# lancedb/lance

Hardware: AMD Instinct MI355X
Metric: QPS @ recall@10 (SIFT-1M IVF_PQ nlist=256 M=16) + index-build sec (higher is better)
Workload: dtype f32; 1 GPU; SIFT-1M-like 1Mx128 f32, IVF_PQ nlist=256 M=16 nbits=8, build+search on MI355X; n=1000000, d=128, nlist=256, m=16, k=10, nprobes=10, refine_factor=10, parallelism=single

## Files before the change

lance_amd/csrc/kernels.h:

```cpp
#pragma once
#include <stdint.h>

#include "common.h"

namespace lh {

struct PairwiseArgs {
  const void *x_native = nullptr;
  int x_dtype = 0;
  const float *x = nullptr;
  bool lanes32 = false;
  int64_t n = 0;
  int64_t ldx = 0;
  int x_batch_off = 0;
  const float *cent = nullptr;
  int k = 0;
  int64_t cent_batch_stride = 0;
  const float *bias = nullptr;
  int64_t bias_batch_stride = 0;
  uint32_t *ids = nullptr;
  float *dists = nullptr;
  int64_t out_batch_stride = 0;
  uint8_t *codes = nullptr;
  int codes_ld = 0;
  float *matrix = nullptr;
  const uint8_t *active = nullptr;
  bool x_aligned = false;
  bool cent_aligned = false;
  bool check_finite = false;
  const uint16_t *x_plane16 = nullptr;
  const float *x_plane_n2 = nullptr;
  int x_plane_dp = 0;
  float *part_vb = nullptr;
  float *part_v = nullptr;
  uint32_t *part_idx = nullptr;
};

struct PqmArgs {
  PairwiseArgs p;
  const void *xn = nullptr;
  const float *rcent = nullptr;
  const uint32_t *rpart = nullptr;
  int round_f16 = 0;
  uint32_t *fb_cnt;
  uint32_t *fb_items;
  int batches;
};
bool pq_mfma_supported(const PairwiseArgs &p, int d, int metric, int batches);
int launch_pq_mfma(lance_hip_ctx *ctx, const PairwiseArgs &p, int d, int batches);
bool pq_mfma_encode_supported(int dtype, int d, int m, int nbits, const void *x, const float *cent, const float *codebook, int64_t n);
int launch_pq_mfma_encode(lance_hip_ctx *ctx, int dtype, const void *x, int64_t n, int d, const float *cent, const uint32_t *part_ids,
                          int residual, const float *codebook, int m, uint8_t *codes);

struct FlatPool {
  const float *x;
  const void *x_native = nullptr;
  int x_dtype = 0;
  const uint64_t *row_ids;
  int64_t r0, r1;
  const float *q;
  int nq, k, cap;
  uint32_t *tkey;
  uint64_t *trid;
  uint32_t *cnt;
  uint32_t *pkeys;
  uint64_t *prids;
  uint32_t *overflow;
  const float *row_sy = nullptr;
  const float *q_norm = nullptr;
};

int launch_wide_filter(lance_hip_ctx *ctx, const FlatPool &fp, int d, int metric);
int build_allow_bits(lance_hip_ctx *ctx, const uint64_t *row_ids, uint64_t n, const uint8_t *allow_by_rowid, uint64_t n_allow, const uint32_t **bits_out);
bool flat_mfma_supported(int metric, int d, int nq, const void *x, const float *q);
int flat_mfma_prepare(lance_hip_ctx *ctx, const float *q, int nq, int d, const uint16_t **qhi, const uint16_t **qlo, const float **qn);
int launch_flat_filter_mfma(lance_hip_ctx *ctx, const FlatPool &e, int d, int metric, const uint16_t *qhi, const uint16_t *qlo, const float *qn);
bool flat_mfma_wide_supported(int metric, int d, int nq, int64_t n, const float *x, const float *q);
int flat_mfma_wide_prepare_rows(lance_hip_ctx *ctx, const float *x, int64_t n, int d, const uint16_t **xb, const float **xn2);
int flat_mfma_wide_prepare_queries(lance_hip_ctx *ctx, const float *q, int nq, int d, const uint16_t **qb, const float **qn2);
int launch_flat_filter_mfma_wide(lance_hip_ctx *ctx, const FlatPool &e, int d, int metric, const uint16_t *xb, const float *xn2, const uint16_t *qb,
                                 const float *qn2);

int launch_assign(lance_hip_ctx *ctx, const PairwiseArgs &p, int d, int metric, int batches);
bool assign_reads_native(PairwiseArgs p, int d, int batches);
bool encode_fused_supported(int dtype, int d, int m, int nbits, const void *x, const float *cent, const float *codebook);
int launch_encode_fused(lance_hip_ctx *ctx, int dtype, const void *x, int64_t n, int d, const float *cent, const uint32_t *part_ids,
                        int residual, const float *codebook, int m, uint8_t *codes);
bool xform_fused_supported(int dtype, int metric, int d, int m, int nbits, int64_t n, int nlist, const void *x, const float *cent,
                           const float *codebook, uint8_t *codes, bool lanes32);
int launch_xform_fused(lance_hip_ctx *ctx, int dtype, int metric, const void *x, int64_t n, int d, const float *cent, int nlist,
                       const float *codebook, int m, uint32_t *part_ids, float *dists, uint8_t *codes, bool round_f16);
bool xform_tail_supported(int d, int m, int nbits, int64_t n, const float *x, const float *cent, const float *codebook);
int launch_xform_tail(lance_hip_ctx *ctx, const float *x, int64_t n, int d, const float *cent, const uint32_t *part_ids, int residual, bool round_f16,
                      const float *codebook, int m, uint8_t *codes);
bool xform_pqtrain_supported(const PairwiseArgs &p, int sd, int batches);
int launch_xform_pqtrain(lance_hip_ctx *ctx, const PairwiseArgs &p, int sd, int batches, uint32_t *fb_cnt, uint32_t *fb_items);
bool xform_assign_supported(const PairwiseArgs &p, int d, int metric, int batches);
int launch_xform_assign(lance_hip_ctx *ctx, const PairwiseArgs &p, int d, int metric);
int launch_xform_sweep_groups(lance_hip_ctx *ctx, int metric, const float *q, uint32_t nq, int d, const float *cent, uint32_t nlist, uint32_t *maxbits,
                              float *gkey, int ng, float *e2, const uint16_t *cpl_ready = nullptr, const uint32_t *maxbits_ready = nullptr);
size_t xform_coarse_planes_elems(uint32_t nlist, int d);
int xform_coarse_planes(lance_hip_ctx *ctx, int metric, const float *cent, uint32_t nlist, int d, uint16_t *cpl, uint32_t *maxbits );
bool coarse_groups_shape(int d, uint32_t nlist);
bool mfma_assign_supported(const PairwiseArgs &p, int d, int batches);
int launch_assign_mfma(lance_hip_ctx *ctx, const PairwiseArgs &p, int d, int metric);
int launch_dist_matrix(lance_hip_ctx *ctx, const PairwiseArgs &p, int d, int metric, int batches);

int stable_group(lance_hip_ctx *ctx, const uint32_t *ids, int64_t n, int64_t id_stride, int k, int batches,
                 uint32_t *starts, uint32_t *sorted_rows, int64_t out_stride, const uint8_t *active);

int kmeans_train_batched(lance_hip_ctx *ctx, int metric, const float *x, int64_t n, int64_t ldx, int x_batch_off, int d,
                         int k, int B, uint32_t max_iters, double tol, float balance_factor_scaled, bool have_init,
                         const uint64_t *seeds, float *cent, double *loss_out, uint32_t *iters_out, bool f16_arith = false);

int kmeans_train_hierarchical(lance_hip_ctx *ctx, int metric, const float *x, int64_t n, int d, int target_k, uint32_t max_iters,
                              double tol, float bf_scaled, int hierarchical_k, uint64_t seed, float *cent_out, uint32_t *n_out,
                              bool f16_arith = false);
int check_dtype(int dtype, const char *what);
int model_dtype(int dtype);
int as_f32(lance_hip_ctx *ctx, int dtype, const void *p, size_t count, const char *slot, const float **out);
int widen_into(lance_hip_ctx *ctx, int dtype, const void *p, size_t count, float *dst);
int from_f32(lance_hip_ctx *ctx, int dtype, const float *src, void *dst, size_t count);
int launch_residual(lance_hip_ctx *ctx, const float *x, int64_t n, int d, const float *cent, const uint32_t *part_ids, float *out, bool f16);


bool pm_supported(const lance_hip_index *ix, uint32_t keff, int has_range, uint32_t nq, uint32_t nprobes);
int ivfpq_scan_merge_pm(lance_hip_ctx *ctx, const lance_hip_index *ix, const float *qs, uint32_t nq, const uint32_t *probes,
                        uint32_t nprobes, uint32_t keff, uint32_t k, bool do_refine, uint64_t *ids, float *dists,
                        uint64_t *cand_rid, uint32_t *cand_cnt, uint32_t *flags, const uint32_t *allow);
int find_partitions_f32(lance_hip_ctx *ctx, int metric, const float *qf, uint32_t nq, uint32_t d, const float *cf, uint32_t nlist,
                        uint32_t nprobes, uint32_t *part_ids, float *dists, bool lanes32);
bool flat_small_supported(int metric, int dtype, uint32_t d, uint32_t nq, uint32_t k, uint64_t n);
int flat_topk_small(lance_hip_ctx *ctx, int metric, int dtype, const void *x, const uint64_t *row_ids, uint64_t n, uint32_t d, const float *q,
                    uint32_t nq, uint32_t k, uint64_t *ids, float *dists, bool *done);
bool coarse_mfma_supported(int metric, int d, uint32_t nq, uint32_t nlist, uint32_t nprobes, bool lanes32, const float *q, const float *cent);
int find_partitions_mfma(lance_hip_ctx *ctx, int metric, const float *q, uint32_t nq, int d, const float *cent, uint32_t nlist, uint32_t nprobes,
                         float *matrix, uint32_t *part_ids, float *dists, const uint16_t *cpl_ready = nullptr, const uint32_t *maxbits_ready = nullptr);
int launch_normalize(lance_hip_ctx *ctx, const float *x, int64_t n, int d, float *out, bool f16);
int launch_normalize_planes(lance_hip_ctx *ctx, const float *x, int64_t n, int d, float *out, bool f16, uint16_t *plane16, int dp, float *n2);

int qscan_index_constants(lance_hip_ctx *ctx, lance_hip_index *ix);
constexpr int QSCAN_SEG_CAP = 256;
struct SelectOut;
bool qscan_supported(const lance_hip_index *ix, uint32_t nq, uint32_t nprobes);
bool qscan_tiled_shape(int m, int sd);
int qscan_classb_to_rescan(lance_hip_ctx *ctx, const uint32_t *tbound, uint32_t nq, uint32_t nprobes, uint32_t *seg_cnt, uint32_t *qovf);
int qscan_nearest_keys(lance_hip_ctx *ctx, const uint32_t *probes, uint32_t nq, uint32_t nprobes, uint32_t *keys, uint32_t nb = 1);
int qscan_item_tables(lance_hip_ctx *ctx, const uint32_t *pair_starts, int nlist, int G, uint32_t *item_start, int4 *desc, uint32_t max_items);
int qscan_group(lance_hip_ctx *ctx, const uint32_t *probes, uint32_t nq, uint32_t nprobes, int nlist, const uint32_t *tglobal,
                uint32_t *keys, uint32_t *tbound, uint32_t *pair_starts, uint32_t *pair_idx, uint32_t *item_start4, int4 *desc4,
                uint32_t max_items4, int G = 4, int dot = 0);
int qbound_launch(lance_hip_ctx *ctx, const lance_hip_index *ix, const float *qs, uint32_t nq, uint32_t keff, const uint32_t *pair_starts0,
                  const uint32_t *pair_idx0, uint32_t *item_start, int4 *desc, uint32_t max_items, uint32_t *tglobal, const uint32_t *allow);
int qscan_launch(lance_hip_ctx *ctx, const lance_hip_index *ix, const float *qs, uint32_t nq, uint32_t nprobes, const uint32_t *pair_idx,
                 const uint32_t *item_start4, const int4 *desc4, uint32_t max_items4, const uint32_t *tbound, uint32_t *seg_cnt,
                 uint32_t *seg_pos, uint32_t *qovf, const uint32_t *allow, const uint32_t *probes = nullptr);
bool qscan_pt_enabled(const lance_hip_index *ix);
int qscan_pt_mode(const lance_hip_index *ix);
int qbound_pt_launch(lance_hip_ctx *ctx, const lance_hip_index *ix, const float *qs, uint32_t nq, uint32_t nprobes, uint32_t keff,
                     const uint32_t *probes, const uint32_t *pair_starts0, const uint32_t *pair_idx0, uint32_t *item_start, int4 *desc,
                     uint32_t max_items, uint32_t *tglobal, const uint32_t *allow);
int qmerge_launch(lance_hip_ctx *ctx, const lance_hip_index *ix, const float *qs, uint32_t nq, const uint32_t *probes, uint32_t nprobes,
                  const uint32_t *tbound, uint32_t *tglobal, const uint32_t *seg_cnt, const uint32_t *seg_pos, const uint32_t *qovf,
                  uint32_t *pool_key, uint32_t *pool_pos, uint32_t *pool_cnt, int pool_cap, const SelectOut &o, const uint32_t *allow,
                  const uint32_t *qslack = nullptr, const float *seg_val = nullptr, const float *seg_scale = nullptr);
constexpr int LH_NOT_TAKEN = 1;
bool mscan_supported(const lance_hip_index *ix, uint32_t nq, uint32_t nprobes);
bool mscan_batch_shape(const lance_hip_index *ix, uint32_t nq, uint32_t nprobes);
bool mscan_dot_ready(const lance_hip_index *ix, uint32_t nq, uint32_t nprobes);
int mscan_launch(lance_hip_ctx *ctx, const lance_hip_index *ix, const float *qs, uint32_t nq, uint32_t nprobes, const uint32_t *probes,
                 const uint32_t *pair_starts, const uint32_t *pair_idx, const uint32_t *tbound, uint32_t *seg_cnt, uint32_t *seg_pos,
                 uint32_t *qovf, const uint32_t *allow, uint32_t **qslack_out, float **seg_val_out, float **seg_scale_out);
void mscan_cut_params(int *cut_shift, uint32_t *cut_slack);
int mscan_prewarm(lance_hip_ctx *ctx, const lance_hip_index *ix);
int msbound_launch(lance_hip_ctx *ctx, const lance_hip_index *ix, const float *qs, uint32_t nq, uint32_t keff, const uint32_t *pair_starts0,
                   const uint32_t *pair_idx0, uint32_t *item_start, int4 *desc, uint32_t max_items, uint32_t *tglobal, const uint32_t *allow,
                   uint32_t nb = 1);
int qscan_items(lance_hip_ctx *ctx, const uint32_t *pair_starts, int nvp, int G, uint32_t *item_start, int4 *desc, uint32_t max_items);
const uint8_t *raw_compact_prepare(lance_hip_ctx *ctx, const lance_hip_index *ix);

}
```

lance_amd/csrc/search_ms.hip:

```cpp
#include <algorithm>
#include <cmath>
#include <cstdio>
#include <cstdlib>
#include <cstring>
#include <vector>

#include "common.h"
#include "exact.cuh"
#include "index.h"
#include "kernels.h"
#include "search_common.cuh"
#include "q_common.cuh"

namespace lh {

typedef _Float16 ms_h8 __attribute__((ext_vector_type(8)));
typedef _Float16 ms_h4 __attribute__((ext_vector_type(4)));
typedef float ms_f16v __attribute__((ext_vector_type(16)));

constexpr float MS_SE = 30000.0f;
constexpr float MS_SLACK_CAP = 1500.0f;
constexpr int MS_CUT_SHIFT = 6;
typedef __attribute__((address_space(1))) const void *ms_gptr;
typedef __attribute__((address_space(3))) void *ms_lptr;

__global__ __launch_bounds__(256) void ms_codebook_kernel(const float *__restrict__ cb, int64_t nwords, int sd, float scale, _Float16 *__restrict__ cbh,
                                                          float *__restrict__ cbn2, const float *__restrict__ mu) {
  const int64_t w = (int64_t)blockIdx.x * 256 + threadIdx.x;
  if (w >= nwords) return;
  float s = 0.0f;
  for (int u = 0; u < sd; ++u) {
    const float v = mu ? cb[w * sd + u] - mu[(w >> 8) * sd + u] : cb[w * sd + u];
    cbh[w * sd + u] = (_Float16)(v * scale);
    s += v * v;
  }
  cbn2[w] = s;
}

__global__ __launch_bounds__(256) void ms_row_norm_kernel(const uint8_t *__restrict__ codes, int64_t n, int m, const float *__restrict__ cbn2, float sigma2,
                                                          float *__restrict__ row_cn2) {
  const int64_t r = (int64_t)blockIdx.x * 256 + threadIdx.x;
  if (r >= n) return;
  const uint8_t *rc = codes + r * m;
  float s = 0.0f;
  for (int mm = 0; mm < m; ++mm) s += cbn2[mm * 256 + rc[mm]];
  row_cn2[r] = s * sigma2;
}

__global__ __launch_bounds__(256) void ms_max_kernel(const float *__restrict__ v, int64_t n, uint32_t *__restrict__ out) {
  float m = 0.0f;
  for (int64_t i = (int64_t)blockIdx.x * 256 + threadIdx.x; i < n; i += (int64_t)gridDim.x * 256) m = fmaxf(m, v[i]);
#pragma unroll
  for (int o = 32; o > 0; o >>= 1) m = fmaxf(m, __shfl_xor(m, o, 64));
  if ((threadIdx.x & 63) == 0) atomicMax(out, __float_as_uint(m));
}

__global__ __launch_bounds__(256) void ms_part_max_kernel(const float *__restrict__ v, const uint32_t *__restrict__ part_offsets, float inv_sigma,
                                                          float *__restrict__ cmaxp) {
  __shared__ float wm[4];
  const uint32_t b = part_offsets[blockIdx.x], e = part_offsets[blockIdx.x + 1];
  float m = 0.0f;
  for (uint32_t i = b + threadIdx.x; i < e; i += 256) m = fmaxf(m, v[i]);
#pragma unroll
  for (int o = 32; o > 0; o >>= 1) m = fmaxf(m, __shfl_xor(m, o, 64));
  if ((threadIdx.x & 63) == 0) wm[threadIdx.x >> 6] = m;
  __syncthreads();
  if (threadIdx.x == 0) cmaxp[blockIdx.x] = sqrtf(fmaxf(fmaxf(wm[0], wm[1]), fmaxf(wm[2], wm[3]))) * inv_sigma * 1.0001f;
}

struct MsPrepArgs {
  const float *q, *centroids;
  const uint32_t *pair_idx;
  const uint32_t *pair_starts;
  const uint32_t *probes;
  const uint32_t *tbound;
  int d, nprobes, nlist, round_f16;
  float sigma;
  _Float16 *rh;
  f4 *prm;
  uint32_t *qslack;
  uint32_t *seg_cnt, *qovf, *ovf;
  uint32_t nan_slot;
  f2 *prm2;
  int dot = 0;
  float cmax = 0.0f;
  const float *cmaxp = nullptr;
  float cmax_full = 0.0f;
  const float *mu = nullptr;
  int m = 0;
};

constexpr int MS_PPW = 4;
__global__ __launch_bounds__(256) void ms_prep_kernel(MsPrepArgs p) {
  const uint32_t g0 = (blockIdx.x * 4u + (threadIdx.x >> 6)) * (uint32_t)MS_PPW;
  const uint32_t ng = p.pair_starts[p.nlist];
  const int lane = threadIdx.x & 63;
  if (blockIdx.x == 0 && threadIdx.x == 0) p.prm[p.nan_slot] = f4{__uint_as_float(0x7FC00000u), 0.0f, 0.0f, 0.0f};
  if (g0 >= ng) return;
  uint32_t pair[MS_PPW];
  const float *qv[MS_PPW], *cv[MS_PPW];
#pragma unroll
  for (int t = 0; t < MS_PPW; ++t) {
    const uint32_t g = min(g0 + (uint32_t)t, ng - 1u);
    pair[t] = p.pair_idx[g];
  }
#pragma unroll
  for (int t = 0; t < MS_PPW; ++t) {
    qv[t] = p.q + (int64_t)(pair[t] / (uint32_t)p.nprobes) * p.d;
    cv[t] = p.centroids + (int64_t)p.probes[pair[t]] * p.d;
  }
  float n2[MS_PPW], vmax[MS_PPW], qmu[MS_PPW];
  bool bad[MS_PPW];
#pragma unroll
  for (int t = 0; t < MS_PPW; ++t) { n2[t] = 0.0f; vmax[t] = 0.0f; qmu[t] = 0.0f; bad[t] = false; }
  for (int e = lane; e < p.d; e += 64) {
    float v[MS_PPW];
    const float mue = p.dot ? p.mu[e] : 0.0f;
#pragma unroll
    for (int t = 0; t < MS_PPW; ++t) v[t] = p.dot ? qv[t][e] : qv[t][e] - cv[t][e];
    const float hs = p.dot ? 0.5f * p.sigma : p.sigma;
#pragma unroll
    for (int t = 0; t < MS_PPW; ++t) {
      if (p.round_f16 && !p.dot) v[t] = __half2float(__float2half_rn(v[t]));
      n2[t] += v[t] * v[t];
      qmu[t] += v[t] * mue;
      vmax[t] = fmaxf(vmax[t], fabsf(v[t]));
      bad[t] |= !(fabsf(v[t]) < INFINITY);
      if (g0 + (uint32_t)t < ng) p.rh[(int64_t)(g0 + t) * p.d + e] = (_Float16)(v[t] * hs);
    }
  }
#pragma unroll
  for (int t = 0; t < MS_PPW; ++t) {
#pragma unroll
    for (int o = 32; o > 0; o >>= 1) {
      n2[t] += __shfl_xor(n2[t], o, 64); qmu[t] += __shfl_xor(qmu[t], o, 64); vmax[t] = fmaxf(vmax[t], __shfl_xor(vmax[t], o, 64));
    }
    bad[t] = __any(bad[t]);
  }
  float n2l = n2[0], vml = vmax[0], qmul = qmu[0]; bool badl = bad[0]; uint32_t pairl = pair[0];
#pragma unroll
  for (int t = 1; t < MS_PPW; ++t) if (lane == t) { n2l = n2[t]; vml = vmax[t]; qmul = qmu[t]; badl = bad[t]; pairl = pair[t]; }
  if (lane >= MS_PPW || g0 + (uint32_t)lane >= ng) return;
  const uint32_t q = pairl / (uint32_t)p.nprobes;
  const float T = key_to_float(p.tbound[q]);
  const float sqd = sqrtf((float)p.d) + 1.0f;
  const float sig2 = p.sigma * p.sigma;
  float s, eu, lim, zsum;
  bool ok;
  if (p.dot) {
    const float qn = sqrtf(n2l) * 1.000001f;
    const float G = qn * p.cmax * 1.000001f, Gf = qn * p.cmax_full * 1.000001f;
    const float e_abs = 6.1035156e-5f * sqd * (qn + 2.0f * p.cmax) / p.sigma + (float)p.d * 3.7252903e-9f / sig2;
    auto slack = [&](float g) {
      return 1.05f * (9.9609375e-4f * g + 1.5258789e-5f * (g + 1.0f + fabsf(T) + fabsf(qmul) + Gf) + 5.9604645e-8f * (float)((p.m + 2) * (p.m + 2))) + e_abs;
    };
    const float Tq = (T - 1.0f) + qmul;
    const float Tp = (Tq + G) + slack(G);
    s = MS_SE / Tp;
    const float Gp = fminf(G, qn * p.cmaxp[p.probes[pairl]] * 1.000001f);
    const float E = slack(Gp);
    eu = E * s * 1.1f + 3.0f;
    lim = Tq + E;
    zsum = (lim + G) * s;
    ok = !badl && fabsf(T) < INFINITY && Tp > 0.0f && Tp < INFINITY && s > 0.0f && s < INFINITY && Gf < INFINITY && vml * p.sigma < 60000.0f &&
         eu <= MS_SLACK_CAP && fabsf(lim * sig2) < INFINITY && G * s < 1e30f && fabsf(zsum) < 1e30f;
  } else {
    s = MS_SE / T;
    const float rn = sqrtf(n2l) * 1.000001f, st = sqrtf(T) * 1.000001f;
    const float e_abs = 6.1035156e-5f * sqd * (3.0f * rn + 2.0f * st) / p.sigma + (float)p.d * 3.7252903e-9f / (p.sigma * p.sigma);
    const float E = 1.05f * (1.9921875e-3f * rn * (rn + st) + 1.2207031e-4f * (n2l + T)) + e_abs;
    eu = E * s * 1.1f + 3.0f;
    lim = (T * 1.0000077f + E) - n2l;
    zsum = (T * 1.0000077f + E) * s;
    ok = !badl && T > 0.0f && T < INFINITY && s > 0.0f && s < INFINITY && n2l < INFINITY && vml * p.sigma < 60000.0f &&
         eu <= MS_SLACK_CAP && fabsf(lim * sig2) < INFINITY && n2l * s < 1e30f;
  }
  f4 o;
  if (ok) {
    o.x = -(lim * sig2); o.y = s / sig2; o.z = n2l * s;
    p.prm2[pairl] = f2{o.y, zsum};
    atomicMax(&p.qslack[q], (uint32_t)ceilf(eu));
  } else {
    o.x = __uint_as_float(0x7FC00000u); o.y = 0.0f; o.z = 0.0f;
    p.seg_cnt[pairl] = (uint32_t)Q_CAP + 1u;
    p.qovf[q] = 1u;
    p.ovf[1u + atomicAdd(&p.ovf[0], 1u)] = pairl;
  }
  o.w = __uint_as_float(pairl);
  p.prm[g0 + (uint32_t)lane] = o;
}

#ifndef LH_MS3_PB
#define LH_MS3_PB 512
#endif
constexpr int MS3_PB = LH_MS3_PB;
constexpr int MS3_RS = 3072;
static int ms_rows_per_slice() {
  static const int v = [] { const char *e = getenv("LANCE_HIP_MS_RS"); const int x = e ? atoi(e) : MS3_RS; return x >= 64 ? (x / 64) * 64 : MS3_RS; }();
  return v;
}
static int ms_rows_per_slice2() {
  static const int v = [] { const char *e = getenv("LANCE_HIP_MS_RS2"); const int x = e ? atoi(e) : 0; return x >= 64 ? (x / 64) * 64 : ms_rows_per_slice(); }();
  return v;
}
struct MsSlice { uint32_t off, np, row_begin, row_count, gs, qp, pad0, pad1; };
__host__ __device__ __forceinline__ uint32_t ms_nrs(uint32_t np, uint32_t rs1, uint32_t rs2) { return np <= rs1 ? (np ? 1u : 0u) : 1u + (np - rs1 + rs2 - 1u) / rs2; }
__device__ __forceinline__ uint32_t ms_row_begin(uint32_t rs, uint32_t rs1, uint32_t rs2) { return rs ? rs1 + (rs - 1u) * rs2 : 0u; }
__device__ __forceinline__ uint32_t ms_row_count(uint32_t rs, uint32_t np, uint32_t rs1, uint32_t rs2) {
  return rs ? min(rs2, np - ms_row_begin(rs, rs1, rs2)) : min(rs1, np);
}

__device__ __forceinline__ uint32_t ms_work_class(uint32_t rows, uint32_t pairs, uint32_t rs_rows) {
  const uint64_t w = (uint64_t)rows * pairs;
  return 31u - (uint32_t)min<uint64_t>(31u, w * 32u / ((uint64_t)rs_rows * MS3_PB));
}
struct MsSplit { uint32_t npb, blk, nrs; };
__device__ __forceinline__ MsSplit ms_split(uint32_t qp, uint32_t np, uint32_t rs_rows, uint32_t rs2_rows) {
  MsSplit r;
  r.npb = (qp + MS3_PB - 1) / MS3_PB;
  r.blk = r.npb ? ((((qp + r.npb - 1) / r.npb) + 31u) & ~31u) : 0u;
  r.nrs = ms_nrs(np, rs_rows, rs2_rows);
  return r;
}

__global__ __launch_bounds__(256) void ms_slice_table_kernel(const uint32_t *__restrict__ pair_starts, const uint32_t *__restrict__ part_offsets, int nlist,
                                                             uint32_t rs_rows, uint32_t rs2_rows, uint32_t cls_rows, uint32_t *__restrict__ slice_start,
                                                             uint32_t *__restrict__ slice_ctr, uint32_t *__restrict__ cls_cursor) {
  __shared__ uint32_t wsum[4];
  __shared__ uint32_t carry_s;
  __shared__ uint32_t hist[32];
  const int lane = threadIdx.x & 63, wave = threadIdx.x >> 6;
  if (threadIdx.x == 0) { carry_s = 0; slice_ctr[0] = 0u; }
  if (threadIdx.x < 32) hist[threadIdx.x] = 0u;
  __syncthreads();
  for (int base = 0; base < nlist; base += 256) {
    const int i = base + threadIdx.x;
    uint32_t v = 0;
    if (i < nlist) {
      const uint32_t qp = pair_starts[i + 1] - pair_starts[i], np = part_offsets[i + 1] - part_offsets[i];
      const MsSplit sp = ms_split(qp, np, rs_rows, rs2_rows);
      v = sp.npb * sp.nrs;
      for (uint32_t pb = 0; pb < sp.npb; pb += max(1u, sp.npb - 1u)) {
        const uint32_t pairs = min(sp.blk, qp - pb * sp.blk), npb_same = (pb + 1 == sp.npb) ? 1u : sp.npb - 1u;
        if (sp.nrs > 0) atomicAdd(&hist[ms_work_class(ms_row_count(0u, np, rs_rows, rs2_rows), pairs, cls_rows)], npb_same);
        if (sp.nrs > 2) atomicAdd(&hist[ms_work_class(rs2_rows, pairs, cls_rows)], npb_same * (sp.nrs - 2u));
        if (sp.nrs > 1) atomicAdd(&hist[ms_work_class(ms_row_count(sp.nrs - 1u, np, rs_rows, rs2_rows), pairs, cls_rows)], npb_same);
        if (sp.npb == 1) break;
      }
    }
    uint32_t incl = v;
#pragma unroll
    for (int off = 1; off < 64; off <<= 1) {
      const uint32_t t = __shfl_up(incl, off, 64);
      if (lane >= off) incl += t;
    }
    if (lane == 63) wsum[wave] = incl;
    __syncthreads();
    uint32_t woff = 0;
    for (int w = 0; w < wave; ++w) woff += wsum[w];
    const uint32_t carry = carry_s;
    if (i < nlist) slice_start[i] = carry + woff + incl - v;
    __syncthreads();
    if (threadIdx.x == 255) carry_s = carry + woff + incl;
    __syncthreads();
  }
  if (threadIdx.x == 0) {
    slice_start[nlist] = carry_s;
    uint32_t run = 0;
    for (int c = 0; c < 32; ++c) { cls_cursor[c] = run; run += hist[c]; }
  }
}

__global__ __launch_bounds__(256) void ms_slice_desc_kernel(const uint32_t *__restrict__ slice_start, const uint32_t *__restrict__ pair_starts,
                                                            const uint32_t *__restrict__ part_offsets, int nlist, uint32_t rs_rows, uint32_t rs2_rows, uint32_t cls_rows,
                                                            MsSlice *__restrict__ slices, uint32_t *__restrict__ cls_cursor, uint32_t *__restrict__ order) {
  const int part = blockIdx.x * 4 + (threadIdx.x >> 6), lane = threadIdx.x & 63;
  if (part >= nlist) return;
  const uint32_t s0 = slice_start[part], s1 = slice_start[part + 1];
  if (s1 == s0) return;
  const uint32_t off = part_offsets[part], np = part_offsets[part + 1] - off;
  const uint32_t gs = pair_starts[part], qp = pair_starts[part + 1] - gs;
  const MsSplit sp = ms_split(qp, np, rs_rows, rs2_rows);
  for (uint32_t t = (uint32_t)lane; t < s1 - s0; t += 64u) {
    const uint32_t pb = t / sp.nrs, rs = t - pb * sp.nrs;
    MsSlice u;
    u.off = off; u.np = np; u.row_begin = ms_row_begin(rs, rs_rows, rs2_rows); u.row_count = ms_row_count(rs, np, rs_rows, rs2_rows);
    u.gs = gs + pb * sp.blk; u.qp = min(sp.blk, qp - pb * sp.blk); u.pad0 = u.pad1 = 0u;
    slices[s0 + t] = u;
    order[atomicAdd(&cls_cursor[ms_work_class(u.row_count, u.qp, cls_rows)], 1u)] = s0 + t;
  }
}

struct MscanArgs {
  const uint32_t *order;
  const MsSlice *slices;
  const uint32_t *slice_start;
  uint32_t *slice_ctr;
  const uint8_t *codes;
  const _Float16 *cbh;
  const float *row_cn2;
  const _Float16 *rh;
  const f4 *prm;
  const f2 *prm2;
  uint32_t nan_slot;
  int nlist, nprobes;
  uint32_t *seg_cnt, *seg_pos;
  uint2 *seg_pv = nullptr;
  uint32_t *ovf;
  const uint32_t *allow;
#ifdef LH_TIMING_EXPERIMENTS
  int dbg = 0;
#endif
  unsigned long long *prof_slices = nullptr;
  unsigned long long *prof = nullptr;
};

#ifdef LH_TIMING_EXPERIMENTS
#define MS_DBG(p) ((p).dbg)
#else
#define MS_DBG(p) 0
#endif

constexpr int MS_QH = 64;
template <int SD, int KS, bool PROF = false>
__global__ __launch_bounds__(1024, 4) void ivfpq_mscan_kernel(MscanArgs p) {
  constexpr int D = KS * 16;
  constexpr int M = D / SD;
  constexpr int RB = D * 2;
  constexpr int CPR = RB / 16;
  constexpr int RPK = 256 / RB;
  constexpr int SPI = 16384 / RB;
  __shared__ __attribute__((aligned(16))) char sB[MS3_PB * RB];
  __shared__ __attribute__((aligned(16))) float sLim[MS3_PB];
  __shared__ __attribute__((aligned(16))) uint32_t sPair[MS3_PB];
  __shared__ __attribute__((aligned(8))) uint2 sQ[16][2][MS_QH + 1];
  __shared__ uint32_t s_slice, s_chunk;
  const int lane = threadIdx.x & 63, wave = __builtin_amdgcn_readfirstlane((int)(threadIdx.x >> 6));
  const int j = lane & 31, g = lane >> 5;
  const uint32_t nslices = p.slice_start[p.nlist];

  uint2 *const qw = &sQ[wave][0][0];
  uint32_t cur = 0;
  uint32_t qn = 0;
  uint32_t pd_n = 0, pd_base = 0;
  uint32_t pd_k = 0;
  float ncn2v = 0.0f;
  long long pc_t0 = 0, pc_stage = 0, pc_gather = 0, pc_tiles = 0, pc_flush = 0, pct = 0, pc_nchunk = 0;
  if constexpr (PROF) { pc_t0 = clock64(); pct = pc_t0; }
  auto flush_end = [&]() {
    if (pd_n) {
      if ((uint32_t)lane < pd_n && pd_k != 0xFFFFFFFFu) {
        const uint2 ent = qw[((uint32_t)(MS_QH + 1) - cur) + (uint32_t)lane];
        const uint32_t pair = sPair[ent.x >> 8];
        if (pd_k < (uint32_t)Q_CAP) {
          p.seg_pv[(int64_t)pair * Q_CAP + pd_k] = make_uint2(pd_base + (ent.x & 255u), ent.y);
        } else if (pd_k == (uint32_t)Q_CAP) {
          p.ovf[1u + atomicAdd(&p.ovf[0], 1u)] = pair;
        }
      }
      pd_n = 0;
    }
  };
  auto flush_begin = [&](uint32_t pos_base) {
    pd_k = 0xFFFFFFFFu;
    {
      const uint2 raw = qw[cur + (uint32_t)lane];
      const uint32_t ln_e = raw.x & 63u, vv = (raw.x >> 6) & 15u, jbb = raw.x >> 10;
      const float nv = __shfl(ncn2v, (int)(ln_e & 31u), 64);
      const uint2 ent = make_uint2(((jbb * 32u + 4u * (ln_e >> 5) + (vv & 3u) + 8u * (vv >> 2)) << 8) | (ln_e & 31u), __float_as_uint(__uint_as_float(raw.y) - nv));
      if ((uint32_t)lane < qn && !(MS_DBG(p) & 1)) {
        qw[cur + (uint32_t)lane] = ent;
        if (row_allowed(p.allow, pos_base + (ent.x & 255u))) pd_k = atomicAdd(&p.seg_cnt[sPair[ent.x >> 8]], 1u);
      }
    }
    pd_n = qn; pd_base = pos_base; qn = 0;
    cur = (uint32_t)(MS_QH + 1) - cur;
  };

  for (;;) {
    __syncthreads();
    if (threadIdx.x == 0) { s_slice = atomicAdd(p.slice_ctr, 1u); s_chunk = 0u; }
    __syncthreads();
    const uint32_t slice = s_slice;
    if (slice >= nslices) break;
    long long pc_slice0 = 0;
    if constexpr (PROF) pc_slice0 = clock64();
    const MsSlice U = p.slices[p.order[slice]];
    const int Qp = (int)U.qp;
    const int nslots = ((Qp + 31) >> 5) << 5;
    {
      const char *src = reinterpret_cast<const char *>(p.rh + (int64_t)U.gs * D);
#pragma unroll 4
      for (int it = 0; it < MS3_PB / SPI; ++it) {
        const int slot = it * SPI + wave * (SPI / 16) + lane / CPR, k = lane % CPR;
        if (it * SPI < nslots && slot < Qp)
          __builtin_amdgcn_global_load_lds((ms_gptr)(src + (int64_t)slot * RB + ((k ^ ((slot / RPK) & (CPR - 1))) << 4)),
                                           (ms_lptr)(&sB[(it * SPI + wave * (SPI / 16)) * RB]), 16, 0, 0);
      }
      const int slot = (wave & 7) * 64 + lane;
      if (slot < nslots) {
        const float *ps = reinterpret_cast<const float *>(slot < Qp && !(MS_DBG(p) & 2) ? p.prm + (int64_t)U.gs + slot : p.prm + p.nan_slot);
        if (wave < 8) __builtin_amdgcn_global_load_lds((ms_gptr)ps, (ms_lptr)(&sLim[(wave & 7) * 64]), 4, 0, 0);
        else __builtin_amdgcn_global_load_lds((ms_gptr)(ps + 3), (ms_lptr)(&sPair[(wave & 7) * 64]), 4, 0, 0);
      }
    }
    asm volatile("s_waitcnt vmcnt(0)" ::: "memory");
    __syncthreads();
    if constexpr (PROF) { const long long t = clock64(); pc_stage += t - pct; pct = t; }
    const uint32_t nchunks = (U.row_count + 31u) >> 5;
    const int nblk = nslots >> 5;
    const int row_end = (int)(U.row_begin + U.row_count);

    for (;;) {
      uint32_t c = 0;
      if (lane == 0) c = atomicAdd(&s_chunk, 1u);
      c = (uint32_t)__builtin_amdgcn_readfirstlane((int)c);
      if (c >= nchunks) break;
      const int row0 = (int)(U.row_begin + c * 32u);

      ms_h8 rw[KS];
      {
        const int rowc = min(row0 + j, row_end - 1);
        uint32_t cw[M / 4];
        {
          const uint4 *rc4 = reinterpret_cast<const uint4 *>(p.codes + ((int64_t)U.off + rowc) * M);
#pragma unroll
          for (int w = 0; w < M / 16; ++w) { const uint4 t = rc4[w]; cw[4 * w] = t.x; cw[4 * w + 1] = t.y; cw[4 * w + 2] = t.z; cw[4 * w + 3] = t.w; }
        }
        ncn2v = row0 + j < row_end ? -p.row_cn2[(int64_t)U.off + rowc] : -INFINITY;
        auto code = [&](int mm) -> uint32_t { return (cw[mm >> 2] >> (8 * (mm & 3))) & 255u; };
#pragma unroll
        for (int s = 0; s < KS; ++s) {
          if constexpr (SD == 8) {
            const uint32_t c0 = code(2 * s), c1 = code(2 * s + 1);
            const int mm = 2 * s + g;
            rw[s] = *reinterpret_cast<const ms_h8 *>(reinterpret_cast<const char *>(p.cbh) + (uint32_t)(((uint32_t)mm * 256u + (g ? c1 : c0)) * 16u));
          } else {
            static_assert(SD == 4, "sub-dimension 4 / 8");
            const uint32_t c0 = g ? code(4 * s + 2) : code(4 * s), c1 = g ? code(4 * s + 3) : code(4 * s + 1);
            const int mm = 4 * s + 2 * g;
            const ms_h4 lo = *reinterpret_cast<const ms_h4 *>(reinterpret_cast<const char *>(p.cbh) + (uint32_t)(((uint32_t)mm * 256u + c0) * 8u));
            const ms_h4 hi = *reinterpret_cast<const ms_h4 *>(reinterpret_cast<const char *>(p.cbh) + (uint32_t)(((uint32_t)(mm + 1) * 256u + c1) * 8u));
            rw[s] = ms_h8{lo[0], lo[1], lo[2], lo[3], hi[0], hi[1], hi[2], hi[3]};
          }
        }
      }
      const uint32_t pos_base = U.off + (uint32_t)row0;
      asm volatile("s_waitcnt vmcnt(0)" ::: "memory");
#pragma unroll
      for (int s = 0; s < KS; ++s) asm volatile("" : "+v"(rw[s]));
      asm volatile("" : "+v"(ncn2v));
      if constexpr (PROF) {
        const long long t = clock64(); pc_gather += t - pct; pct = t;
      }

      ms_h8 qa[KS];
      auto load_qa = [&](int jbx) {
        const int sl = jbx * 32 + j;
        const char *br = &sB[sl * RB];
        const int key = (sl / RPK) & (CPR - 1);
#pragma unroll
        for (int s = 0; s < KS; ++s) qa[s] = *reinterpret_cast<const ms_h8 *>(br + (((2 * s + g) ^ key) << 4));
      };
      load_qa(0);
      for (int jb = 0; jb < nblk; ++jb) {
        const int slot = jb * 32 + j;
        ms_f16v acc;
        {
          const f4 *lp = reinterpret_cast<const f4 *>(&sLim[jb * 32 + 4 * g]);
#pragma unroll
          for (int vq = 0; vq < 4; ++vq) {
            const f4 t = lp[2 * vq];
            acc[4 * vq] = t.x; acc[4 * vq + 1] = t.y; acc[4 * vq + 2] = t.z; acc[4 * vq + 3] = t.w;
          }
        }
        if (qn > (uint32_t)(MS_QH - 32)) {
          if constexpr (PROF) { const long long t = clock64(); pc_tiles += t - pct; pct = t; }
          flush_end(); flush_begin(pos_base);
          if constexpr (PROF) { const long long t = clock64(); pc_flush += t - pct; pct = t; }
        }
        uint32_t qraw = qn;
#pragma unroll
        for (int s = 0; s < KS; ++s) acc = __builtin_amdgcn_mfma_f32_32x32x16_f16(qa[s], rw[s], acc, 0, 0, 0);
        __builtin_amdgcn_sched_barrier(0);
        load_qa(min(jb + 1, nblk - 1));
        __builtin_amdgcn_sched_barrier(0);
        uint64_t mk[16];
#pragma unroll
        for (int v = 0; v < 16; ++v) mk[v] = __ballot(acc[v] <= ncn2v);
        __builtin_amdgcn_sched_barrier(0);
#pragma unroll
        for (int v = 0; v < 16; ++v) {
          if (mk[v]) {
            const uint32_t idx = min(qraw + __builtin_amdgcn_mbcnt_hi((uint32_t)(mk[v] >> 32), __builtin_amdgcn_mbcnt_lo((uint32_t)mk[v], 0u)),
                                     (uint32_t)MS_QH);
            if (acc[v] <= ncn2v) {
#ifdef MS_LN_RECOMPUTE
              uint32_t ln;
              asm volatile("v_mbcnt_lo_u32_b32 %0, -1, 0\n\tv_mbcnt_hi_u32_b32 %0, -1, %0" : "=v"(ln));
#else
              const uint32_t ln = (uint32_t)lane;
#endif
              qw[cur + idx] = make_uint2((((uint32_t)jb << 10) | (uint32_t)(v << 6)) | ln, __float_as_uint(acc[v]));
            }
            qraw += (uint32_t)__popcll(mk[v]);
          }
        }
        qn = min(qraw, (uint32_t)MS_QH);
        if (qraw > (uint32_t)MS_QH) {
          if (g == 0 && slot < Qp) {
            const uint32_t pair = sPair[slot];
            const uint32_t k = atomicAdd(&p.seg_cnt[pair], (uint32_t)Q_CAP + 1u);
            if (k <= (uint32_t)Q_CAP) p.ovf[1u + atomicAdd(&p.ovf[0], 1u)] = pair;
          }
        }
      }
      if constexpr (PROF) { const long long t = clock64(); pc_tiles += t - pct; pct = t; }
      flush_end(); flush_begin(pos_base);
      if constexpr (PROF) { const long long t = clock64(); pc_flush += t - pct; pct = t; ++pc_nchunk; }
    }
    flush_end();
    if constexpr (PROF) {
      __syncthreads();
      if (threadIdx.x == 0 && p.prof_slices) p.prof_slices[slice] = (unsigned long long)(clock64() - pc_slice0);
    }
  }
  if constexpr (PROF) {
    if (lane == 0) {
      const long long t1 = clock64();
      atomicAdd(&p.prof[0], (unsigned long long)pc_stage);
      atomicAdd(&p.prof[1], (unsigned long long)pc_gather);
      atomicAdd(&p.prof[2], (unsigned long long)pc_tiles);
      atomicAdd(&p.prof[3], (unsigned long long)pc_flush);
      atomicAdd(&p.prof[4], (unsigned long long)(t1 - pc_t0));
      atomicAdd(&p.prof[5], 1ull);
      atomicAdd(&p.prof[6], (unsigned long long)pc_nchunk);
      atomicMax(&p.prof[7], (unsigned long long)(t1 - pc_t0));
    }
  }
}

constexpr int MSB_BQ = 64;
constexpr int MSB_BINS = 512;
constexpr float MSB_MEAN_BIN = 496.0f;
struct MsBoundArgs {
  const float *q, *centroids, *cb_mean;
  const uint32_t *pair_idx0;
  const uint32_t *item_start;
  const int4 *desc;
  const uint32_t *part_offsets;
  const uint8_t *codes;
  const _Float16 *cbh;
  const float *row_cn2;
  int d, nlist, keff, round_f16;
  float sigma;
  uint32_t *tglobal;
  const uint32_t *allow;
  int dot = 0;
  float cmax = 0.0f, cmax_full = 0.0f;
  const float *cmaxp = nullptr;
  uint32_t nb = 1;
};

template <int SD, int KS>
__global__ __launch_bounds__(1024) void ms_bound_kernel(MsBoundArgs p) {
  constexpr int D = KS * 16;
  constexpr int M = D / SD;
  constexpr int RB = D * 2;
  constexpr int CPR = RB / 16;
  constexpr int RPK = 256 / RB;
  constexpr int CBB = 256 * D * 2;
  __shared__ __attribute__((aligned(16))) char sCB[CBB];
  __shared__ __attribute__((aligned(16))) char sB[MSB_BQ * RB];
  __shared__ __attribute__((aligned(16))) uint32_t sH[MSB_BQ * (MSB_BINS / 2)];
  __shared__ __attribute__((aligned(16))) float sPa[MSB_BQ];
  __shared__ __attribute__((aligned(16))) float sPb[MSB_BQ];
  __shared__ float sN2[MSB_BQ], sSb[MSB_BQ], sRmu[MSB_BQ];
  __shared__ uint32_t s_chunk;
  const int lane = threadIdx.x & 63, wave = threadIdx.x >> 6;
  const int j = lane & 31, g = lane >> 5;
  const uint32_t item = blockIdx.x;
  if (item >= p.item_start[p.nlist]) return;
  const int4 dsc = p.desc[item];
  const int part = dsc.x, i0 = dsc.y, cnt = dsc.z;
  const uint32_t off = p.part_offsets[part];
  const int np_all = (int)(p.part_offsets[part + 1] - off);
  if (np_all < p.keff) return;
  const int np = min(np_all, 65535);
  const int nslots = ((cnt + 31) >> 5) << 5;

  for (int b = (int)threadIdx.x * 16; b < CBB; b += 1024 * 16)
    *reinterpret_cast<uint4 *>(&sCB[b]) = *reinterpret_cast<const uint4 *>(reinterpret_cast<const char *>(p.cbh) + b);
  for (int i = threadIdx.x; i < MSB_BQ * (MSB_BINS / 2); i += 1024) sH[i] = 0u;
  if (threadIdx.x == 0) s_chunk = 0u;
  {
    constexpr int SPW = MSB_BQ / 16;
    const int e = 2 * lane;
    uint32_t qi[SPW];
#pragma unroll
    for (int t = 0; t < SPW; ++t) { const int sl = wave + 16 * t; qi[t] = sl < cnt ? p.pair_idx0[i0 + sl] / p.nb : 0u; }
    f2 qv[SPW], cv = {0.0f, 0.0f}, mu = {0.0f, 0.0f};
    if (e < D) {
      if (!p.dot) cv = *reinterpret_cast<const f2 *>(p.centroids + (int64_t)part * D + e);
      mu = *reinterpret_cast<const f2 *>(p.cb_mean + e);
    }
    const float hs = p.dot ? 0.5f * p.sigma : p.sigma;
#pragma unroll
    for (int t = 0; t < SPW; ++t) {
      qv[t] = f2{0.0f, 0.0f};
      if (wave + 16 * t < cnt && e < D) qv[t] = *reinterpret_cast<const f2 *>(p.q + (int64_t)qi[t] * D + e);
    }
#pragma unroll
    for (int t = 0; t < SPW; ++t) {
      const int sl = wave + 16 * t;
      if (sl >= nslots) break;
      const int key = (sl / RPK) & (CPR - 1);
      float n2 = 0.0f, vmax = 0.0f, rmu = 0.0f;
      bool bad = false;
      uint32_t packed = 0u;
      if (sl < cnt && e < D) {
        float v0 = qv[t].x - cv.x, v1 = qv[t].y - cv.y;
        if (p.round_f16 && !p.dot) { v0 = __half2float(__float2half_rn(v0)); v1 = __half2float(__float2half_rn(v1)); }
        n2 = v0 * v0 + v1 * v1;
        vmax = fmaxf(fabsf(v0), fabsf(v1));
        rmu = v0 * mu.x + v1 * mu.y;
        bad = !(fabsf(v0) < INFINITY) || !(fabsf(v1) < INFINITY);
        typedef _Float16 h2 __attribute__((ext_vector_type(2)));
        const h2 hv = {(_Float16)(v0 * hs), (_Float16)(v1 * hs)};
        packed = __builtin_bit_cast(uint32_t, hv);
      }
      if (e < D) *reinterpret_cast<uint32_t *>(&sB[sl * RB + ((((e >> 3) ^ key)) << 4) + ((e & 7) << 1)]) = packed;
#pragma unroll
      for (int o = 32; o > 0; o >>= 1) {
        n2 += __shfl_xor(n2, o, 64); rmu += __shfl_xor(rmu, o, 64); vmax = fmaxf(vmax, __shfl_xor(vmax, o, 64));
      }
      bad = __any(bad);
      if (lane == 0) {
        float a = __uint_as_float(0x7FC00000u), b = 0.0f, sb = 0.0f;
        if (sl < cnt) {
          const float G = p.dot ? sqrtf(n2) * 1.000001f * fminf(p.cmax, p.cmaxp[part]) * 1.000001f : 0.0f;
          const float mean = p.dot ? G : n2 - 2.0f * rmu + p.cb_mean[D];
          const float off = p.dot ? G : n2;
          sb = MSB_MEAN_BIN / mean;
          const float sig2 = p.sigma * p.sigma;
          const bool ok = !bad && off < INFINITY && vmax * p.sigma < 60000.0f && mean > 0.0f && mean < INFINITY && sb > 0.0f && sb < INFINITY &&
                          off * sb < 1e30f && sb / sig2 > 0.0f && sb / sig2 < INFINITY;
          if (ok) { a = sb / sig2; b = off * sb; }
        }
        sPa[sl] = a; sPb[sl] = b; sN2[sl] = n2; sSb[sl] = sb; sRmu[sl] = rmu;
      }
    }
  }
  for (int sl = nslots + (int)threadIdx.x; sl < MSB_BQ; sl += 1024) { sPa[sl] = __uint_as_float(0x7FC00000u); sPb[sl] = 0.0f; }
  __syncthreads();

  const uint32_t nchunks = ((uint32_t)np + 31u) >> 5;
  const int nblk = nslots >> 5;
  auto take = [&]() -> uint32_t {
    uint32_t c = 0;
    if (lane == 0) c = atomicAdd(&s_chunk, 1u);
    return (uint32_t)__builtin_amdgcn_readfirstlane((int)c);
  };
  uint32_t cwn[M / 4];
  float cn2n = INFINITY;
  auto request = [&](uint32_t c) {
    const int row0 = (int)(c * 32u);
    const int rowc = min(row0 + j, np - 1);
    const uint4 *rc4 = reinterpret_cast<const uint4 *>(p.codes + ((int64_t)off + rowc) * M);
#pragma unroll
    for (int w = 0; w < M / 16; ++w) { const uint4 t = rc4[w]; cwn[4 * w] = t.x; cwn[4 * w + 1] = t.y; cwn[4 * w + 2] = t.z; cwn[4 * w + 3] = t.w; }
    const bool live = row0 + j < np && row_allowed(p.allow, off + (uint32_t)rowc);
    cn2n = live ? p.row_cn2[(int64_t)off + rowc] : INFINITY;
  };
  uint32_t c = take();
  if (c < nchunks) request(c);
  while (c < nchunks) {
    const uint32_t cnext = take();
    uint32_t cw[M / 4];
#pragma unroll
    for (int w = 0; w < M / 4; ++w) cw[w] = cwn[w];
    const float cn2v = cn2n;
    asm volatile("s_waitcnt vmcnt(0)" ::: "memory");
#pragma unroll
    for (int w = 0; w < M / 4; ++w) asm volatile("" : "+v"(cw[w]));
    if (cnext < nchunks) request(cnext);
    ms_h8 rw[KS];
    {
      auto code = [&](int mm) -> uint32_t { return (cw[mm >> 2] >> (8 * (mm & 3))) & 255u; };
#pragma unroll
      for (int s = 0; s < KS; ++s) {
        if constexpr (SD == 8) {
          const uint32_t c0 = code(2 * s), c1 = code(2 * s + 1);
          const int mm = 2 * s + g;
          rw[s] = *reinterpret_cast<const ms_h8 *>(&sCB[((uint32_t)mm * 256u + (g ? c1 : c0)) * 16u]);
        } else {
          static_assert(SD == 4, "sub-dimension 4 / 8");
          const uint32_t c0 = g ? code(4 * s + 2) : code(4 * s), c1 = g ? code(4 * s + 3) : code(4 * s + 1);
          const int mm = 4 * s + 2 * g;
          const ms_h4 lo = *reinterpret_cast<const ms_h4 *>(&sCB[((uint32_t)mm * 256u + c0) * 8u]);
          const ms_h4 hi = *reinterpret_cast<const ms_h4 *>(&sCB[((uint32_t)(mm + 1) * 256u + c1) * 8u]);
          rw[s] = ms_h8{lo[0], lo[1], lo[2], lo[3], hi[0], hi[1], hi[2], hi[3]};
        }
      }
    }
    for (int jb = 0; jb < nblk; ++jb) {
      ms_h8 qa[KS];
      {
        const int sl = jb * 32 + j;
        const char *br = &sB[sl * RB];
        const int key = (sl / RPK) & (CPR - 1);
#pragma unroll
        for (int s = 0; s < KS; ++s) qa[s] = *reinterpret_cast<const ms_h8 *>(br + (((2 * s + g) ^ key) << 4));
      }
      ms_f16v acc;
#pragma unroll
      for (int v = 0; v < 16; ++v) acc[v] = 0.0f;
#pragma unroll
      for (int s = 0; s < KS; ++s) acc = __builtin_amdgcn_mfma_f32_32x32x16_f16(qa[s], rw[s], acc, 0, 0, 0);
      const f4 *pa = reinterpret_cast<const f4 *>(&sPa[jb * 32 + 4 * g]);
      const f4 *pb = reinterpret_cast<const f4 *>(&sPb[jb * 32 + 4 * g]);
#pragma unroll
      for (int vq = 0; vq < 4; ++vq) {
        const f4 a4 = pa[2 * vq], b4 = pb[2 * vq];
#pragma unroll
        for (int e = 0; e < 4; ++e) {
          const float t = __builtin_fmaf(acc[4 * vq + e] + cn2v, a4[e], b4[e]);
          if (t < (float)MSB_BINS) {
            const int bin = max((int)t, 0);
            const int slot = jb * 32 + 8 * vq + 4 * g + e;
            atomicAdd(&sH[slot * (MSB_BINS / 2) + (bin >> 1)], 1u << (16 * (bin & 1)));
          }
        }
      }
    }
    c = cnext;
  }
  __syncthreads();
  for (int sl = wave; sl < cnt; sl += 16) {
    const float a = sPa[sl];
    if (!(a > 0.0f)) continue;
    const uint4 hw = *reinterpret_cast<const uint4 *>(&sH[sl * (MSB_BINS / 2) + lane * 4]);
    const uint32_t loc[8] = {hw.x & 0xFFFFu, hw.x >> 16, hw.y & 0xFFFFu, hw.y >> 16, hw.z & 0xFFFFu, hw.z >> 16, hw.w & 0xFFFFu, hw.w >> 16};
    uint32_t tot = 0;
#pragma unroll
    for (int i = 0; i < 8; ++i) tot += loc[i];
    uint32_t incl = tot;
#pragma unroll
    for (int o = 1; o < 64; o <<= 1) {
      const uint32_t t = __shfl_up(incl, o, 64);
      if (lane >= o) incl += t;
    }
    uint32_t run = incl - tot;
    int found = -1;
#pragma unroll
    for (int i = 0; i < 8; ++i) {
      run += loc[i];
      if (found < 0 && run >= (uint32_t)p.keff) found = lane * 8 + i;
    }
    const uint64_t mask = __ballot(found >= 0);
    if (mask) {
      const int leader = __ffsll((long long)mask) - 1;
      const int bin = __shfl(found, leader, 64);
      if (lane == 0) {
        const float n2 = sN2[sl], sb = sSb[sl];
        const float Ta = (float)(bin + 1) / sb * 1.000001f;
        const float rn = sqrtf(n2) * 1.000001f, st = sqrtf(Ta) * 1.000001f;
        const float sqd = sqrtf((float)D) + 1.0f;
        if (p.dot) {
          const float G = rn * fminf(p.cmax, p.cmaxp[part]) * 1.000001f, Gf = rn * p.cmax_full * 1.000001f, qmu = sRmu[sl];
          const float tmag = fabsf(1.0f - qmu) + G + Ta;
          const float e_abs = 6.1035156e-5f * sqd * (rn + 2.0f * p.cmax) / p.sigma + (float)D * 3.7252903e-9f / (p.sigma * p.sigma);
          const float E = 1.05f * (9.9609375e-4f * G + 1.5258789e-5f * (G + 1.0f + tmag + fabsf(qmu) + Gf) + 5.9604645e-8f * (float)((M + 2) * (M + 2))) + e_abs;
          const float T = (((1.0f - qmu) - G) + Ta) + (1.1f * E + 1.5258789e-5f * tmag);
          if (fabsf(T) < INFINITY) atomicMin(&p.tglobal[p.pair_idx0[i0 + sl] / p.nb], order_key(T));
        } else {
        const float e_abs = 6.1035156e-5f * sqd * (3.0f * rn + 2.0f * st) / p.sigma + (float)D * 3.7252903e-9f / (p.sigma * p.sigma);
        const float E = 1.05f * (1.9921875e-3f * rn * (rn + st) + 1.2207031e-4f * (n2 + Ta)) + e_abs;
        const float T = (Ta + 1.1f * E) * 1.0000153f;
        if (T > 0.0f && T < INFINITY) atomicMin(&p.tglobal[p.pair_idx0[i0 + sl] / p.nb], order_key(T));
        }
      }
    }
  }
}

static bool ms_shape(const lance_hip_index *ix, int *sd_out, int *ks_out) {
  if (!ix || ix->m == 0 || ix->nbits != 8 || ix->d % ix->m != 0) return false;
  const int d = (int)ix->d, m = (int)ix->m, sd = d / m;
  if (!(m == 16 || m == 32)) return false;
  const bool ok = (d == 128 && (sd == 8 || sd == 4)) || (d == 64 && sd == 4);
  if (!ok) return false;
  if (sd_out) *sd_out = sd;
  if (ks_out) *ks_out = d / 16;
  return true;
}

bool mscan_batch_shape(const lance_hip_index *ix, uint32_t nq, uint32_t nprobes) {
  static const bool off = getenv("LANCE_HIP_NO_MSCAN") != nullptr;
  static const uint32_t minq = getenv("LANCE_HIP_MSCAN_MINQ") ? (uint32_t)std::max(1, atoi(getenv("LANCE_HIP_MSCAN_MINQ"))) : 96u;
  if (off || !ms_shape(ix, nullptr, nullptr)) return false;
  if (ix->metric != LANCE_HIP_L2 && ix->metric != LANCE_HIP_COSINE && ix->metric != LANCE_HIP_DOT) return false;
  return (uint64_t)nq * nprobes >= (uint64_t)minq * ix->nlist;
}

static bool ms_dot_skew_ok(const lance_hip_index *ix) {
  static const double skew = getenv("LANCE_HIP_DOT_FLOW_SKEW") ? atof(getenv("LANCE_HIP_DOT_FLOW_SKEW")) : 1e18;
  return (double)ix->max_part * (double)ix->nlist <= skew * (double)ix->n;
}

bool mscan_dot_ready(const lance_hip_index *ix, uint32_t nq, uint32_t nprobes) {
  static const bool off = getenv("LANCE_HIP_NO_MSBOUND") != nullptr || getenv("LANCE_HIP_NO_DOT_FLOW") != nullptr;
  if (off || !mscan_batch_shape(ix, nq, nprobes) || !ix->cb_mean) return false;
  if (!ms_dot_skew_ok(ix)) return false;
  lance_hip_index *mix = const_cast<lance_hip_index *>(ix);
  std::lock_guard<std::mutex> lk(mix->lazy_mu);
  return !mix->ms || mix->ms->usable;
}

bool mscan_supported(const lance_hip_index *ix, uint32_t nq, uint32_t nprobes) {
  return mscan_batch_shape(ix, nq, nprobes) && qscan_supported(ix, nq, nprobes);
}

static int mscan_prepare(lance_hip_ctx *ctx, lance_hip_index *ix) {
  std::lock_guard<std::mutex> lk(ix->lazy_mu);
  if (ix->ms) return LANCE_HIP_OK;
  const int d = (int)ix->d, m = (int)ix->m, sd = d / m;
  const int64_t nwords = (int64_t)m * 256;
  std::vector<float> cb((size_t)nwords * sd);
  LH_CHECK_HIP(hipMemcpyAsync(cb.data(), ix->codebook, cb.size() * 4, hipMemcpyDeviceToHost, ctx->stream));
  LH_CHECK_HIP(hipStreamSynchronize(ctx->stream));
  const bool dot = ix->metric == LANCE_HIP_DOT;
  std::vector<float> mu;
  if (dot && ix->cb_mean) {
    mu.resize((size_t)d);
    LH_CHECK_HIP(hipMemcpyAsync(mu.data(), ix->cb_mean, (size_t)d * 4, hipMemcpyDeviceToHost, ctx->stream));
    LH_CHECK_HIP(hipStreamSynchronize(ctx->stream));
  }
  auto *mc = new lance_hip_index::MsConst();
  if (dot) {
    if (!ix->cb_mean) { mc->usable = false; ix->ms = mc; return LANCE_HIP_OK; }
    double tot = 0.0;
    for (int mm = 0; mm < m; ++mm) {
      double best = 0.0;
      for (int c = 0; c < 256; ++c) {
        double sq = 0.0;
        for (int u = 0; u < sd; ++u) { const double v = cb[((size_t)mm * 256 + c) * sd + u]; sq += v * v; }
        best = std::max(best, sq);
      }
      tot += best;
    }
    mc->cmax_full = (float)(std::sqrt(tot) * 1.00001);
  }
  float cbmax = 0.0f;
  for (size_t i = 0; i < cb.size(); ++i) cbmax = std::max(cbmax, std::fabs(dot ? cb[i] - mu[(i / ((size_t)256 * sd)) * sd + i % sd] : cb[i]));
  if (!(cbmax > 0.0f) || !std::isfinite(cbmax) || ix->n == 0) {
    mc->usable = false;
    ix->ms = mc;
    return LANCE_HIP_OK;
  }
  int e = 0;
  (void)std::frexp(cbmax, &e);
  mc->sigma = std::ldexp(1.0f, 13 - e);
  bool ok = hipMalloc(reinterpret_cast<void **>(&mc->cbh), (size_t)nwords * sd * 2) == hipSuccess;
  ok = ok && hipMalloc(reinterpret_cast<void **>(&mc->cbn2), (size_t)nwords * 4) == hipSuccess;
  ok = ok && hipMalloc(reinterpret_cast<void **>(&mc->row_cn2), (size_t)ix->n * 4) == hipSuccess;
  if (dot) ok = ok && hipMalloc(reinterpret_cast<void **>(&mc->cmaxp), (size_t)std::max<uint32_t>(ix->nlist, 1u) * 4) == hipSuccess;
  auto drop = [&]() { (void)hipFree(mc->cbh); (void)hipFree(mc->cbn2); (void)hipFree(mc->row_cn2); (void)hipFree(mc->cmaxp); delete mc; };
  if (!ok) { drop(); set_error("matrix-core scan: out of device memory for the index constants"); return LANCE_HIP_ENOMEM; }
  hipLaunchKernelGGL(ms_codebook_kernel, dim3((unsigned)cdiv((uint64_t)nwords, 256)), dim3(256), 0, ctx->stream, ix->codebook, nwords, sd,
                     -2.0f * mc->sigma, reinterpret_cast<_Float16 *>(mc->cbh), mc->cbn2, dot ? ix->cb_mean : nullptr);
  hipLaunchKernelGGL(ms_row_norm_kernel, dim3((unsigned)cdiv(ix->n, 256)), dim3(256), 0, ctx->stream, ix->codes, (int64_t)ix->n, m, mc->cbn2,
                     mc->sigma * mc->sigma, mc->row_cn2);
  uint32_t rowmax_bits = 0;
  if (dot) {
    uint32_t *mx = reinterpret_cast<uint32_t *>(mc->cbn2);
    (void)lh::memset_async(mx, 0, 4, ctx->stream);
    hipLaunchKernelGGL(ms_max_kernel, dim3(256), dim3(256), 0, ctx->stream, mc->row_cn2, (int64_t)ix->n, mx);
    (void)hipMemcpyAsync(&rowmax_bits, mx, 4, hipMemcpyDeviceToHost, ctx->stream);
    hipLaunchKernelGGL(ms_part_max_kernel, dim3(ix->nlist), dim3(256), 0, ctx->stream, mc->row_cn2, ix->part_offsets, 1.0f / mc->sigma, mc->cmaxp);
    (void)lh::memset_async(mc->row_cn2, 0, (size_t)ix->n * 4, ctx->stream);
  }
  for (uint32_t pid = 0; pid < ix->nlist; ++pid) {
    const uint32_t rs = ms_nrs((uint32_t)(ix->part_offsets_h[pid + 1] - ix->part_offsets_h[pid]), (uint32_t)ms_rows_per_slice(), (uint32_t)ms_rows_per_slice2());
    mc->sum_rs += rs; mc->max_rs = std::max(mc->max_rs, rs);
  }
  if (hipGetLastError() != hipSuccess || hipStreamSynchronize(ctx->stream) != hipSuccess) {
    drop();
    set_error("matrix-core scan: building the index constants failed");
    return LANCE_HIP_ERUNTIME;
  }
  if (dot) {
    float rm; memcpy(&rm, &rowmax_bits, 4);
    mc->cmax = (float)(std::sqrt((double)rm) / (double)mc->sigma * 1.0001);
    if (!(mc->cmax > 0.0f) || !std::isfinite(mc->cmax)) mc->cmax = mc->cmax_full;
  }
  mc->usable = true;
  ix->ms = mc;
  return LANCE_HIP_OK;
}

int mscan_launch(lance_hip_ctx *ctx, const lance_hip_index *ix_c, const float *qs, uint32_t nq, uint32_t nprobes, const uint32_t *probes,
                 const uint32_t *pair_starts, const uint32_t *pair_idx, const uint32_t *tbound, uint32_t *seg_cnt, uint32_t *seg_pos,
                 uint32_t *qovf, const uint32_t *allow, uint32_t **qslack_out, float **seg_val_out, float **seg_scale_out) {
  lance_hip_index *ix = const_cast<lance_hip_index *>(ix_c);
  int sd = 0, ks = 0;
  if (!ms_shape(ix, &sd, &ks)) return LH_NOT_TAKEN;
  LH_TRY(mscan_prepare(ctx, ix));
  if (!ix->ms->usable) return LH_NOT_TAKEN;
  const int d = (int)ix->d, nlist = (int)ix->nlist;
  const size_t npairs = (size_t)nq * nprobes;
  const uint64_t cap = (uint64_t)ix->ms->sum_rs + (uint64_t)ix->ms->max_rs * cdiv(npairs, MS3_PB) + 8;
  _Float16 *rh = reinterpret_cast<_Float16 *>(ctx->scratch("ms.rh", (npairs + 32) * (size_t)d * 2));
  f4 *prm = reinterpret_cast<f4 *>(ctx->scratch("ms.prm", (npairs + 32) * 16));
  f2 *prm2 = reinterpret_cast<f2 *>(ctx->scratch("ms.prm2", npairs * 8));
  uint32_t *qslack = ctx->scratch_t<uint32_t>("ms.qslack", nq);
  uint32_t *slice_start = ctx->scratch_t<uint32_t>("ms.slice_start", (size_t)nlist + 2 + 32);
  MsSlice *slices = reinterpret_cast<MsSlice *>(ctx->scratch("ms.slices", cap * sizeof(MsSlice)));
  uint32_t *order = ctx->scratch_t<uint32_t>("ms.order", cap);
  float *seg_val = ctx->scratch_t<float>("ms.seg_val", npairs * Q_CAP * 2);
  uint32_t *ovf = ctx->scratch_t<uint32_t>("q.ovf", npairs + 1);
  if (!rh || !prm || !prm2 || !qslack || !slice_start || !slices || !order || !seg_val || !ovf) return LANCE_HIP_ENOMEM;
  uint32_t *slice_ctr = slice_start + nlist + 1, *cls_cursor = slice_ctr + 1;
  const uint32_t nan_slot = (uint32_t)npairs + 1u;
  {
    ScopedTimer t(ctx, "q_residual");
    LH_CHECK_HIP(lh::memset_multi(ctx->stream, {{seg_cnt, 0, npairs * 4}, {qovf, 0, (size_t)nq * 4}, {qslack, 0, (size_t)nq * 4}, {ovf, 0, 4}}));
    MsPrepArgs pa;
    pa.q = qs; pa.centroids = ix->centroids; pa.pair_idx = pair_idx; pa.pair_starts = pair_starts; pa.probes = probes; pa.tbound = tbound;
    pa.d = d; pa.nprobes = (int)nprobes; pa.nlist = nlist; pa.round_f16 = ix->dtype == LANCE_HIP_F16 ? 1 : 0;
    pa.sigma = ix->ms->sigma; pa.rh = rh; pa.prm = prm; pa.qslack = qslack; pa.seg_cnt = seg_cnt; pa.qovf = qovf; pa.ovf = ovf;
    pa.nan_slot = nan_slot; pa.prm2 = prm2;
    pa.dot = ix->metric == LANCE_HIP_DOT ? 1 : 0; pa.cmax = ix->ms->cmax; pa.cmax_full = ix->ms->cmax_full; pa.cmaxp = ix->ms->cmaxp; pa.mu = ix->cb_mean; pa.m = (int)ix->m;
    hipLaunchKernelGGL(ms_prep_kernel, dim3((unsigned)cdiv(npairs, 4 * MS_PPW)), dim3(256), 0, ctx->stream, pa);
    const uint32_t rs_rows = (uint32_t)ms_rows_per_slice(), rs2_rows = (uint32_t)ms_rows_per_slice2();
    static const bool no_order = getenv("LANCE_HIP_MS_NOORDER") != nullptr;
    const uint32_t cls_rows = no_order ? 0x40000000u : rs_rows;
    hipLaunchKernelGGL(ms_slice_table_kernel, dim3(1), dim3(256), 0, ctx->stream, pair_starts, ix->part_offsets, nlist, rs_rows, rs2_rows, cls_rows, slice_start,
                       slice_ctr, cls_cursor);
    hipLaunchKernelGGL(ms_slice_desc_kernel, dim3((unsigned)cdiv((uint64_t)nlist, 4)), dim3(256), 0, ctx->stream, slice_start, pair_starts, ix->part_offsets,
                       nlist, rs_rows, rs2_rows, cls_rows, slices, cls_cursor, order);
  }
  ScopedTimer t(ctx, "ivfpq_scan_c1");
  ScopedTimer tm(ctx, "ivfpq_mscan");
  MscanArgs a;
  a.order = order; a.slices = slices; a.slice_start = slice_start; a.slice_ctr = slice_ctr; a.codes = ix->codes;
  a.cbh = reinterpret_cast<const _Float16 *>(ix->ms->cbh); a.row_cn2 = ix->ms->row_cn2; a.rh = rh; a.prm = prm; a.prm2 = prm2;
  a.nan_slot = nan_slot; a.nlist = nlist; a.nprobes = (int)nprobes;
  a.seg_cnt = seg_cnt; a.seg_pos = seg_pos; a.seg_pv = reinterpret_cast<uint2 *>(seg_val); a.ovf = ovf; a.allow = allow;
#ifdef LH_TIMING_EXPERIMENTS
  static const int dbg = [] {
    const int v = getenv("LANCE_HIP_MS_DBG") ? atoi(getenv("LANCE_HIP_MS_DBG")) : 0;
    if (v) fprintf(stderr, "lance_hip: LANCE_HIP_MS_DBG=%d -- timing experiment, search RESULTS ARE WRONG\n", v);
    return v;
  }();
  a.dbg = dbg;
#endif
  static const int grid_env = getenv("LANCE_HIP_MS_GRID") ? atoi(getenv("LANCE_HIP_MS_GRID")) : 0;
  const unsigned grid = (unsigned)std::min<uint64_t>((uint64_t)(grid_env > 0 ? std::min(grid_env, ctx->num_cus) : ctx->num_cus), cap);
  static const bool prof = getenv("LANCE_HIP_MS_PROF") != nullptr;
  if (prof && sd == 8 && ks == 8 && !ctx->capturing) {
    a.prof = ctx->scratch_t<unsigned long long>("ms.prof", 8);
    if (!a.prof) return LANCE_HIP_ENOMEM;
    LH_CHECK_HIP(lh::memset_async(a.prof, 0, 64, ctx->stream));
    a.prof_slices = ctx->scratch_t<unsigned long long>("ms.prof_slices", cap);
    if (!a.prof_slices) return LANCE_HIP_ENOMEM;
    LH_CHECK_HIP(lh::memset_async(a.prof_slices, 0, cap * 8, ctx->stream));
    hipLaunchKernelGGL((ivfpq_mscan_kernel<8, 8, true>), dim3(grid), dim3(1024), 0, ctx->stream, a);
    unsigned long long h[8];
    LH_CHECK_HIP(hipMemcpyAsync(h, a.prof, 64, hipMemcpyDeviceToHost, ctx->stream));
    LH_CHECK_HIP(hipStreamSynchronize(ctx->stream));
    {
      std::vector<unsigned long long> st(cap);
      std::vector<MsSlice> sl(cap);
      std::vector<uint32_t> ord(cap), ss((size_t)nlist + 1);
      (void)hipMemcpy(st.data(), a.prof_slices, cap * 8, hipMemcpyDeviceToHost);
      (void)hipMemcpy(sl.data(), slices, cap * sizeof(MsSlice), hipMemcpyDeviceToHost);
      (void)hipMemcpy(ord.data(), order, cap * 4, hipMemcpyDeviceToHost);
      (void)hipMemcpy(ss.data(), slice_start, ((size_t)nlist + 1) * 4, hipMemcpyDeviceToHost);
      const uint32_t ns = ss[nlist];
      std::vector<uint32_t> idx(ns);
      for (uint32_t i = 0; i < ns; ++i) idx[i] = i;
      std::sort(idx.begin(), idx.end(), [&](uint32_t x, uint32_t y) { return st[x] > st[y]; });
      double tot = 0, totw = 0;
      for (uint32_t i = 0; i < ns; ++i) { tot += (double)st[i]; totw += (double)sl[ord[i]].row_count * sl[ord[i]].qp; }
      fprintf(stderr, "[ms prof] %u slices, mean %.0f ticks, mean ticks per 1000 cells %.2f; slowest (taken#, ticks, rows, pairs, ticks per 1000 cells):", ns, tot / ns, tot / totw * 1e3);
      for (uint32_t t = 0; t < std::min<uint32_t>(ns, 12); ++t) {
        const uint32_t i = idx[t];
        fprintf(stderr, " (%u, %llu, %u, %u, %.2f)", i, st[i], sl[ord[i]].row_count, sl[ord[i]].qp, (double)st[i] / ((double)sl[ord[i]].row_count * sl[ord[i]].qp) * 1e3);
      }
      fprintf(stderr, " | last taken:");
      for (uint32_t i = ns > 12 ? ns - 12 : 0; i < ns; ++i)
        fprintf(stderr, " (%u, %llu, %u, %u)", i, st[i], sl[ord[i]].row_count, sl[ord[i]].qp);
      fprintf(stderr, "\n");
    }
    if (h[5])
      fprintf(stderr, "[ms prof] waves=%llu chunks/wave %.2f | s_memtime ticks per wave: stage+barriers %.0f | gather %.0f | tiles %.0f | flush %.0f | life %.0f (longest %llu)\n",
              h[5], (double)h[6] / h[5], (double)h[0] / h[5], (double)h[1] / h[5], (double)h[2] / h[5], (double)h[3] / h[5], (double)h[4] / h[5], h[7]);
  } else if (sd == 8 && ks == 8) hipLaunchKernelGGL((ivfpq_mscan_kernel<8, 8>), dim3(grid), dim3(1024), 0, ctx->stream, a);
  else if (sd == 4 && ks == 8) hipLaunchKernelGGL((ivfpq_mscan_kernel<4, 8>), dim3(grid), dim3(1024), 0, ctx->stream, a);
  else if (sd == 4 && ks == 4) hipLaunchKernelGGL((ivfpq_mscan_kernel<4, 4>), dim3(grid), dim3(1024), 0, ctx->stream, a);
  else { set_error("matrix-core scan: unsupported shape (d=%d, sd=%d)", d, sd); return LANCE_HIP_EINVAL; }
  LH_CHECK_HIP(hipGetLastError());
  *qslack_out = qslack; *seg_val_out = seg_val; *seg_scale_out = reinterpret_cast<float *>(prm2);
  return LANCE_HIP_OK;
}

int msbound_launch(lance_hip_ctx *ctx, const lance_hip_index *ix_c, const float *qs, uint32_t nq, uint32_t keff, const uint32_t *pair_starts0,
                   const uint32_t *pair_idx0, uint32_t *item_start, int4 *desc, uint32_t max_items, uint32_t *tglobal, const uint32_t *allow,
                   uint32_t nb) {
  static const bool off = getenv("LANCE_HIP_NO_MSBOUND") != nullptr;
  lance_hip_index *ix = const_cast<lance_hip_index *>(ix_c);
  int sd = 0, ks = 0;
  const bool dot = ix->metric == LANCE_HIP_DOT;
  if (off || !ms_shape(ix, &sd, &ks) || !ix->cb_mean || (!dot && ix->max_part >= 65536u)) return LH_NOT_TAKEN;
  if (((reinterpret_cast<uintptr_t>(qs) | reinterpret_cast<uintptr_t>(ix->centroids)) & 7) != 0) return LH_NOT_TAKEN;
  LH_TRY(mscan_prepare(ctx, ix));
  if (!ix->ms->usable) return LH_NOT_TAKEN;
  const int nlist = (int)ix->nlist;
  LH_TRY(qscan_items(ctx, pair_starts0, nlist, MSB_BQ, item_start, desc, max_items));
  if (!((sd == 8 && ks == 8) || (sd == 4 && (ks == 8 || ks == 4)))) return LH_NOT_TAKEN;
  ScopedTimer t(ctx, "ivfpq_msbound");
  MsBoundArgs a;
  a.q = qs; a.centroids = ix->centroids; a.cb_mean = ix->cb_mean; a.pair_idx0 = pair_idx0; a.item_start = item_start; a.desc = desc;
  a.part_offsets = ix->part_offsets; a.codes = ix->codes; a.cbh = reinterpret_cast<const _Float16 *>(ix->ms->cbh); a.row_cn2 = ix->ms->row_cn2;
  a.d = (int)ix->d; a.nlist = nlist; a.keff = (int)keff; a.round_f16 = ix->dtype == LANCE_HIP_F16 ? 1 : 0; a.sigma = ix->ms->sigma;
  a.tglobal = tglobal; a.allow = allow;
  a.dot = ix->metric == LANCE_HIP_DOT ? 1 : 0; a.cmax = ix->ms->cmax; a.cmax_full = ix->ms->cmax_full; a.cmaxp = ix->ms->cmaxp;
  a.nb = std::max<uint32_t>(nb, 1u);
  const unsigned grid = (unsigned)std::min<uint64_t>(max_items, (uint64_t)nq * a.nb / MSB_BQ + (uint64_t)nlist + 1);
  if (sd == 8 && ks == 8) hipLaunchKernelGGL((ms_bound_kernel<8, 8>), dim3(grid), dim3(1024), 0, ctx->stream, a);
  else if (sd == 4 && ks == 8) hipLaunchKernelGGL((ms_bound_kernel<4, 8>), dim3(grid), dim3(1024), 0, ctx->stream, a);
  else hipLaunchKernelGGL((ms_bound_kernel<4, 4>), dim3(grid), dim3(1024), 0, ctx->stream, a);
  LH_CHECK_HIP(hipGetLastError());
  return LANCE_HIP_OK;
}

int mscan_prewarm(lance_hip_ctx *ctx, const lance_hip_index *ix_c) {
  lance_hip_index *ix = const_cast<lance_hip_index *>(ix_c);
  static const bool off = getenv("LANCE_HIP_NO_MSCAN") != nullptr;
  if (off || !ms_shape(ix, nullptr, nullptr) || !ix->model_finite) return LANCE_HIP_OK;
  if (ix->metric == LANCE_HIP_DOT && (!ms_dot_skew_ok(ix) || getenv("LANCE_HIP_NO_DOT_FLOW"))) return LANCE_HIP_OK;
  return mscan_prepare(ctx, ix);
}

void mscan_cut_params(int *cut_shift, uint32_t *cut_slack) { *cut_shift = MS_CUT_SHIFT; *cut_slack = 2u; }

}
```

lance_amd/csrc/search_pm.hip:

```cpp
#include <algorithm>
#include <cstdio>
#include <cstdlib>
#include <cstdlib>
#include <vector>

#include "common.h"
#include "exact.cuh"
#include "index.h"
#include "kernels.h"
#include "search_common.cuh"
#include "pm_common.cuh"

#pragma clang fp contract(off)

namespace lh {

#ifndef LH_PM_BS
#define LH_PM_BS 512
#endif
#ifndef LH_PM_STATIC_LUT
#define LH_PM_STATIC_LUT 0
#endif
constexpr int PM_BS = LH_PM_BS;
constexpr int PM_CAP = PM_BS + 256;
// ... 288 lines not shown
    }
#pragma unroll
    for (int u = 0; u < RP; ++u) scan_rows(base, u, cwc[u], T0, T1);
    __syncthreads();
    if constexpr (RP > 1) {
      if (misc[5] & ROUND_OVF) {
        __syncthreads();
        if (threadIdx.x == 0) { misc[0] = cnt0_before; misc[2] = cnt1_before; misc[5] &= ~ROUND_OVF; }
        __syncthreads();
#pragma unroll
        for (int u = 0; u < RP; ++u) {
          const uint32_t r0 = misc[0], r1 = misc[2];
          __syncthreads();
          if ((int)r0 > CAP - PM_BS) tighten_bs<PM_BS, CAP>(b0, p.keff, sorted, &misc[4]);
          if ((int)r1 > CAP - PM_BS) tighten_bs<PM_BS, CAP>(b1, p.keff, sorted, &misc[4]);
          scan_rows(base, u, cwc[u], misc[1], misc[3]);
          __syncthreads();
        }
        if (misc[5] & ROUND_OVF) {
          __syncthreads();
          if (threadIdx.x == 0) misc[5] = (misc[5] & ~ROUND_OVF) | FLAG_OVERFLOW;
          __syncthreads();
        }
      }
    } else {
      if (misc[5] & ROUND_OVF) {
        __syncthreads();
        if (threadIdx.x == 0) misc[5] = (misc[5] & ~ROUND_OVF) | FLAG_OVERFLOW;
        __syncthreads();
      }
    }
  }
  const long long pt4 = p.prof ? clock64() : 0;
  __shared__ uint32_t s_tg[2], s_base[2], s_tot[2], s_wr[2];
  for (int j = 0; j < 2; ++j) {
    if (j == 1 && !has1) break;
    const CandBuf &b = j ? b1 : b0;
    if ((int)*b.cnt > p.keff + 32) tighten_bs<PM_BS, CAP>(b, p.keff, sorted, &misc[4]);
    if ((int)*b.cnt > PM_BS) tighten_bs<PM_BS, CAP>(b, p.keff, sorted, &misc[4]);
  }
  __syncthreads();
  if (threadIdx.x < 2) {
    const int j = threadIdx.x;
    const CandBuf &b = j ? b1 : b0;
    const bool on = j == 0 || has1;
    uint32_t tg = on ? *b.T : 0u;
    if (on && *b.cnt > 0 && tg < misc[6 + j]) tg = min(atomicMin(&p.tglobal[j ? q1 : q0], tg), tg);
    s_tg[j] = tg; s_tot[j] = 0; s_wr[j] = 0;
  }
  __syncthreads();
  const int c0n = min((int)*b0.cnt, CAP), c1n = has1 ? min((int)*b1.cnt, CAP) : 0;
  {
    uint32_t m0 = 0, m1 = 0;
    const uint32_t tg0 = s_tg[0], tg1 = s_tg[1];
    for (int i = threadIdx.x; i < c0n; i += PM_BS) m0 += ck0[i] <= tg0 ? 1u : 0u;
    for (int i = threadIdx.x; i < c1n; i += PM_BS) m1 += ck1[i] <= tg1 ? 1u : 0u;
    if (m0) atomicAdd(&s_tot[0], m0);
    if (m1) atomicAdd(&s_tot[1], m1);
  }
  __syncthreads();
  if (threadIdx.x < 2) {
    const int j = threadIdx.x;
    const uint32_t tot = s_tot[j];
    s_base[j] = tot ? atomicAdd(&p.pool_cnt[j ? q1 : q0], tot) : 0u;
  }
  __syncthreads();
  for (int j = 0; j < 2; ++j) {
    const uint32_t tot = s_tot[j], basep = s_base[j], tg = s_tg[j];
    if (!tot) continue;
    const int qj = j ? q1 : q0;
    if (basep + tot > (uint32_t)p.pool_cap) {
      if (threadIdx.x == 0) atomicOr(&p.flags[qj], FLAG_OVERFLOW);
      continue;
    }
    const uint32_t *bk = j ? ck1 : ck0, *bp = j ? cp1 : cp0;
    const int c = j ? c1n : c0n;
    for (int i = threadIdx.x; i < c; i += PM_BS) {
      if (bk[i] <= tg) {
        const uint32_t slot = basep + atomicAdd(&s_wr[j], 1u);
        p.pool_key[(int64_t)qj * p.pool_cap + slot] = bk[i];
        p.pool_pos[(int64_t)qj * p.pool_cap + slot] = bp[i];
      }
    }
  }
  if (p.prof && threadIdx.x == 0) {
    const long long pt5 = clock64();
    atomicAdd(&p.prof[0], (unsigned long long)(pt1 - pt0)); atomicAdd(&p.prof[1], (unsigned long long)(pt2 - pt1));
    atomicAdd(&p.prof[2], (unsigned long long)(pt3 - pt2)); atomicAdd(&p.prof[3], (unsigned long long)(pt4 - pt3));
    atomicAdd(&p.prof[4], (unsigned long long)(pt5 - pt4)); atomicAdd(&p.prof[5], 1ull);
  }
  if (threadIdx.x == 0 && (misc[5] & FLAG_OVERFLOW)) {
    atomicOr(&p.flags[q0], FLAG_OVERFLOW);
    if (has1) atomicOr(&p.flags[q1], FLAG_OVERFLOW);
  }
}

template <int SD, int METRIC, int MU, int RPL, int CAP>
__global__ __launch_bounds__(PM_BS) void ivfpq_scan_pm_kernel(PmArgs p) {
  pm_scan_item<SD, METRIC, MU, RPL, CAP>(p, blockIdx.x);
}

template <int SD, int METRIC, int MU, int RPL, int CAP>
__global__ __launch_bounds__(PM_BS) void ivfpq_scan_pm_loop_kernel(PmArgs p) {
  const uint32_t lo = p.cls == 1 ? p.item_start[p.nlist] : 0u;
  const uint32_t hi = p.item_start[(p.cls == 0 ? 1 : 2) * p.nlist];
  for (uint32_t item = lo + blockIdx.x; item < hi; item += gridDim.x) {
    pm_scan_item<SD, METRIC, MU, RPL, CAP>(p, item);
    __syncthreads();
  }
}

constexpr int PMM_CAP = 1024;
__global__ __launch_bounds__(256) void ivfpq_merge_pm_kernel(const uint32_t *__restrict__ pool_key, const uint32_t *__restrict__ pool_pos,
                                                             const uint32_t *__restrict__ pool_cnt, const uint32_t *__restrict__ tglobal,
                                                             const uint64_t *__restrict__ row_ids, int pool_cap, SelectOut o) {
  __shared__ uint32_t ckey[PMM_CAP], cpos[PMM_CAP], sorted[256], misc[8];
  __shared__ uint64_t rid[SCAN_LCAP];
  __shared__ uint32_t skey[SCAN_LCAP], spos[SCAN_LCAP];
  __shared__ int s_amb;
  const int q = blockIdx.x;
  if (o.flags[q] & FLAG_OVERFLOW) return;
  const int n = min((int)pool_cnt[q], pool_cap);
  if (threadIdx.x == 0) { misc[0] = 0; misc[1] = tglobal[q]; s_amb = 0; }
  __syncthreads();
  CandBuf b{ckey, cpos, &misc[0], &misc[1]};
  const uint32_t *pk = pool_key + (int64_t)q * pool_cap, *pp = pool_pos + (int64_t)q * pool_cap;
  for (int base = 0; base < n; base += 512) {
    const bool need_tighten = (int)misc[0] > PMM_CAP - 512;
    __syncthreads();
    if (need_tighten) tighten_bs<256, PMM_CAP>(b, o.keff, sorted, &misc[2]);
    const uint32_t T = misc[1];
#pragma unroll
    for (int u = 0; u < 2; ++u) {
      const int i = base + u * 256 + threadIdx.x;
      if (i < n) {
        const uint32_t kk = pk[i];
        if (kk <= T) {
          const uint32_t slot = atomicAdd(&misc[0], 1u);
          if (slot < PMM_CAP) { ckey[slot] = kk; cpos[slot] = pp[i]; }
        }
      }
    }
    __syncthreads();
  }
  for (int iter = 0; iter < 8 && (int)misc[0] > SCAN_LCAP; ++iter) tighten_bs<256, PMM_CAP>(b, o.keff, sorted, &misc[2]);
  __syncthreads();
  int c = min((int)misc[0], PMM_CAP);
  if (c > SCAN_LCAP) {
    if (threadIdx.x == 0) atomicOr(&o.flags[q], FLAG_OVERFLOW);
    c = SCAN_LCAP;
  }
  for (int i = threadIdx.x; i < SCAN_LCAP; i += 256) {
    if (i < c) { skey[i] = ckey[i]; spos[i] = cpos[i]; rid[i] = row_ids[cpos[i]]; }
    else { skey[i] = 0xFFFFFFFFu; spos[i] = 0; rid[i] = ~0ull; }
  }
  __syncthreads();
  int Pq = 64;
  while (Pq < c) Pq <<= 1;
  bitonic_sort_kr<256>(skey, rid, spos, Pq);
  select_and_emit<256>(o, q, skey, rid, spos, c, &s_amb);
}

template <int SD, int METRIC>
static bool launch_pm_mu(lance_hip_ctx *ctx, const PmArgs &a, unsigned grid, size_t lds) {
  const int mu = a.m / 16;
  if (a.cls == 0 && a.bound_pass) {
    if (mu == 1) { hipLaunchKernelGGL((ivfpq_scan_pm_kernel<SD, METRIC, 1, 0, PM_CAP_BOUND>), dim3(grid), dim3(PM_BS), lds, ctx->stream, a); return true; }
    if (mu == 2) { hipLaunchKernelGGL((ivfpq_scan_pm_kernel<SD, METRIC, 2, 0, PM_CAP_BOUND>), dim3(grid), dim3(PM_BS), lds, ctx->stream, a); return true; }
  } else if (a.cls == 0) {
    if (mu == 1) { hipLaunchKernelGGL((ivfpq_scan_pm_kernel<SD, METRIC, 1, 1, PM_CAP>), dim3(grid), dim3(PM_BS), lds, ctx->stream, a); return true; }
    if (mu == 2) { hipLaunchKernelGGL((ivfpq_scan_pm_kernel<SD, METRIC, 2, 1, PM_CAP>), dim3(grid), dim3(PM_BS), lds, ctx->stream, a); return true; }
  } else if (a.unbounded) {
    if (mu == 1) { hipLaunchKernelGGL((ivfpq_scan_pm_loop_kernel<SD, METRIC, 1, 1, PM_CAP>), dim3(grid), dim3(PM_BS), lds, ctx->stream, a); return true; }
    if (mu == 2) { hipLaunchKernelGGL((ivfpq_scan_pm_loop_kernel<SD, METRIC, 2, 1, PM_CAP>), dim3(grid), dim3(PM_BS), lds, ctx->stream, a); return true; }
  } else {
    if (mu == 1) { hipLaunchKernelGGL((ivfpq_scan_pm_kernel<SD, METRIC, 1, PM_RPL1, PM_CAP>), dim3(grid), dim3(PM_BS), lds, ctx->stream, a); return true; }
    if (mu == 2) { hipLaunchKernelGGL((ivfpq_scan_pm_kernel<SD, METRIC, 2, 1, PM_CAP>), dim3(grid), dim3(PM_BS), lds, ctx->stream, a); return true; }
  }
  return false;
}

template <int METRIC>
static bool launch_pm_sd(lance_hip_ctx *ctx, const PmArgs &a, int sd, unsigned grid, size_t lds) {
  if (sd == 4) return launch_pm_mu<4, METRIC>(ctx, a, grid, lds);
  if (sd == 8) return launch_pm_mu<8, METRIC>(ctx, a, grid, lds);
  if (sd == 16) return launch_pm_mu<16, METRIC>(ctx, a, grid, lds);
  return false;
}

static bool pm_nobound() { static const bool v = getenv("LANCE_HIP_PM_NOBOUND") != nullptr; return v; }

bool pm_supported(const lance_hip_index *ix, uint32_t keff, int has_range, uint32_t nq, uint32_t nprobes) {
  const int d = (int)ix->d, m = (int)ix->m;
  if (ix->nbits != 8 || has_range || keff > (uint32_t)SCAN_MAX_KEFF) return false;
  if (m == 0 || d % m != 0) return false;
  const int sd = d / m;
  if (sd != 4 && sd != 8 && sd != 16) return false;
  if ((reinterpret_cast<uintptr_t>(ix->codebook) & 15) || (reinterpret_cast<uintptr_t>(ix->codes) & 15)) return false;
  if (qscan_tiled_shape(m, sd))
    return !pm_nobound() && qscan_supported(ix, nq, nprobes);
  if (m % 16 != 0 || m / 16 > 2) return false;
  return true;
}

static size_t pm_lds_base(int d, int m) {
  const int dpad = (d + 3) & ~3;
#if LH_PM_STATIC_LUT
  return (size_t)dpad * 8 + PM_BS * 4 + 8 * 4;
#else
  return (size_t)dpad * 8 + (size_t)m * 256 * 8 + PM_BS * 4 + 8 * 4;
#endif
}

static int ivfpq_scan_merge_q(lance_hip_ctx *ctx, const lance_hip_index *ix, const float *qs, uint32_t nq, const uint32_t *probes,
                              uint32_t nprobes, uint32_t keff, uint32_t k, bool do_refine, uint64_t *ids, float *dists,
                              uint64_t *cand_rid, uint32_t *cand_cnt, uint32_t *flags, const uint32_t *allow) {
  const int d = (int)ix->d, m = (int)ix->m, sd = d / m, nlist = (int)ix->nlist;
  const size_t npairs = (size_t)nq * nprobes;
  const uint32_t max_items2 = (uint32_t)(npairs / 2 + 2 * nlist + 2);
  const uint32_t max_items4 = (uint32_t)(npairs / 4 + nlist + 2);
  uint32_t *keys = ctx->scratch_t<uint32_t>("pm.keys", npairs);
  uint32_t *pair_starts = ctx->scratch_t<uint32_t>("pm.pair_starts", (size_t)2 * nlist + 1);
  uint32_t *pair_idx = ctx->scratch_t<uint32_t>("pm.pair_idx", npairs);
  uint32_t *item_start = ctx->scratch_t<uint32_t>("pm.item_start", (size_t)2 * nlist + 1);
  int4 *desc = ctx->scratch_t<int4>("pm.desc", max_items2);
  uint32_t *pair_starts0 = ctx->scratch_t<uint32_t>("q.pair_starts0", (size_t)nlist + 1);
  static const uint32_t dot_nb_env = getenv("LANCE_HIP_DOT_BOUND_LISTS") ? (uint32_t)std::max(1, atoi(getenv("LANCE_HIP_DOT_BOUND_LISTS"))) : 3u;
  static const uint32_t l2_nb_env = getenv("LANCE_HIP_BOUND_LISTS") ? (uint32_t)std::max(1, atoi(getenv("LANCE_HIP_BOUND_LISTS"))) : 1u;
  static const bool no_msbound_env = getenv("LANCE_HIP_NO_MSBOUND") != nullptr || getenv("LANCE_HIP_EXACT_BOUND") != nullptr;
  const uint32_t l2_nb = (!no_msbound_env && l2_nb_env > 1 && mscan_supported(ix, nq, nprobes) && qscan_pt_mode(ix) != 2) ? l2_nb_env : 1u;
  const uint32_t nb0 = std::min<uint32_t>(std::min<uint32_t>(ix->metric == LANCE_HIP_DOT ? dot_nb_env : l2_nb, 4u), nprobes);
  const uint32_t max_items0 = (uint32_t)((size_t)nq * nb0 / 2 + nlist + 2);
  uint32_t *pair_idx0 = ctx->scratch_t<uint32_t>("q.pair_idx0", (size_t)nq * nb0);
  uint32_t *item_start0 = ctx->scratch_t<uint32_t>("q.item_start0", (size_t)nlist + 1);
  int4 *desc0 = ctx->scratch_t<int4>("q.desc0", max_items0);
  uint32_t *item_start4 = ctx->scratch_t<uint32_t>("q.item_start4", (size_t)nlist + 1);
  int4 *desc4 = ctx->scratch_t<int4>("q.desc4", max_items4);
  uint32_t *tglobal = ctx->scratch_t<uint32_t>("pm.tglobal", (size_t)nq * 4);
  uint32_t *seg_cnt = ctx->scratch_t<uint32_t>("q.seg_cnt", npairs);
  uint32_t *seg_pos = ctx->scratch_t<uint32_t>("q.seg_pos", npairs * QSCAN_SEG_CAP);
  uint64_t pool_max = qscan_tiled_shape(m, sd) ? 65536 : 8192;
  while (pool_max > 8192 && (uint64_t)nq * pool_max * 8 > (1ull << 30)) pool_max /= 2;
  int pool_cap = (int)std::min<uint64_t>(pool_max, std::max<uint64_t>(512, (uint64_t)nprobes * (keff + 28)));
  pool_cap = (pool_cap + 255) & ~255;
  uint32_t *pool_key = ctx->scratch_t<uint32_t>("pm.pool_key", (size_t)nq * pool_cap);
  uint32_t *pool_pos = ctx->scratch_t<uint32_t>("pm.pool_pos", (size_t)nq * pool_cap);
  if (!keys || !pair_starts || !pair_idx || !item_start || !desc || !pair_starts0 || !pair_idx0 || !item_start0 || !desc0 || !item_start4 ||
      !desc4 || !tglobal || !seg_cnt || !seg_pos || !pool_key || !pool_pos)
    return LANCE_HIP_ENOMEM;
  uint32_t *pool_cnt = tglobal + nq, *tbound = tglobal + 2 * (size_t)nq, *qovf = tglobal + 3 * (size_t)nq;
  LH_CHECK_HIP(lh::memset_multi(ctx->stream, {{tglobal, 0xFF, (size_t)nq * 4}, {pool_cnt, 0, (size_t)nq * 4}}));
  PmArgs a;
  a.q = qs; a.probes = probes;
  a.centroids = ix->centroids; a.codebook = ix->codebook; a.part_offsets = ix->part_offsets; a.codes = ix->codes;
  a.d = d; a.m = m; a.nprobes = (int)nprobes; a.nlist = nlist; a.keff = (int)keff;
  const bool dot = ix->metric == LANCE_HIP_DOT;
  a.residual = dot ? 0 : 1;
  a.round_f16 = ix->dtype == LANCE_HIP_F16 ? 1 : 0;
  a.prof = nullptr;
  a.tglobal = tglobal; a.pool_key = pool_key; a.pool_pos = pool_pos; a.pool_cnt = pool_cnt; a.pool_cap = pool_cap; a.flags = flags;
  a.unbounded = 0; a.loop = 0; a.allow = allow;
  const bool tiled = qscan_tiled_shape(m, sd);
  static const bool exact_bound_env = getenv("LANCE_HIP_EXACT_BOUND") != nullptr;
  const bool exact_bound = exact_bound_env && !tiled && !dot;
  {
    ScopedTimer t(ctx, "pm_group");
    LH_TRY(qscan_nearest_keys(ctx, probes, nq, nprobes, keys, nb0));
    LH_TRY(stable_group(ctx, keys, (int64_t)nq * nb0, (int64_t)nq * nb0, nlist, 1, pair_starts0, pair_idx0, (int64_t)nq * nb0, nullptr));
    if (exact_bound) {
      hipLaunchKernelGGL(pm_item_table_kernel, dim3(1), dim3(256), 0, ctx->stream, pair_starts0, nlist, item_start0);
      hipLaunchKernelGGL(pm_item_desc_kernel, dim3((unsigned)cdiv(max_items0, 256)), dim3(256), 0, ctx->stream, item_start0, pair_starts0, pair_idx0,
                         nlist, nlist, 1, max_items0, desc0);
    }
  }
  if (exact_bound) {
    ScopedTimer t(ctx, "ivfpq_scan_c0");
    a.pair_starts = pair_starts0; a.pair_idx = pair_idx0; a.item_start = item_start0; a.desc = desc0;
    a.cls = 0; a.bound_pass = 1;
    const size_t lds = pm_lds_base(d, m) + (size_t)PM_CAP_BOUND * 16;
    const bool ok = launch_pm_sd<METRIC_L2>(ctx, a, sd, (unsigned)(nq / 2 + nlist + 1), lds);
    LH_REQUIRE(ok, "partition-major scan: unsupported shape (m=%d, sd=%d)", m, sd);
  } else if (!dot && qscan_pt_mode(ix) == 2) {
    ScopedTimer t(ctx, "ivfpq_scan_c0");
    LH_TRY(qbound_pt_launch(ctx, ix, qs, nq, nprobes, keff, probes, pair_starts0, pair_idx0, item_start0, desc0, (uint32_t)(nq / 4 + nlist + 2), tglobal,
                            allow));
  } else {
    ScopedTimer t(ctx, "ivfpq_scan_c0");
    int mb_rc = LH_NOT_TAKEN;
    if (mscan_supported(ix, nq, nprobes))
      mb_rc = msbound_launch(ctx, ix, qs, nq, keff, pair_starts0, pair_idx0, item_start0, desc0, (uint32_t)((size_t)nq * nb0 / 4 + nlist + 2), tglobal, allow, nb0);
    if (mb_rc < 0) return mb_rc;
    if (mb_rc == LH_NOT_TAKEN && dot) return LH_NOT_TAKEN;
    if (mb_rc == LH_NOT_TAKEN) LH_TRY(qbound_launch(ctx, ix, qs, nq, keff, pair_starts0, pair_idx0, item_start0, desc0, (uint32_t)(nq / 4 + nlist + 2), tglobal, allow));
  }
  {
    ScopedTimer t(ctx, "pm_group");
    LH_TRY(qscan_group(ctx, probes, nq, nprobes, nlist, tglobal, keys, tbound, pair_starts, pair_idx, item_start4, desc4, max_items4, 4, dot ? 1 : 0));
    hipLaunchKernelGGL(pm_item_table_kernel, dim3(1), dim3(256), 0, ctx->stream, pair_starts, 2 * nlist, item_start);
    hipLaunchKernelGGL(pm_item_desc_kernel, dim3((unsigned)cdiv(max_items2, 256)), dim3(256), 0, ctx->stream, item_start, pair_starts, pair_idx,
                       2 * nlist, nlist, (int)nprobes, max_items2, desc);
  }
  uint32_t *qslack = nullptr;
  float *seg_val = nullptr, *seg_scale = nullptr;
  int ms_rc = LH_NOT_TAKEN;
  if (mscan_supported(ix, nq, nprobes))
    ms_rc = mscan_launch(ctx, ix, qs, nq, nprobes, probes, pair_starts, pair_idx, tbound, seg_cnt, seg_pos, qovf, allow, &qslack, &seg_val, &seg_scale);
  if (ms_rc < 0) return ms_rc;
  if (ms_rc == LH_NOT_TAKEN && dot) return LH_NOT_TAKEN;
  if (ms_rc == LH_NOT_TAKEN) {
    qslack = nullptr; seg_val = nullptr; seg_scale = nullptr;
    LH_TRY(qscan_launch(ctx, ix, qs, nq, nprobes, pair_idx, item_start4, desc4, max_items4, tbound, seg_cnt, seg_pos, qovf, allow, probes));
  }
  static const bool q_stats = getenv("LANCE_HIP_Q_STATS") != nullptr;
  if (q_stats) {
    std::vector<uint32_t> sc(npairs), tb(nq);
    (void)hipMemcpyAsync(sc.data(), seg_cnt, npairs * 4, hipMemcpyDeviceToHost, ctx->stream);
    (void)hipMemcpyAsync(tb.data(), tbound, (size_t)nq * 4, hipMemcpyDeviceToHost, ctx->stream);
    (void)hipStreamSynchronize(ctx->stream);
    uint64_t tot = 0, ovf = 0, mx = 0, nb = 0, r0 = 0;
    for (size_t i = 0; i < npairs; ++i) { tot += std::min<uint32_t>(sc[i], QSCAN_SEG_CAP); ovf += sc[i] > (uint32_t)QSCAN_SEG_CAP; mx = std::max<uint64_t>(mx, sc[i]); if (i % nprobes == 0) r0 += sc[i]; }
    for (uint32_t i = 0; i < nq; ++i) nb += tb[i] == 0xFFFFFFFFu;
    fprintf(stderr, "[qscan] nq=%u nprobes=%u keff=%u survivors/query %.1f (nearest partition %.1f) max segment %llu overflowed segments %llu class-B queries %llu\n",
            nq, nprobes, keff, (double)tot / nq, (double)r0 / nq, (unsigned long long)mx, (unsigned long long)ovf, (unsigned long long)nb);
  }
  if (tiled) {
    ScopedTimer t(ctx, "ivfpq_scan_cb");
    LH_TRY(qscan_classb_to_rescan(ctx, tbound, nq, nprobes, seg_cnt, qovf));
  } else {
    ScopedTimer t(ctx, "ivfpq_scan_cb");
    a.pair_starts = pair_starts; a.pair_idx = pair_idx; a.item_start = item_start; a.desc = desc;
    a.cls = 1; a.bound_pass = 0; a.unbounded = 1; a.loop = 1;
    const size_t lds = pm_lds_base(d, m) + (size_t)PM_CAP * 16;
    const unsigned grid = (unsigned)std::min<uint64_t>((uint64_t)ctx->num_cus * 3, (uint64_t)max_items2);
    const bool ok = dot ? launch_pm_sd<METRIC_DOT>(ctx, a, sd, grid, lds) : launch_pm_sd<METRIC_L2>(ctx, a, sd, grid, lds);
    LH_REQUIRE(ok, "partition-major scan: unsupported shape (m=%d, sd=%d)", m, sd);
  }
  {
    SelectOut o;
    o.keff = (int)keff; o.k = (int)k; o.refine = do_refine ? 1 : 0;
    o.out_ids = ids; o.out_dists = dists; o.cand_rid = cand_rid; o.cand_cnt = cand_cnt; o.flags = flags;
    o.part_offsets = ix->part_offsets; o.nlist = nlist;
    ScopedTimer t(ctx, "ivfpq_merge");
    LH_TRY(qmerge_launch(ctx, ix, qs, nq, probes, nprobes, tbound, tglobal, seg_cnt, seg_pos, qovf, pool_key, pool_pos, pool_cnt, pool_cap, o, allow, qslack, seg_val, seg_scale));
  }
  LH_CHECK_HIP(hipGetLastError());
  return LANCE_HIP_OK;
}

int ivfpq_scan_merge_pm(lance_hip_ctx *ctx, const lance_hip_index *ix, const float *qs, uint32_t nq, const uint32_t *probes,
                        uint32_t nprobes, uint32_t keff, uint32_t k, bool do_refine, uint64_t *ids, float *dists,
                        uint64_t *cand_rid, uint32_t *cand_cnt, uint32_t *flags, const uint32_t *allow) {
  const int d = (int)ix->d, m = (int)ix->m, sd = d / m, nlist = (int)ix->nlist;
  const int scan_metric = ix->metric == LANCE_HIP_COSINE ? LANCE_HIP_L2 : ix->metric;
  if (!pm_nobound() && qscan_supported(ix, nq, nprobes)) {
    const int rc = ivfpq_scan_merge_q(ctx, ix, qs, nq, probes, nprobes, keff, k, do_refine, ids, dists, cand_rid, cand_cnt, flags, allow);
    if (rc != LH_NOT_TAKEN) return rc;
  }
  const size_t npairs = (size_t)nq * nprobes;
  uint32_t *pair_starts = ctx->scratch_t<uint32_t>("pm.pair_starts", (size_t)2 * nlist + 1);
  uint32_t *pair_idx = ctx->scratch_t<uint32_t>("pm.pair_idx", npairs);
  uint32_t *item_start = ctx->scratch_t<uint32_t>("pm.item_start", (size_t)2 * nlist + 1);
  uint32_t *tglobal = ctx->scratch_t<uint32_t>("pm.tglobal", (size_t)nq * 2);
  int pool_cap = (int)std::min<uint64_t>(8192, std::max<uint64_t>(512, (uint64_t)nprobes * (keff + 28)));
  pool_cap = (pool_cap + 255) & ~255;
  uint32_t *pool_key = ctx->scratch_t<uint32_t>("pm.pool_key", (size_t)nq * pool_cap);
  uint32_t *pool_pos = ctx->scratch_t<uint32_t>("pm.pool_pos", (size_t)nq * pool_cap);
  if (!pair_starts || !pair_idx || !item_start || !tglobal || !pool_key || !pool_pos) return LANCE_HIP_ENOMEM;
  uint32_t *pool_cnt = tglobal + nq;
  LH_CHECK_HIP(lh::memset_multi(ctx->stream, {{tglobal, 0xFF, (size_t)nq * 4}, {pool_cnt, 0, (size_t)nq * 4}}));
  uint32_t *keys = ctx->scratch_t<uint32_t>("pm.keys", npairs);
  const uint32_t max_items = (uint32_t)(npairs / 2 + 2 * nlist + 2);
  int4 *desc = ctx->scratch_t<int4>("pm.desc", max_items);
  if (!keys || !desc) return LANCE_HIP_ENOMEM;
  {
    ScopedTimer t(ctx, "pm_group");
    hipLaunchKernelGGL(pm_keys_kernel, dim3((unsigned)cdiv(npairs, 256)), dim3(256), 0, ctx->stream, probes, (int64_t)npairs, (int)nprobes,
                       nlist, keys);
    LH_TRY(stable_group(ctx, keys, (int64_t)npairs, (int64_t)npairs, 2 * nlist, 1, pair_starts, pair_idx, (int64_t)npairs, nullptr));
    hipLaunchKernelGGL(pm_item_table_kernel, dim3(1), dim3(256), 0, ctx->stream, pair_starts, 2 * nlist, item_start);
    hipLaunchKernelGGL(pm_item_desc_kernel, dim3((unsigned)cdiv(max_items, 256)), dim3(256), 0, ctx->stream, item_start, pair_starts, pair_idx,
                       2 * nlist, nlist, (int)nprobes, max_items, desc);
  }
  PmArgs a;
  a.q = qs; a.probes = probes; a.pair_starts = pair_starts; a.pair_idx = pair_idx; a.item_start = item_start;
  a.centroids = ix->centroids; a.codebook = ix->codebook; a.part_offsets = ix->part_offsets; a.codes = ix->codes;
  a.d = d; a.m = m; a.nprobes = (int)nprobes; a.nlist = nlist; a.keff = (int)keff;
  a.residual = scan_metric == LANCE_HIP_L2 ? 1 : 0;
  a.round_f16 = ix->dtype == LANCE_HIP_F16 ? 1 : 0;
  a.desc = desc;
  a.unbounded = 0; a.loop = 0; a.allow = allow;
  a.prof = nullptr;
  static const bool pm_prof = getenv("LANCE_HIP_PM_PROF") != nullptr;
  if (pm_prof) {
    a.prof = ctx->scratch_t<unsigned long long>("pm.prof", 8);
    if (a.prof) (void)lh::memset_async(a.prof, 0, 64, ctx->stream);
  }
  a.tglobal = tglobal; a.pool_key = pool_key; a.pool_pos = pool_pos; a.pool_cnt = pool_cnt; a.pool_cap = pool_cap; a.flags = flags;
  const size_t lds_base = pm_lds_base(d, m);
  {
    const bool nobound = pm_nobound();
    for (int pass = 0; pass < 2; ++pass) {
      if (nobound && pass == 1 && nprobes == 1) break;
      ScopedTimer t(ctx, pass == 0 ? "ivfpq_scan_c0" : "ivfpq_scan_c1");
      a.cls = pass == 0 ? 0 : (nobound ? 1 : 2);
      a.bound_pass = (pass == 0 && !nobound) ? 1 : 0;
      const size_t lds = lds_base + (size_t)(a.bound_pass ? PM_CAP_BOUND : PM_CAP) * 16;
      const size_t cpairs = a.cls == 0 ? (size_t)nq : (a.cls == 1 ? (size_t)nq * (nprobes - 1) : (size_t)nq * nprobes);
      const unsigned grid = (unsigned)(cpairs / 2 + (a.cls == 2 ? 2 : 1) * nlist + 1);
      bool ok = false;
      if (scan_metric == LANCE_HIP_DOT) {
        if (sd == 4) ok = launch_pm_mu<4, METRIC_DOT>(ctx, a, grid, lds);
        else if (sd == 8) ok = launch_pm_mu<8, METRIC_DOT>(ctx, a, grid, lds);
        else if (sd == 16) ok = launch_pm_mu<16, METRIC_DOT>(ctx, a, grid, lds);
      } else {
        if (sd == 4) ok = launch_pm_mu<4, METRIC_L2>(ctx, a, grid, lds);
        else if (sd == 8) ok = launch_pm_mu<8, METRIC_L2>(ctx, a, grid, lds);
        else if (sd == 16) ok = launch_pm_mu<16, METRIC_L2>(ctx, a, grid, lds);
      }
      LH_REQUIRE(ok, "partition-major scan: unsupported shape (m=%d, sd=%d)", m, sd);
      if (a.prof && pass == 1) {
        unsigned long long h[8];
        (void)hipMemcpyAsync(h, a.prof, 64, hipMemcpyDeviceToHost, ctx->stream);
        (void)hipStreamSynchronize(ctx->stream);
        if (h[5]) fprintf(stderr, "[pm prof] items=%llu clocks/item: desc %.0f | q,centroid,residual %.0f | LUT %.0f | scan %.0f | publish %.0f\n", h[5],
                          (double)h[0] / h[5], (double)h[1] / h[5], (double)h[2] / h[5], (double)h[3] / h[5], (double)h[4] / h[5]);
        (void)lh::memset_async(a.prof, 0, 64, ctx->stream);
      }
    }
  }
  {
    SelectOut o;
    o.keff = (int)keff; o.k = (int)k; o.refine = do_refine ? 1 : 0;
    o.out_ids = ids; o.out_dists = dists; o.cand_rid = cand_rid; o.cand_cnt = cand_cnt; o.flags = flags;
    o.part_offsets = ix->part_offsets; o.nlist = nlist;
    ScopedTimer t(ctx, "ivfpq_merge");
    hipLaunchKernelGGL(ivfpq_merge_pm_kernel, dim3(nq), dim3(256), 0, ctx->stream, pool_key, pool_pos, pool_cnt, tglobal, ix->row_ids, pool_cap, o);
  }
  LH_CHECK_HIP(hipGetLastError());
  return LANCE_HIP_OK;
}

}
```

lance_amd/csrc/search_q.hip:

```cpp
#include <algorithm>
#include <cstdio>
#include <cstdlib>

#include "common.h"
#include "exact.cuh"
#include "index.h"
#include "kernels.h"
#include "search_common.cuh"
#include "pm_common.cuh"
#include "q_common.cuh"

#pragma clang fp contract(off)

namespace lh {

__global__ __launch_bounds__(256) void q_tclass_keys_kernel(const uint32_t *__restrict__ probes, int64_t npairs, int nprobes, int nlist,
                                                            const uint32_t *__restrict__ tglobal, uint32_t *__restrict__ keys,
                                                            uint32_t *__restrict__ tbound, int dot) {
  const int64_t i = (int64_t)blockIdx.x * 256 + threadIdx.x;
  if (i >= npairs) return;
  const int64_t q = i / nprobes;
  const uint32_t T = tglobal[q];
  const bool usable = T > (dot ? 0x007FFFFFu : 0x80000000u) && T < 0xFF800000u;
  keys[i] = probes[i] + (usable ? 0u : (uint32_t)nlist);
// ... 17 lines not shown
    uint32_t incl = v;
#pragma unroll
    for (int off = 1; off < 64; off <<= 1) {
      const uint32_t t = __shfl_up(incl, off, 64);
      if (lane >= off) incl += t;
    }
    if (lane == 63) wsum[wave] = incl;
    __syncthreads();
    uint32_t woff = 0;
    for (int w = 0; w < wave; ++w) woff += wsum[w];
    const uint32_t carry = carry_s;
    if (i < nvp) item_start[i] = carry + woff + incl - v;
    __syncthreads();
    if (threadIdx.x == 255) carry_s = carry + woff + incl;
    __syncthreads();
  }
  if (threadIdx.x == 0) item_start[nvp] = carry_s;
}

__global__ __launch_bounds__(256) void q_item_desc_kernel(const uint32_t *__restrict__ item_start, const uint32_t *__restrict__ pair_starts,
                                                          int nvp, int G, uint32_t max_items, int4 *__restrict__ desc) {
  const uint32_t item = blockIdx.x * 256 + threadIdx.x;
  if (item >= max_items) return;
  int4 dsc = make_int4(-1, 0, 0, 0);
  if (item < item_start[nvp]) {
    int vp = (int)find_partition_dev(item_start, nvp, item);
    while (item_start[vp + 1] <= item) ++vp;
    const uint32_t g = item - item_start[vp];
    const uint32_t ps = pair_starts[vp], pe = pair_starts[vp + 1];
    const uint32_t i0 = ps + (uint32_t)G * g;
    dsc.x = vp;
    dsc.y = (int)i0;
    dsc.z = (int)min((uint32_t)G, pe - i0);
  }
  desc[item] = dsc;
}

__global__ __launch_bounds__(256) void q_residual_kernel(const float *__restrict__ q, const uint32_t *__restrict__ pair_idx,
                                                         const uint32_t *__restrict__ item_start, const int4 *__restrict__ desc,
                                                         const float *__restrict__ centroids, int d, int nlist, int pdiv, int round_f16,
                                                         f4 *__restrict__ rq) {
  const uint32_t item = blockIdx.x * 4u + (threadIdx.x >> 6);
  if (item >= item_start[nlist]) return;
  const int lane = threadIdx.x & 63;
  const int4 dsc = desc[item];
  const int part = dsc.x, i0 = dsc.y, cnt = dsc.z;
  uint32_t qj[Q_G];
#pragma unroll
  for (int j = 0; j < Q_G; ++j) qj[j] = pair_idx[i0 + (j < cnt ? j : 0)] / (uint32_t)pdiv;
  for (int dim = lane; dim < d; dim += 64) {
    const float cen = centroids[(int64_t)part * d + dim];
    f4 r4;
#pragma unroll
    for (int j = 0; j < Q_G; ++j) {
      float v = q[(int64_t)qj[j] * d + dim] - cen;
      if (round_f16) v = __half2float(__float2half_rn(v));
      r4[j] = -v;
    }
    rq[(int64_t)item * d + dim] = r4;
  }
}

template <int SD, int MU>
__global__ __launch_bounds__(Q_BS, (MU == 1 ? (SD <= 8 ? Q_WAVES : 6) : 4)) void ivfpq_qscan_kernel(QscanArgs p) {
  extern __shared__ __attribute__((aligned(16))) char smem[];
  constexpr int M = MU * 16;
  constexpr uint32_t CAPE = 65535u / M;
  constexpr uint32_t SE = CAPE - CAPE / 32;
  constexpr uint32_t LIM = SE + M + 2;
  static_assert(LIM < CAPE - 1, "a saturated entry must put the row above the limit");
  __shared__ __attribute__((aligned(16))) uint2 lutq[M * 256];
  uint32_t *cand = reinterpret_cast<uint32_t *>(smem);
  uint32_t *misc = cand + 4 * Q_CAP;
  float *sc = reinterpret_cast<float *>(misc + 4);
  uint16_t *csum = reinterpret_cast<uint16_t *>(sc + 4);

  const uint32_t item = blockIdx.x;
  if (item >= p.item_start[p.nlist]) return;
  {
    const int4 dsc = p.desc[item];
    const int part = dsc.x, i0 = dsc.y, cnt = dsc.z;
    const uint32_t off = p.part_offsets[part];
    const int np = (int)(p.part_offsets[part + 1] - off);
    if (np == 0) return;
    uint32_t qj[Q_G], rk[Q_G];
#pragma unroll
    for (int j = 0; j < Q_G; ++j) {
      const uint32_t pr = p.pair_idx[i0 + (j < cnt ? j : 0)];
      qj[j] = pr / (uint32_t)p.nprobes;
      rk[j] = pr % (uint32_t)p.nprobes;
    }
    if (threadIdx.x < Q_G) {
      misc[threadIdx.x] = 0;
      float s = 1e30f;
      if ((int)threadIdx.x < cnt) {
        const float T = key_to_float(p.tbound[qj[threadIdx.x]]);
        s = fminf((float)SE / T, 1e30f);
      }
      sc[threadIdx.x] = s * (1.0f / 65535.0f);
    }
    __syncthreads();
    const f4 *rq4 = p.rq + (int64_t)item * p.d;
    const uint32_t lim4[Q_G] = {LIM, LIM, LIM, LIM};
    {
      const int c = threadIdx.x & 255, half = __builtin_amdgcn_readfirstlane((int)(threadIdx.x >> 8));
      constexpr int MH = M / 2;
      const f4 s4 = *reinterpret_cast<const f4 *>(sc);
      const f2 s01 = {s4.x, s4.y}, s23 = {s4.z, s4.w};
#pragma unroll LH_Q_LUT_UNROLL
      for (int i = 0; i < MH; ++i) {
        const int mm = half * MH + i;
        f2 acc01, acc23;
        q_entry_acc<SD>(rq4 + mm * SD, p.codebook + ((int64_t)mm * 256 + c) * SD, acc01, acc23);
        lutq[mm * 256 + c] = q_entry_quantise<CAPE>(acc01, acc23, s01, s23);
      }
    }
    __syncthreads();
    {
      const uint8_t *pcodes = p.codes + (int64_t)off * M;
      uint4 cwn[MU];
      if ((int)threadIdx.x < np) {
#pragma unroll
        for (int w = 0; w < MU; ++w) cwn[w] = *reinterpret_cast<const uint4 *>(pcodes + (int64_t)threadIdx.x * M + w * 16);
      }
      for (int base = 0; base < np; base += Q_BS) {
        const int row = base + threadIdx.x;
        uint4 cw[MU];
#pragma unroll
        for (int w = 0; w < MU; ++w) cw[w] = cwn[w];
        if (row + Q_BS < np) {
#pragma unroll
          for (int w = 0; w < MU; ++w) cwn[w] = *reinterpret_cast<const uint4 *>(pcodes + (int64_t)(row + Q_BS) * M + w * 16);
        }
        if (row < np) {
          uint32_t a0 = 0, a1 = 0;
#pragma unroll
          for (int w = 0; w < MU; ++w) {
            const uint32_t cws[4] = {cw[w].x, cw[w].y, cw[w].z, cw[w].w};
#pragma unroll
            for (int e = 0; e < 4; ++e)
#pragma unroll
              for (int bb = 0; bb < 4; ++bb) {
                const uint2 v = lutq[(w * 16 + e * 4 + bb) * 256 + ((cws[e] >> (8 * bb)) & 255u)];
                a0 += v.x; a1 += v.y;
              }
          }
          const bool p0 = (a0 & 0xFFFFu) <= lim4[0], p1 = (a0 >> 16) <= lim4[1], p2 = (a1 & 0xFFFFu) <= lim4[2], p3 = (a1 >> 16) <= lim4[3];
          if ((p0 | p1 | p2 | p3) && row_allowed(p.allow, off + (uint32_t)row)) {
            const uint32_t pos = off + (uint32_t)row;
            if (p0) { const uint32_t slot = atomicAdd(&misc[0], 1u); if (slot < (uint32_t)Q_CAP) { cand[0 * Q_CAP + slot] = pos; csum[0 * Q_CAP + slot] = (uint16_t)(a0 & 0xFFFFu); } }
            if (p1) { const uint32_t slot = atomicAdd(&misc[1], 1u); if (slot < (uint32_t)Q_CAP) { cand[1 * Q_CAP + slot] = pos; csum[1 * Q_CAP + slot] = (uint16_t)(a0 >> 16); } }
            if (p2) { const uint32_t slot = atomicAdd(&misc[2], 1u); if (slot < (uint32_t)Q_CAP) { cand[2 * Q_CAP + slot] = pos; csum[2 * Q_CAP + slot] = (uint16_t)(a1 & 0xFFFFu); } }
            if (p3) { const uint32_t slot = atomicAdd(&misc[3], 1u); if (slot < (uint32_t)Q_CAP) { cand[3 * Q_CAP + slot] = pos; csum[3 * Q_CAP + slot] = (uint16_t)(a1 >> 16); } }
          }
        }
      }
    }
    __syncthreads();
#pragma unroll
    for (int j = 0; j < Q_G; ++j) {
      if (j < cnt) {
        const uint32_t raw = misc[j];
        const uint32_t n = raw > (uint32_t)Q_CAP ? (uint32_t)Q_CAP : raw;
        const int64_t seg = (int64_t)qj[j] * p.nprobes + rk[j];
        if (threadIdx.x == 0) {
          p.seg_cnt[seg] = raw;
          if (raw > (uint32_t)Q_CAP) { p.qovf[qj[j]] = 1u; p.ovf[1u + atomicAdd(&p.ovf[0], 1u)] = (uint32_t)seg; }
        }
        for (uint32_t i = threadIdx.x; i < n; i += Q_BS) {
          p.seg_pos[seg * Q_CAP + i] = cand[j * Q_CAP + i];
          p.seg_sum[seg * Q_CAP + i] = csum[j * Q_CAP + i];
        }
      }
    }
  }
}

template <int SD, int MU>
__global__ __launch_bounds__(Q_BS, (MU == 1 ? 6 : 4)) void ivfpq_qbound_kernel(QboundArgs p) {
  extern __shared__ __attribute__((aligned(16))) char smem[];
  constexpr int M = MU * 16;
  constexpr uint32_t CAPE = 65535u / M;
  constexpr uint32_t SE = CAPE - CAPE / 32;
  constexpr uint32_t HMAX = (uint32_t)(QB_BINS << QB_SHIFT) - 1u < CAPE - 1u ? (uint32_t)(QB_BINS << QB_SHIFT) - 1u : CAPE - 1u;
  __shared__ __attribute__((aligned(16))) uint2 lutq[M * 256];
  uint32_t *hist = reinterpret_cast<uint32_t *>(smem);
  float *sums = reinterpret_cast<float *>(hist + 4 * QB_BINS);
  float *sc = sums + 4;
  const int lane = threadIdx.x & 63, wave = threadIdx.x >> 6;
  const uint32_t item = blockIdx.x;
  if (item >= p.item_start[p.nlist]) return;
  {
    const int4 dsc = p.desc[item];
    const int part = dsc.x, i0 = dsc.y, cnt = dsc.z;
    const uint32_t off = p.part_offsets[part];
    const int np = (int)(p.part_offsets[part + 1] - off);
    if (np < p.keff) return;
    uint32_t qj[Q_G];
#pragma unroll
    for (int j = 0; j < Q_G; ++j) qj[j] = p.pair_idx[i0 + (j < cnt ? j : 0)];
    const f4 *rq4 = p.rq + (int64_t)item * p.d;
    for (int i = threadIdx.x; i < 4 * QB_BINS; i += Q_BS) hist[i] = 0u;
    if (threadIdx.x < 4) sums[threadIdx.x] = 0.0f;
    __syncthreads();
    const int c = threadIdx.x & 255, half = __builtin_amdgcn_readfirstlane((int)(threadIdx.x >> 8));
    constexpr int MH = M / 2;
    q_mean_entry_sums<Q_BS>(p.rq + (int64_t)item * p.d, p.cb_mean, p.d, sums);
    __syncthreads();
    if (threadIdx.x < Q_G) {
      const float mean = sums[threadIdx.x] + p.cb_mean[p.d];
      float s = 1e30f;
      if ((int)threadIdx.x < cnt && mean > 0.0f && mean < INFINITY) s = fminf((float)SE / mean, 1e30f);
      sc[threadIdx.x] = s;
    }
    __syncthreads();
    {
      const f4 s4 = *reinterpret_cast<const f4 *>(sc) * (1.0f / 65535.0f);
      const f2 s01 = {s4.x, s4.y}, s23 = {s4.z, s4.w};
#pragma unroll 1
      for (int i = 0; i < MH; ++i) {
        const int mm = half * MH + i;
        f2 acc01, acc23;
        q_entry_acc<SD>(rq4 + mm * SD, p.codebook + ((int64_t)mm * 256 + c) * SD, acc01, acc23);
        lutq[mm * 256 + c] = q_entry_quantise<CAPE>(acc01, acc23, s01, s23);
      }
    }
    __syncthreads();
    {
      const uint8_t *pcodes = p.codes + (int64_t)off * M;
      for (int row = threadIdx.x; row < np; row += Q_BS) {
        uint32_t a0 = 0, a1 = 0;
#pragma unroll
        for (int w = 0; w < MU; ++w) {
          const uint4 cw = *reinterpret_cast<const uint4 *>(pcodes + (int64_t)row * M + w * 16);
          const uint32_t cws[4] = {cw.x, cw.y, cw.z, cw.w};
#pragma unroll
          for (int e = 0; e < 4; ++e)
#pragma unroll
            for (int bb = 0; bb < 4; ++bb) {
              const uint2 v = lutq[(w * 16 + e * 4 + bb) * 256 + ((cws[e] >> (8 * bb)) & 255u)];
              a0 += v.x; a1 += v.y;
            }
        }
        const uint32_t sj[4] = {a0 & 0xFFFFu, a0 >> 16, a1 & 0xFFFFu, a1 >> 16};
        if (row_allowed(p.allow, off + (uint32_t)row)) {
#pragma unroll
          for (int j = 0; j < Q_G; ++j)
            if (sj[j] <= HMAX) atomicAdd(&hist[j * QB_BINS + (sj[j] >> QB_SHIFT)], 1u);
        }
      }
    }
    __syncthreads();
    if (wave < cnt) {
      const uint32_t *h = hist + wave * QB_BINS;
      constexpr int PER = QB_BINS / 64;
      uint32_t loc[PER], tot = 0;
#pragma unroll
      for (int i = 0; i < PER; ++i) { loc[i] = h[lane * PER + i]; tot += loc[i]; }
      uint32_t incl = tot;
#pragma unroll
      for (int o = 1; o < 64; o <<= 1) {
        const uint32_t t = __shfl_up(incl, o, 64);
        if (lane >= o) incl += t;
      }
      uint32_t run = incl - tot;
      int found = -1;
#pragma unroll
      for (int i = 0; i < PER; ++i) {
        run += loc[i];
        if (found < 0 && run >= (uint32_t)p.keff) found = lane * PER + i;
      }
      const uint64_t mask = __ballot(found >= 0);
      if (mask) {
        const int leader = __ffsll((long long)mask) - 1;
        const int bin = __shfl(found, leader, 64);
        if (lane == 0) {
          const float B = (float)(((uint32_t)bin + 1u) << QB_SHIFT);
          const float T = (B + (float)M) / sc[wave] * 1.00001f;
          if (T > 0.0f && T < INFINITY) atomicMin(&p.tglobal[qj[wave]], order_key(T));
        }
      }
    }
  }
}

constexpr int QM_G = 16;

struct QmergeArgs {
  const float *q;
  const uint32_t *probes;
  const float *centroids, *codebook;
  const uint8_t *codes;
  const uint64_t *row_ids;
  int d, nprobes, round_f16;
  int qm_g;
  int vec4;
  const uint16_t *seg_sum;
  int cut_shift;
  uint32_t cut_slack;
  const uint32_t *qslack;
  const float *seg_val;
  const uint2 *seg_pv;
  const f2 *seg_scale;
#ifdef LH_TIMING_EXPERIMENTS
  int dbg;
#define QM_DBG_RETURN(a, n) do { if ((a).dbg == (n)) return; } while (0)
#else
#define QM_DBG_RETURN(a, n) do { } while (0)
#endif
  const uint32_t *tbound;
  uint32_t *tglobal;
  const uint32_t *seg_cnt, *seg_pos;
  uint32_t *pool_key, *pool_pos, *pool_cnt;
  int pool_cap;
  const uint32_t *qovf;
  const uint32_t *ovf;
  const uint32_t *allow;
  SelectOut o;
};

template <int SD, int MU, int BS, bool DOT = false>
__global__ __launch_bounds__(BS) void ivfpq_qrescan_kernel(QmergeArgs a) {
  extern __shared__ __attribute__((aligned(16))) char smem[];
  constexpr int M = MU * 16;
  constexpr int QV = SD / 4;
  constexpr int QMET = DOT ? METRIC_DOT : METRIC_L2;
  constexpr int CAP = BS > 256 ? 2 * BS : 1024;
  __shared__ uint32_t ckey[CAP], cpos[CAP], sorted[BS], misc[8];
  const SelectOut &o = a.o;
  const int dpad = (a.d + 3) & ~3;
  float *r = reinterpret_cast<float *>(smem);
  float *lutx = r + dpad;
  CandBuf b{ckey, cpos, &misc[0], &misc[1]};
  const uint32_t nseg = a.ovf[0];
  for (uint32_t it = blockIdx.x; it < nseg; it += gridDim.x) {
    const uint32_t seg = a.ovf[1 + it];
    const int q = (int)(seg / (uint32_t)a.nprobes);
    const uint32_t part = a.probes[seg];
    const float *qv = a.q + (int64_t)q * a.d;
    __syncthreads();
    const uint32_t t_start = min(a.tbound[q], __hip_atomic_load(&a.tglobal[q], __ATOMIC_RELAXED, __HIP_MEMORY_SCOPE_AGENT));
    if (threadIdx.x == 0) {
      misc[0] = 0; misc[1] = t_start; misc[3] = 0;
      const_cast<uint32_t *>(a.qovf)[q] = 1u;
    }
    for (int e = threadIdx.x; e < a.d; e += BS) {
      float v = qv[e];
      if constexpr (!DOT) {
        v = v - a.centroids[(int64_t)part * a.d + e];
        if (a.round_f16) v = __half2float(__float2half_rn(v));
      }
      r[e] = v;
    }
    __syncthreads();
    for (int idx = threadIdx.x; idx < M * 256; idx += BS) {
      const int mm = idx >> 8;
      RegVec<SD> av;
#pragma unroll
      for (int u = 0; u < QV; ++u) av.q[u] = *reinterpret_cast<const f4 *>(&r[mm * SD + 4 * u]);
      lutx[idx] = finish_metric<QMET>(dist_exact<SD, QMET>(av, a.codebook + (int64_t)idx * SD));
    }
    __syncthreads();
    const uint32_t off = o.part_offsets[part];
    const int np = (int)(o.part_offsets[part + 1] - off);
    for (int base = 0; base < np; base += BS) {
      const bool need_tighten = (int)misc[0] > CAP - BS;
      __syncthreads();
      if (need_tighten) tighten_bs<BS, CAP>(b, o.keff, sorted, &misc[2]);
      const uint32_t T = misc[1];
      const int row = base + threadIdx.x;
      if (row < np) {
        const uint8_t *rc = a.codes + ((int64_t)off + row) * M;
        float dist = 0.0f;
#pragma unroll
        for (int w = 0; w < MU; ++w) {
          const uint4 cw = *reinterpret_cast<const uint4 *>(rc + w * 16);
          const uint32_t cws[4] = {cw.x, cw.y, cw.z, cw.w};
#pragma unroll
          for (int e = 0; e < 4; ++e)
#pragma unroll
            for (int bb = 0; bb < 4; ++bb) dist += lutx[(w * 16 + e * 4 + bb) * 256 + ((cws[e] >> (8 * bb)) & 255u)];
        }
        if constexpr (DOT) dist = dist - ((float)M - 1.0f);
        const uint32_t kk = order_key(dist);
        if (kk <= T && row_allowed(a.allow, off + (uint32_t)row)) {
          const uint32_t slot = atomicAdd(&misc[0], 1u);
          if (slot < (uint32_t)CAP) { ckey[slot] = kk; cpos[slot] = off + (uint32_t)row; } else misc[3] = 1u;
        }
      }
      __syncthreads();
    }
    for (int iter = 0; iter < 3; ++iter) {
      const bool more = (int)misc[0] > o.keff + 28;
      __syncthreads();
      if (!more) break;
      tighten_bs<BS, CAP>(b, o.keff, sorted, &misc[2]);
    }
    __syncthreads();
    const int c = min((int)misc[0], CAP);
    if (threadIdx.x == 0) {
      uint32_t basep = 0xFFFFFFFFu;
      if (!misc[3] && c > 0) {
        if (misc[1] < t_start) atomicMin(&a.tglobal[q], misc[1]);
        basep = atomicAdd(&a.pool_cnt[q], (uint32_t)c);
      }
      if (misc[3] || (c > 0 && basep + (uint32_t)c > (uint32_t)a.pool_cap)) { atomicOr(&o.flags[q], FLAG_OVERFLOW); basep = 0xFFFFFFFFu; }
      misc[4] = basep;
    }
    __syncthreads();
    const uint32_t basep = misc[4];
    if (basep != 0xFFFFFFFFu) {
      for (int i = threadIdx.x; i < c; i += BS) {
        a.pool_key[(int64_t)q * a.pool_cap + basep + i] = ckey[i];
        a.pool_pos[(int64_t)q * a.pool_cap + basep + i] = cpos[i];
      }
    }
  }
}

#ifndef LH_QM_WAVES
#define LH_QM_WAVES 6
#endif
#if LH_QM_WAVES > 0
#define LH_QM_BOUNDS(BS) __launch_bounds__(BS, (SD <= 8 && MU == 1 ? LH_QM_WAVES : 4))
#else
#define LH_QM_BOUNDS(BS) __launch_bounds__(BS)
#endif
template <int SD, int MU, int BS, bool DOT = false>
__global__ LH_QM_BOUNDS(BS) void ivfpq_qmerge_kernel(QmergeArgs a) {
  extern __shared__ __attribute__((aligned(16))) char smem[];
  constexpr int M = MU * 16;
  constexpr int QV = SD / 4;
  constexpr int QMET = DOT ? METRIC_DOT : METRIC_L2;
  constexpr int CAP = BS == 128 ? 512 : 1024;
  static_assert(BS >= SCAN_MAX_KEFF, "tighten_bs selects among one value per lane");
  __shared__ uint32_t ckey[CAP], cpos[CAP], sorted[BS], misc[8];
  uint64_t *rid = reinterpret_cast<uint64_t *>(smem);
  uint32_t *skey = reinterpret_cast<uint32_t *>(rid + SCAN_LCAP);
  uint32_t *spos = skey + SCAN_LCAP;
  __shared__ uint32_t s_cnt[QM_G + 1], s_pre[QM_G + 1];
  __shared__ f2 s_yz[QM_G];
  __shared__ int s_amb;
  constexpr int QM_LC = 512;
  __shared__ uint32_t s_hist[512], l_pos[QM_LC], s_cut, l_cnt;
  __shared__ uint8_t l_rr[QM_LC];
  const SelectOut &o = a.o;
  const int q = blockIdx.x;
  if (o.flags[q] & FLAG_OVERFLOW) return;
  const uint32_t tb = a.tbound[q];
  const bool class_a = tb != 0xFFFFFFFFu;
  if (threadIdx.x == 0) { misc[0] = 0; misc[1] = a.tglobal[q]; misc[3] = 0; s_amb = 0; }
  __syncthreads();
  CandBuf b{ckey, cpos, &misc[0], &misc[1]};
  if (!class_a || a.qovf[q]) {
    const int n = min((int)a.pool_cnt[q], a.pool_cap);
    const uint32_t *pk = a.pool_key + (int64_t)q * a.pool_cap, *pp = a.pool_pos + (int64_t)q * a.pool_cap;
    for (int base = 0; base < n; base += BS) {
      const bool need_tighten = (int)misc[0] > CAP - BS;
      __syncthreads();
      if (need_tighten) tighten_bs<BS, CAP>(b, o.keff, sorted, &misc[2]);
      const uint32_t T = misc[1];
      const int i = base + threadIdx.x;
      if (i < n) {
        const uint32_t kk = pk[i];
        if (kk <= T) {
          const uint32_t slot = atomicAdd(&misc[0], 1u);
          if (slot < (uint32_t)CAP) { ckey[slot] = kk; cpos[slot] = pp[i]; } else misc[3] = 1u;
        }
      }
      __syncthreads();
    }
  }
  if (class_a) {
    const int dpad = (a.d + 3) & ~3;
    float *r = reinterpret_cast<float *>(smem);
    const float *qv = a.q + (int64_t)q * a.d;
    for (int i = threadIdx.x; i < 512; i += BS) s_hist[i] = 0u;
    if (threadIdx.x == 0) s_cut = 0xFFFFFFFFu;
    for (int g0 = 0; a.cut_shift >= 0 && g0 < a.nprobes; g0 += QM_G) {
      const int ng = min(QM_G, a.nprobes - g0);
      __syncthreads();
      if ((int)threadIdx.x < ng) {
        const uint32_t c = a.seg_cnt[(int64_t)q * a.nprobes + g0 + threadIdx.x];
        s_cnt[threadIdx.x] = c > (uint32_t)Q_CAP ? 0u : c;
        if (a.seg_val) s_yz[threadIdx.x] = a.seg_scale[(int64_t)q * a.nprobes + g0 + threadIdx.x];
      }
      __syncthreads();
      if (threadIdx.x == 0) {
        uint32_t run = 0;
        for (int i = 0; i < QM_G; ++i) { s_pre[i] = run; run += i < ng ? s_cnt[i] : 0u; }
        s_pre[QM_G] = run;
      }
      __syncthreads();
      const int total = (int)s_pre[QM_G];
      for (int t = threadIdx.x; t < total; t += BS) {
        int rr = 0, st = 0;
#pragma unroll
        for (int i = 1; i < QM_G; ++i) {
          const int pi = (int)s_pre[i];
          if (t >= pi) { rr = i; st = pi; }
        }
        const int64_t e = ((int64_t)q * a.nprobes + g0 + rr) * Q_CAP + (t - st);
        const uint32_t sv = a.seg_val ? (uint32_t)__builtin_amdgcn_fmed3f(rintf(__builtin_fmaf(__uint_as_float(a.seg_pv[e].y), s_yz[rr].x, s_yz[rr].y)), 0.0f, 65535.0f)
                                      : (uint32_t)a.seg_sum[e];
        atomicAdd(&s_hist[min(511u, sv >> a.cut_shift)], 1u);
      }
    }
    __syncthreads();
    if (a.cut_shift >= 0 && threadIdx.x < 64) {
      const int lane = threadIdx.x;
      uint32_t loc[8], tot = 0;
#pragma unroll
      for (int i = 0; i < 8; ++i) { loc[i] = s_hist[lane * 8 + i]; tot += loc[i]; }
      uint32_t incl = tot;
#pragma unroll
      for (int off = 1; off < 64; off <<= 1) {
        const uint32_t tt = __shfl_up(incl, off, 64);
        if (lane >= off) incl += tt;
      }
      uint32_t run = incl - tot;
      int found = -1;
#pragma unroll
      for (int i = 0; i < 8; ++i) {
        run += loc[i];
        if (found < 0 && run >= (uint32_t)o.keff) found = lane * 8 + i;
      }
      const uint64_t mask = __ballot(found >= 0);
      if (mask) {
        const int leader = __ffsll((long long)mask) - 1;
        const int bin = __shfl(found, leader, 64);
        if (lane == 0 && bin < 511) s_cut = (((uint32_t)bin + 1u) << a.cut_shift) - 1u + a.cut_slack + (a.qslack ? 2u * a.qslack[q] : 0u);
      }
    }
    __syncthreads();
    QM_DBG_RETURN(a, 1);
    const uint32_t cut = s_cut;
    for (int g0 = 0; g0 < a.nprobes; g0 += a.qm_g) {
      const int ng = min(a.qm_g, a.nprobes - g0);
      __syncthreads();
      if ((int)threadIdx.x < ng) {
        const uint32_t c = a.seg_cnt[(int64_t)q * a.nprobes + g0 + threadIdx.x];
        s_cnt[threadIdx.x] = c > (uint32_t)Q_CAP ? 0u : c;
        if (a.seg_val) s_yz[threadIdx.x] = a.seg_scale[(int64_t)q * a.nprobes + g0 + threadIdx.x];
      }
      if constexpr (DOT) {
        for (int t = threadIdx.x; t < a.d; t += BS) r[t] = qv[t];
      } else if (a.vec4) {
        const int d4 = a.d >> 2, tot4 = ng * d4;
#pragma unroll 4
        for (int t = threadIdx.x; t < tot4; t += BS) {
          const int rr = t / d4, e4 = t - rr * d4;
          const uint32_t part = a.probes[(int64_t)q * a.nprobes + g0 + rr];
          const f4 qq = reinterpret_cast<const f4 *>(qv)[e4];
          const f4 cc = reinterpret_cast<const f4 *>(a.centroids + (int64_t)part * a.d)[e4];
          f4 v = qq - cc;
          if (a.round_f16) {
#pragma unroll
            for (int e = 0; e < 4; ++e) v[e] = __half2float(__float2half_rn(v[e]));
          }
          *reinterpret_cast<f4 *>(&r[rr * dpad + 4 * e4]) = v;
        }
      } else {
        for (int t = threadIdx.x; t < ng * a.d; t += BS) {
          const int rr = t / a.d, e = t - rr * a.d;
          const uint32_t part = a.probes[(int64_t)q * a.nprobes + g0 + rr];
          float v = qv[e] - a.centroids[(int64_t)part * a.d + e];
          if (a.round_f16) v = __half2float(__float2half_rn(v));
          r[rr * dpad + e] = v;
        }
      }
      __syncthreads();
      QM_DBG_RETURN(a, 2);
      if (threadIdx.x == 0) {
        uint32_t run = 0;
        for (int i = 0; i < QM_G; ++i) { s_pre[i] = run; run += i < ng ? s_cnt[i] : 0u; }
        s_pre[QM_G] = run;
      }
      __syncthreads();
      const int total = (int)s_pre[QM_G];
      for (int chunk0 = 0; chunk0 < total; chunk0 += QM_LC) {
        __syncthreads();
        if (threadIdx.x == 0) l_cnt = 0u;
        __syncthreads();
        const int cend = min(total, chunk0 + QM_LC);
        for (int t = chunk0 + threadIdx.x; t < cend; t += BS) {
          int rr = 0, st = 0;
#pragma unroll
          for (int i = 1; i < QM_G; ++i) {
            const int pi = (int)s_pre[i];
            if (t >= pi) { rr = i; st = pi; }
          }
          const int64_t e = ((int64_t)q * a.nprobes + g0 + rr) * Q_CAP + (t - st);
          uint2 pv = make_uint2(0u, 0u);
          if (a.seg_val) pv = a.seg_pv[e];
          const uint32_t sv = a.seg_val ? (uint32_t)__builtin_amdgcn_fmed3f(rintf(__builtin_fmaf(__uint_as_float(pv.y), s_yz[rr].x, s_yz[rr].y)), 0.0f, 65535.0f)
                                        : (uint32_t)a.seg_sum[e];
          if (sv <= cut) {
            const uint32_t slot = atomicAdd(&l_cnt, 1u);
            l_pos[slot] = a.seg_val ? pv.x : a.seg_pos[e]; l_rr[slot] = (uint8_t)rr;
          }
        }
        __syncthreads();
        QM_DBG_RETURN(a, 3);
        const int nl = (int)l_cnt;
        for (int base = 0; base < nl; base += BS) {
          const bool need_tighten = (int)misc[0] > CAP - BS;
          __syncthreads();
          if (need_tighten) tighten_bs<BS, CAP>(b, o.keff, sorted, &misc[2]);
          const uint32_t T = misc[1];
          const int t = base + threadIdx.x;
          if (t < nl) {
            const uint32_t pos = l_pos[t];
            const int rr = (int)l_rr[t];
            const uint8_t *rc = a.codes + (int64_t)pos * M;
            const float *rres = r + (DOT ? 0 : rr * dpad);
            float dist = 0.0f;
#pragma unroll
            for (int w = 0; w < MU; ++w) {
              const uint4 cw = *reinterpret_cast<const uint4 *>(rc + w * 16);
              const uint32_t cws[4] = {cw.x, cw.y, cw.z, cw.w};
#pragma unroll
              for (int hh = 0; hh < 16 / Q_MPF; ++hh) {
                f4 cbv[Q_MPF][QV];
#pragma unroll
                for (int t8 = 0; t8 < Q_MPF; ++t8) {
                  const int mi = hh * Q_MPF + t8, mm = w * 16 + mi;
                  const uint32_t code = (cws[mi >> 2] >> (8 * (mi & 3))) & 255u;
                  const f4 *src = reinterpret_cast<const f4 *>(a.codebook + ((int64_t)mm * 256 + code) * SD);
#pragma unroll
                  for (int u = 0; u < QV; ++u) cbv[t8][u] = src[u];
                }
#pragma unroll
                for (int t8 = 0; t8 < Q_MPF; ++t8) {
                  const int mm = w * 16 + hh * Q_MPF + t8;
                  RegVec<SD> av;
#pragma unroll
                  for (int u = 0; u < QV; ++u) av.q[u] = *reinterpret_cast<const f4 *>(&rres[mm * SD + 4 * u]);
                  dist += finish_metric<QMET>(dist_exact<SD, QMET>(av, reinterpret_cast<const float *>(&cbv[t8][0])));
                }
              }
            }
            if constexpr (DOT) dist = dist - ((float)M - 1.0f);
            const uint32_t kk = order_key(dist);
            if (kk <= T) {
              const uint32_t slot = atomicAdd(&misc[0], 1u);
              if (slot < (uint32_t)CAP) { ckey[slot] = kk; cpos[slot] = pos; } else misc[3] = 1u;
            }
          }
          __syncthreads();
        }
      }
    }
    __syncthreads();
  }
  QM_DBG_RETURN(a, 4);
  for (int iter = 0; iter < 8 && (int)misc[0] > SCAN_LCAP; ++iter) tighten_bs<BS, CAP>(b, o.keff, sorted, &misc[2]);
  __syncthreads();
  int c = min((int)misc[0], CAP);
  if (c > SCAN_LCAP || misc[3]) {
    if (threadIdx.x == 0) atomicOr(&o.flags[q], FLAG_OVERFLOW);
    c = min(c, SCAN_LCAP);
  }
  for (int i = threadIdx.x; i < SCAN_LCAP; i += BS) {
    if (i < c) { skey[i] = ckey[i]; spos[i] = cpos[i]; rid[i] = a.row_ids[cpos[i]]; }
    else { skey[i] = 0xFFFFFFFFu; spos[i] = 0; rid[i] = ~0ull; }
  }
  __syncthreads();
  int Pq = 64;
  while (Pq < c) Pq <<= 1;
  bitonic_sort_kr<BS>(skey, rid, spos, Pq);
  QM_DBG_RETURN(a, 5);
  select_and_emit<BS>(o, q, skey, rid, spos, c, &s_amb);
}

template <int SD, int MU, int BS, bool DOT = false>
__global__ LH_QM_BOUNDS(BS) void ivfpq_qmerge1g_kernel(QmergeArgs a) {
  extern __shared__ __attribute__((aligned(16))) char smem[];
  constexpr int M = MU * 16;
  constexpr int QV = SD / 4;
  constexpr int QMET = DOT ? METRIC_DOT : METRIC_L2;
  constexpr int CAP = BS == 128 ? 512 : 1024;
  static_assert(BS >= SCAN_MAX_KEFF, "tighten_bs selects among one value per lane");
  __shared__ uint32_t ckey[CAP], cpos[CAP], sorted[BS], misc[8];
  uint64_t *rid = reinterpret_cast<uint64_t *>(smem);
  uint32_t *skey = reinterpret_cast<uint32_t *>(rid + SCAN_LCAP);
  uint32_t *spos = skey + SCAN_LCAP;
  constexpr int QM_LC = 512;
  constexpr int SPL = QM_LC / BS;
  __shared__ uint32_t s_cnt[QM_G], s_part[QM_G];
  __shared__ f2 s_yz[QM_G];
  __shared__ int s_amb;
  __shared__ uint32_t s_hist[512], l_pos[QM_LC], s_cut, l_cnt;
  __shared__ uint8_t l_rr[QM_LC];
  const SelectOut &o = a.o;
  const int q = blockIdx.x;
  const int np = a.nprobes;
  const uint32_t qflags = o.flags[q];
  const uint32_t tb = a.tbound[q];
  uint32_t c_l = 0, part_l = 0;
  f2 yz_l = {0.0f, 0.0f};
  if ((int)threadIdx.x < np) {
    c_l = a.seg_cnt[(int64_t)q * np + threadIdx.x];
    part_l = a.probes[(int64_t)q * np + threadIdx.x];
    if (a.seg_val) yz_l = a.seg_scale[(int64_t)q * np + threadIdx.x];
  }
  const uint32_t qov = a.qovf[q];
  uint32_t tg0 = 0;
  if (threadIdx.x == 0) tg0 = a.tglobal[q];
  if (qflags & FLAG_OVERFLOW) return;
  const bool class_a = tb != 0xFFFFFFFFu;
  if (threadIdx.x == 0) { misc[0] = 0; misc[1] = tg0; misc[3] = 0; s_amb = 0; s_cut = 0xFFFFFFFFu; l_cnt = 0u; }
  for (int i = threadIdx.x; i < 512; i += BS) s_hist[i] = 0u;
  if ((int)threadIdx.x < QM_G) {
    s_cnt[threadIdx.x] = ((int)threadIdx.x < np && c_l <= (uint32_t)Q_CAP) ? c_l : 0u;
    s_part[threadIdx.x] = part_l;
    s_yz[threadIdx.x] = yz_l;
  }
  __syncthreads();
  CandBuf b{ckey, cpos, &misc[0], &misc[1]};
  if (!class_a || qov) {
    const int n = min((int)a.pool_cnt[q], a.pool_cap);
    const uint32_t *pk = a.pool_key + (int64_t)q * a.pool_cap, *pp = a.pool_pos + (int64_t)q * a.pool_cap;
    for (int base = 0; base < n; base += BS) {
      const bool need_tighten = (int)misc[0] > CAP - BS;
      __syncthreads();
      if (need_tighten) tighten_bs<BS, CAP>(b, o.keff, sorted, &misc[2]);
      const uint32_t T = misc[1];
      const int i = base + threadIdx.x;
      if (i < n) {
        const uint32_t kk = pk[i];
        if (kk <= T) {
          const uint32_t slot = atomicAdd(&misc[0], 1u);
          if (slot < (uint32_t)CAP) { ckey[slot] = kk; cpos[slot] = pp[i]; } else misc[3] = 1u;
        }
      }
      __syncthreads();
    }
  }
  if (class_a) {
    const int dpad = (a.d + 3) & ~3;
    float *r = reinterpret_cast<float *>(smem);
    const float *qv = a.q + (int64_t)q * a.d;
    uint32_t total = 0;
    for (int i = 0; i < np; ++i) total += s_cnt[i];
    const int nchunks = ((int)total + QM_LC - 1) / QM_LC;
    uint32_t sv_pos[SPL], sv_sum[SPL];
    uint32_t sv_rr[SPL];
    auto load_chunk = [&](int ch) {
#pragma unroll
      for (int j = 0; j < SPL; ++j) {
        const int t = ch * QM_LC + j * BS + (int)threadIdx.x;
        sv_sum[j] = 0xFFFFFFFFu; sv_pos[j] = 0u; sv_rr[j] = 0u;
        if (t < (int)total) {
          int rr = 0, st = 0, run = 0;
          for (int i = 0; i < np; ++i) {
            if (t >= run) { rr = i; st = run; }
            run += (int)s_cnt[i];
          }
          const int64_t e = ((int64_t)q * np + rr) * Q_CAP + (t - st);
          sv_rr[j] = (uint32_t)rr;
          if (a.seg_val) { const uint2 pv = a.seg_pv[e]; sv_pos[j] = pv.x; sv_sum[j] = pv.y; }
          else { sv_pos[j] = a.seg_pos[e]; sv_sum[j] = (uint32_t)a.seg_sum[e]; }
        }
      }
    };
    bool have[SPL];
    auto mark = [&](int ch) {
#pragma unroll
      for (int j = 0; j < SPL; ++j) have[j] = ch * QM_LC + j * BS + (int)threadIdx.x < (int)total;
    };
    if (nchunks > 0) load_chunk(0);
    mark(0);
    if constexpr (DOT) {
      for (int t = threadIdx.x; t < a.d; t += BS) r[t] = qv[t];
    } else if (a.vec4) {
      const int d4 = a.d >> 2, tot4 = np * d4;
#pragma unroll 4
      for (int t = threadIdx.x; t < tot4; t += BS) {
        const int rr = t / d4, e4 = t - rr * d4;
        const uint32_t part = s_part[rr];
        const f4 qq = reinterpret_cast<const f4 *>(qv)[e4];
        const f4 cc = reinterpret_cast<const f4 *>(a.centroids + (int64_t)part * a.d)[e4];
        f4 v = qq - cc;
        if (a.round_f16) {
#pragma unroll
          for (int e = 0; e < 4; ++e) v[e] = __half2float(__float2half_rn(v[e]));
        }
        *reinterpret_cast<f4 *>(&r[rr * dpad + 4 * e4]) = v;
      }
    } else {
      for (int t = threadIdx.x; t < np * a.d; t += BS) {
        const int rr = t / a.d, e = t - rr * a.d;
        float v = qv[e] - a.centroids[(int64_t)s_part[rr] * a.d + e];
        if (a.round_f16) v = __half2float(__float2half_rn(v));
        r[rr * dpad + e] = v;
      }
    }
    auto to_sums = [&]() {
      if (a.seg_val) {
#pragma unroll
        for (int j = 0; j < SPL; ++j)
          if (have[j]) {
            const f2 yz = s_yz[sv_rr[j]];
            sv_sum[j] = (uint32_t)__builtin_amdgcn_fmed3f(rintf(__builtin_fmaf(__uint_as_float(sv_sum[j]), yz.x, yz.y)), 0.0f, 65535.0f);
          }
      }
    };
    if (a.cut_shift >= 0) {
      for (int ch = 0; ch < nchunks; ++ch) {
        if (ch > 0) { load_chunk(ch); mark(ch); }
        to_sums();
#pragma unroll
        for (int j = 0; j < SPL; ++j)
          if (have[j]) atomicAdd(&s_hist[min(511u, sv_sum[j] >> a.cut_shift)], 1u);
      }
    } else if (nchunks > 0) {
      to_sums();
    }
    __syncthreads();
    if (a.cut_shift >= 0 && threadIdx.x < 64) {
      const int lane = threadIdx.x;
      uint32_t loc[8], tot = 0;
#pragma unroll
      for (int i = 0; i < 8; ++i) { loc[i] = s_hist[lane * 8 + i]; tot += loc[i]; }
      uint32_t incl = tot;
#pragma unroll
      for (int off = 1; off < 64; off <<= 1) {
        const uint32_t tt = __shfl_up(incl, off, 64);
        if (lane >= off) incl += tt;
      }
      uint32_t run = incl - tot;
      int found = -1;
#pragma unroll
      for (int i = 0; i < 8; ++i) {
        run += loc[i];
        if (found < 0 && run >= (uint32_t)o.keff) found = lane * 8 + i;
      }
      const uint64_t mask = __ballot(found >= 0);
      if (mask) {
        const int leader = __ffsll((long long)mask) - 1;
        const int bin = __shfl(found, leader, 64);
        if (lane == 0 && bin < 511) s_cut = (((uint32_t)bin + 1u) << a.cut_shift) - 1u + a.cut_slack + (a.qslack ? 2u * a.qslack[q] : 0u);
      }
    }
    __syncthreads();
    QM_DBG_RETURN(a, 1);
    const uint32_t cut = s_cut;
    for (int ch = 0; ch < nchunks; ++ch) {
      if (nchunks > 1) {
        __syncthreads();
        if (threadIdx.x == 0) l_cnt = 0u;
        __syncthreads();
        load_chunk(ch); mark(ch); to_sums();
      }
#pragma unroll
      for (int j = 0; j < SPL; ++j)
        if (have[j] && sv_sum[j] <= cut) {
          const uint32_t slot = atomicAdd(&l_cnt, 1u);
          l_pos[slot] = sv_pos[j]; l_rr[slot] = (uint8_t)sv_rr[j];
        }
      __syncthreads();
      QM_DBG_RETURN(a, 3);
      const int nl = (int)l_cnt;
      for (int base = 0; base < nl; base += BS) {
        const bool need_tighten = (int)misc[0] > CAP - BS;
        __syncthreads();
        if (need_tighten) tighten_bs<BS, CAP>(b, o.keff, sorted, &misc[2]);
        const uint32_t T = misc[1];
        const int t = base + threadIdx.x;
        if (t < nl) {
          const uint32_t pos = l_pos[t];
          const int rr = (int)l_rr[t];
          const uint8_t *rc = a.codes + (int64_t)pos * M;
          const float *rres = r + (DOT ? 0 : rr * dpad);
          float dist = 0.0f;
#pragma unroll
          for (int w = 0; w < MU; ++w) {
            const uint4 cw = *reinterpret_cast<const uint4 *>(rc + w * 16);
            const uint32_t cws[4] = {cw.x, cw.y, cw.z, cw.w};
#pragma unroll
            for (int hh = 0; hh < 16 / Q_MPF; ++hh) {
              f4 cbv[Q_MPF][QV];
#pragma unroll
              for (int t8 = 0; t8 < Q_MPF; ++t8) {
                const int mi = hh * Q_MPF + t8, mm = w * 16 + mi;
                const uint32_t code = (cws[mi >> 2] >> (8 * (mi & 3))) & 255u;
                const f4 *src = reinterpret_cast<const f4 *>(a.codebook + ((int64_t)mm * 256 + code) * SD);
#pragma unroll
                for (int u = 0; u < QV; ++u) cbv[t8][u] = src[u];
              }
#pragma unroll
              for (int t8 = 0; t8 < Q_MPF; ++t8) {
                const int mm = w * 16 + hh * Q_MPF + t8;
                RegVec<SD> av;
#pragma unroll
                for (int u = 0; u < QV; ++u) av.q[u] = *reinterpret_cast<const f4 *>(&rres[mm * SD + 4 * u]);
                dist += finish_metric<QMET>(dist_exact<SD, QMET>(av, reinterpret_cast<const float *>(&cbv[t8][0])));
              }
            }
          }
          if constexpr (DOT) dist = dist - ((float)M - 1.0f);
          const uint32_t kk = order_key(dist);
          if (kk <= T) {
            const uint32_t slot = atomicAdd(&misc[0], 1u);
            if (slot < (uint32_t)CAP) { ckey[slot] = kk; cpos[slot] = pos; } else misc[3] = 1u;
          }
        }
        __syncthreads();
      }
    }
    __syncthreads();
  }
  QM_DBG_RETURN(a, 4);
  if (o.refine) {
    for (int iter = 0; iter < 8; ++iter) {
      __syncthreads();
      const bool more = (int)misc[0] > BS;
      if (!more) break;
      tighten_bs<BS, CAP>(b, o.keff, sorted, &misc[2]);
    }
    __syncthreads();
    int c1 = (int)misc[0];
    const bool lost = misc[3] != 0u;
    __syncthreads();
    if (!lost && c1 <= BS) {
      if (c1 >= o.keff) {
        tighten_bs<BS, CAP>(b, o.keff, sorted, &misc[2]);
        c1 = (int)misc[0];
      }
      if (c1 <= o.keff) {
        for (int i = threadIdx.x; i < o.keff; i += BS) o.cand_rid[(int64_t)q * o.keff + i] = i < c1 ? a.row_ids[cpos[i]] : ~0ull;
        if (threadIdx.x == 0) o.cand_cnt[q] = (uint32_t)c1;
        return;
      }
    }
  }
  for (int iter = 0; iter < 8 && (int)misc[0] > SCAN_LCAP; ++iter) tighten_bs<BS, CAP>(b, o.keff, sorted, &misc[2]);
  __syncthreads();
  int c = min((int)misc[0], CAP);
  if (c > SCAN_LCAP || misc[3]) {
    if (threadIdx.x == 0) atomicOr(&o.flags[q], FLAG_OVERFLOW);
    c = min(c, SCAN_LCAP);
  }
  for (int i = threadIdx.x; i < SCAN_LCAP; i += BS) {
    if (i < c) { skey[i] = ckey[i]; spos[i] = cpos[i]; rid[i] = a.row_ids[cpos[i]]; }
    else { skey[i] = 0xFFFFFFFFu; spos[i] = 0; rid[i] = ~0ull; }
  }
  __syncthreads();
  int Pq = 64;
  while (Pq < c) Pq <<= 1;
  bitonic_sort_kr<BS>(skey, rid, spos, Pq);
  QM_DBG_RETURN(a, 5);
  select_and_emit<BS>(o, q, skey, rid, spos, c, &s_amb);
}

bool qscan_supported(const lance_hip_index *ix, uint32_t nq, uint32_t nprobes) {
  static const bool off = getenv("LANCE_HIP_NO_QSCAN") != nullptr;
  if (off || !ix->model_finite) return false;
  const int scan_metric = ix->metric == LANCE_HIP_COSINE ? LANCE_HIP_L2 : ix->metric;
  if (scan_metric == LANCE_HIP_DOT) { if (!mscan_dot_ready(ix, nq, nprobes)) return false; }
  else if (scan_metric != LANCE_HIP_L2) return false;
  {
    const int m = (int)ix->m, sd = (int)(ix->d / ix->m);
    if (!((m == 16 || m == 32) && (sd == 4 || sd == 8 || sd == 16)) && !qscan_tiled_shape(m, sd)) return false;
  }
  if ((uint64_t)nq * nprobes * Q_CAP * 4 > (2ull << 30)) return false;
  const bool needs_rq = !qscan_pt_enabled(ix) && !mscan_batch_shape(ix, nq, nprobes);
  if (needs_rq && ((uint64_t)nq * nprobes / Q_G + ix->nlist + 1) * ix->d * 16 > (2ull << 30)) return false;
  return true;
}

size_t qscan_lds_bytes(int d, int m) {
  (void)d; (void)m;
  return (size_t)4 * Q_CAP * 4 + 8 * 4 + (size_t)4 * Q_CAP * 2;
}

int qscan_group(lance_hip_ctx *ctx, const uint32_t *probes, uint32_t nq, uint32_t nprobes, int nlist, const uint32_t *tglobal,
                uint32_t *keys, uint32_t *tbound, uint32_t *pair_starts, uint32_t *pair_idx, uint32_t *item_start4, int4 *desc4,
                uint32_t max_items4, int G, int dot) {
  const size_t npairs = (size_t)nq * nprobes;
  hipLaunchKernelGGL(q_tclass_keys_kernel, dim3((unsigned)cdiv(npairs, 256)), dim3(256), 0, ctx->stream, probes, (int64_t)npairs, (int)nprobes,
                     nlist, tglobal, keys, tbound, dot);
  LH_TRY(stable_group(ctx, keys, (int64_t)npairs, (int64_t)npairs, 2 * nlist, 1, pair_starts, pair_idx, (int64_t)npairs, nullptr));
  hipLaunchKernelGGL(q_item_table_kernel, dim3(1), dim3(256), 0, ctx->stream, pair_starts, nlist, G, item_start4);
  hipLaunchKernelGGL(q_item_desc_kernel, dim3((unsigned)cdiv(max_items4, 256)), dim3(256), 0, ctx->stream, item_start4, pair_starts, nlist, G,
                     max_items4, desc4);
  return LANCE_HIP_OK;
}

int qscan_item_tables(lance_hip_ctx *ctx, const uint32_t *pair_starts, int nlist, int G, uint32_t *item_start, int4 *desc, uint32_t max_items) {
  hipLaunchKernelGGL(q_item_table_kernel, dim3(1), dim3(256), 0, ctx->stream, pair_starts, nlist, G, item_start);
  hipLaunchKernelGGL(q_item_desc_kernel, dim3((unsigned)cdiv(max_items, 256)), dim3(256), 0, ctx->stream, item_start, pair_starts, nlist, G, max_items, desc);
  return LANCE_HIP_OK;
}

int qscan_nearest_keys(lance_hip_ctx *ctx, const uint32_t *probes, uint32_t nq, uint32_t nprobes, uint32_t *keys, uint32_t nb) {
  hipLaunchKernelGGL(q_nearest_keys_kernel, dim3((unsigned)cdiv((uint64_t)nq * nb, 256)), dim3(256), 0, ctx->stream, probes, (int)nq, (int)nprobes, (int)nb, keys);
  return LANCE_HIP_OK;
}

template <int SD>
static bool launch_qscan_sd(lance_hip_ctx *ctx, const QscanArgs &a, int m, unsigned grid, size_t lds) {
  if (m == 16) { hipLaunchKernelGGL((ivfpq_qscan_kernel<SD, 1>), dim3(grid), dim3(Q_BS), lds, ctx->stream, a); return true; }
  if (m == 32) { hipLaunchKernelGGL((ivfpq_qscan_kernel<SD, 2>), dim3(grid), dim3(Q_BS), lds, ctx->stream, a); return true; }
  return false;
}

int qscan_launch(lance_hip_ctx *ctx, const lance_hip_index *ix, const float *qs, uint32_t nq, uint32_t nprobes, const uint32_t *pair_idx,
                 const uint32_t *item_start4, const int4 *desc4, uint32_t max_items4, const uint32_t *tbound, uint32_t *seg_cnt,
                 uint32_t *seg_pos, uint32_t *qovf, const uint32_t *allow, const uint32_t *probes) {
  const int d = (int)ix->d, m = (int)ix->m, sd = d / m;
  const bool pt = probes != nullptr && qscan_pt_enabled(ix);
  f4 *rq = pt ? nullptr : reinterpret_cast<f4 *>(ctx->scratch_t<float>("qscan.rq", (size_t)max_items4 * d * 4));
  if (!pt && !rq) return LANCE_HIP_ENOMEM;
  {
    ScopedTimer t(ctx, "q_residual");
    if (!pt)
      hipLaunchKernelGGL(q_residual_kernel, dim3((unsigned)cdiv(max_items4, 4)), dim3(256), 0, ctx->stream, qs, pair_idx, item_start4, desc4,
                         ix->centroids, d, (int)ix->nlist, (int)nprobes, ix->dtype == LANCE_HIP_F16 ? 1 : 0, rq);
    LH_CHECK_HIP(lh::memset_async(seg_cnt, 0, (size_t)nq * nprobes * 4, ctx->stream));
    LH_CHECK_HIP(lh::memset_async(qovf, 0, (size_t)nq * 4, ctx->stream));
  }
  ScopedTimer t(ctx, "ivfpq_scan_c1");
  QscanArgs a;
  a.rq = rq; a.pair_idx = pair_idx; a.item_start = item_start4; a.desc = desc4;
  a.centroids = ix->centroids; a.codebook = ix->codebook; a.part_offsets = ix->part_offsets; a.codes = ix->codes;
  a.d = d; a.nprobes = (int)nprobes; a.nlist = (int)ix->nlist; a.round_f16 = ix->dtype == LANCE_HIP_F16 ? 1 : 0;
  a.tbound = tbound; a.seg_cnt = seg_cnt; a.seg_pos = seg_pos; a.qovf = qovf; a.allow = allow;
  a.seg_sum = ctx->scratch_t<uint16_t>("q.seg_sum", (size_t)nq * nprobes * Q_CAP);
  a.ovf = ctx->scratch_t<uint32_t>("q.ovf", (size_t)nq * nprobes + 1);
  if (!a.seg_sum || !a.ovf) return LANCE_HIP_ENOMEM;
  LH_CHECK_HIP(lh::memset_async(a.ovf, 0, 4, ctx->stream));
  const size_t lds = qscan_lds_bytes(d, m);
  const unsigned grid = max_items4;
  bool ok = false;
#ifdef LH_QT_PROF
  static const bool qt_prof = getenv("LANCE_HIP_QT_PROF") != nullptr;
  if (qt_prof && qscan_tiled_shape(m, sd)) {
    a.prof = ctx->scratch_t<unsigned long long>("qt.prof", 8);
    if (a.prof) (void)lh::memset_async(a.prof, 0, 64, ctx->stream);
  }
#endif
  if (pt) { LH_TRY(qscan_pt_launch(ctx, ix, a, qs, nq, probes, grid)); ok = true; }
  else if (qscan_tiled_shape(m, sd)) ok = qscan_tiled_launch(ctx, a, m, sd, grid);
  else if (sd == 4) ok = launch_qscan_sd<4>(ctx, a, m, grid, lds);
  else if (sd == 8) ok = launch_qscan_sd<8>(ctx, a, m, grid, lds);
  else if (sd == 16) ok = launch_qscan_sd<16>(ctx, a, m, grid, lds);
  LH_REQUIRE(ok, "quantised scan: unsupported shape (m=%d, sd=%d)", m, sd);
#ifdef LH_QT_PROF
  if (a.prof) {
    unsigned long long h[8];
    (void)hipMemcpyAsync(h, a.prof, 64, hipMemcpyDeviceToHost, ctx->stream);
    (void)hipStreamSynchronize(ctx->stream);
    if (h[3]) fprintf(stderr, "[qt prof] items=%llu  100 MHz clocks per item: table build %.0f | row scan %.0f\n", h[3], (double)h[0] / h[3], (double)h[1] / h[3]);
  }
#endif
  return LANCE_HIP_OK;
}

template <int SD>
static bool launch_qbound_sd(lance_hip_ctx *ctx, const QboundArgs &a, int m, unsigned grid, size_t lds) {
  if (m == 16) { hipLaunchKernelGGL((ivfpq_qbound_kernel<SD, 1>), dim3(grid), dim3(Q_BS), lds, ctx->stream, a); return true; }
  if (m == 32) { hipLaunchKernelGGL((ivfpq_qbound_kernel<SD, 2>), dim3(grid), dim3(Q_BS), lds, ctx->stream, a); return true; }
  return false;
}

__global__ __launch_bounds__(256) void q_codebook_mean_kernel(const float *__restrict__ codebook, int sd, int d, float *__restrict__ out) {
  __shared__ float part[4];
  const int mm = blockIdx.x, c = threadIdx.x, lane = c & 63, wave = c >> 6;
  const float *cw = codebook + ((int64_t)mm * 256 + c) * sd;
  float sq = 0.0f;
  for (int e = 0; e <= sd; ++e) {
    float v;
    if (e < sd) { v = cw[e]; sq += v * v; } else v = sq;
#pragma unroll
    for (int o = 32; o > 0; o >>= 1) v += __shfl_xor(v, o, 64);
    __syncthreads();
    if (lane == 0) part[wave] = v;
    __syncthreads();
    if (c == 0) {
      const float tot = (part[0] + part[1] + part[2] + part[3]) * (1.0f / 256.0f);
      if (e < sd) out[mm * sd + e] = tot; else atomicAdd(&out[d], tot);
    }
  }
}

__global__ __launch_bounds__(256) void q_model_finite_kernel(const float *__restrict__ a, int64_t na, const float *__restrict__ b, int64_t nb,
                                                             uint32_t *__restrict__ flag) {
  const int64_t i = (int64_t)blockIdx.x * 256 + threadIdx.x;
  bool bad = false;
  if (i < na) bad = !isfinite(a[i]);
  else if (i < na + nb) bad = !isfinite(b[i - na]);
  if (__any(bad) && (threadIdx.x & 63) == 0) atomicOr(flag, 1u);
}

int qscan_index_constants(lance_hip_ctx *ctx, lance_hip_index *ix) {
  const int d = (int)ix->d, m = (int)ix->m;
  if (!ix->cb_mean) LH_CHECK_HIP(hipMalloc(reinterpret_cast<void **>(&ix->cb_mean), (size_t)(d + 2) * 4));
  LH_CHECK_HIP(lh::memset_async(ix->cb_mean, 0, (size_t)(d + 2) * 4, ctx->stream));
  hipLaunchKernelGGL(q_codebook_mean_kernel, dim3((unsigned)m), dim3(256), 0, ctx->stream, ix->codebook, d / m, d, ix->cb_mean);
  const int64_t nc = (int64_t)ix->nlist * d, ncb = (int64_t)m * 256 * (d / m);
  hipLaunchKernelGGL(q_model_finite_kernel, dim3((unsigned)cdiv((uint64_t)(nc + ncb), 256)), dim3(256), 0, ctx->stream, ix->centroids, nc, ix->codebook,
                     ncb, reinterpret_cast<uint32_t *>(ix->cb_mean + d + 1));
  LH_CHECK_HIP(hipGetLastError());
  return LANCE_HIP_OK;
}

int qscan_items(lance_hip_ctx *ctx, const uint32_t *pair_starts, int nvp, int G, uint32_t *item_start, int4 *desc, uint32_t max_items) {
  hipLaunchKernelGGL(q_item_table_kernel, dim3(1), dim3(256), 0, ctx->stream, pair_starts, nvp, G, item_start);
  hipLaunchKernelGGL(q_item_desc_kernel, dim3((unsigned)cdiv(max_items, 256)), dim3(256), 0, ctx->stream, item_start, pair_starts, nvp, G, max_items, desc);
  LH_CHECK_HIP(hipGetLastError());
  return LANCE_HIP_OK;
}

int qbound_launch(lance_hip_ctx *ctx, const lance_hip_index *ix, const float *qs, uint32_t nq, uint32_t keff, const uint32_t *pair_starts0,
                  const uint32_t *pair_idx0, uint32_t *item_start, int4 *desc, uint32_t max_items, uint32_t *tglobal, const uint32_t *allow) {
  const int d = (int)ix->d, m = (int)ix->m, sd = d / m, nlist = (int)ix->nlist;
  hipLaunchKernelGGL(q_item_table_kernel, dim3(1), dim3(256), 0, ctx->stream, pair_starts0, nlist, Q_G, item_start);
  hipLaunchKernelGGL(q_item_desc_kernel, dim3((unsigned)cdiv(max_items, 256)), dim3(256), 0, ctx->stream, item_start, pair_starts0, nlist, Q_G,
                     max_items, desc);
  f4 *rq = reinterpret_cast<f4 *>(ctx->scratch_t<float>("qbound.rq", (size_t)max_items * d * 4));
  if (!rq) return LANCE_HIP_ENOMEM;
  hipLaunchKernelGGL(q_residual_kernel, dim3((unsigned)cdiv(max_items, 4)), dim3(256), 0, ctx->stream, qs, pair_idx0, item_start, desc, ix->centroids, d,
                     nlist, 1, ix->dtype == LANCE_HIP_F16 ? 1 : 0, rq);
  QboundArgs a;
  a.rq = rq; a.pair_idx = pair_idx0; a.item_start = item_start; a.desc = desc;
  a.centroids = ix->centroids; a.codebook = ix->codebook; a.part_offsets = ix->part_offsets; a.codes = ix->codes;
  a.d = d; a.nlist = nlist; a.keff = (int)keff; a.round_f16 = ix->dtype == LANCE_HIP_F16 ? 1 : 0;
  a.tglobal = tglobal; a.allow = allow;
  LH_REQUIRE(ix->cb_mean, "integer bound pass: the index carries no codebook means (8-bit PQ only)");
  a.cb_mean = ix->cb_mean;
  const size_t lds = (size_t)4 * QB_BINS * 4 + 8 * 4;
  bool ok = false;
  if (qscan_tiled_shape(m, sd)) ok = qbound_tiled_launch(ctx, a, m, sd, max_items);
  else if (sd == 4) ok = launch_qbound_sd<4>(ctx, a, m, max_items, lds);
  else if (sd == 8) ok = launch_qbound_sd<8>(ctx, a, m, max_items, lds);
  else if (sd == 16) ok = launch_qbound_sd<16>(ctx, a, m, max_items, lds);
  LH_REQUIRE(ok, "integer bound pass: unsupported shape (m=%d, sd=%d)", m, sd);
  (void)nq;
  return LANCE_HIP_OK;
}

template <int SD, int MU, bool DOT = false>
static void launch_qmerge_mu(lance_hip_ctx *ctx, const QmergeArgs &a, unsigned nq, int bs) {
  const int dpad = (a.d + 3) & ~3;
  const size_t lds_rescan = (size_t)dpad * 4 + (size_t)MU * 16 * 256 * 4;
  const unsigned rgrid = (unsigned)std::min<uint64_t>((uint64_t)nq * a.nprobes, (uint64_t)ctx->num_cus);
  hipLaunchKernelGGL((ivfpq_qrescan_kernel<SD, MU, 1024, DOT>), dim3(rgrid), dim3(1024), lds_rescan, ctx->stream, a);
  const size_t lds = std::max((size_t)std::min<int>(a.qm_g, a.nprobes) * dpad * 4, (size_t)SCAN_LCAP * 16);
  static const bool v1 = getenv("LANCE_HIP_QMERGE_V1") != nullptr;
  if (!v1 && a.nprobes <= a.qm_g) {
    if (bs == 256) hipLaunchKernelGGL((ivfpq_qmerge1g_kernel<SD, MU, 256, DOT>), dim3(nq), dim3(256), lds, ctx->stream, a);
    else hipLaunchKernelGGL((ivfpq_qmerge1g_kernel<SD, MU, 128, DOT>), dim3(nq), dim3(128), lds, ctx->stream, a);
    return;
  }
  if (bs == 256) hipLaunchKernelGGL((ivfpq_qmerge_kernel<SD, MU, 256, DOT>), dim3(nq), dim3(256), lds, ctx->stream, a);
  else hipLaunchKernelGGL((ivfpq_qmerge_kernel<SD, MU, 128, DOT>), dim3(nq), dim3(128), lds, ctx->stream, a);
}

int qmerge_launch(lance_hip_ctx *ctx, const lance_hip_index *ix, const float *qs, uint32_t nq, const uint32_t *probes, uint32_t nprobes,
                  const uint32_t *tbound, uint32_t *tglobal, const uint32_t *seg_cnt, const uint32_t *seg_pos, const uint32_t *qovf,
                  uint32_t *pool_key, uint32_t *pool_pos, uint32_t *pool_cnt, int pool_cap, const SelectOut &o, const uint32_t *allow,
                  const uint32_t *qslack, const float *seg_val, const float *seg_scale) {
  const int d = (int)ix->d, m = (int)ix->m, sd = d / m;
  QmergeArgs a;
  a.qslack = qslack; a.seg_val = seg_val; a.seg_pv = reinterpret_cast<const uint2 *>(seg_val); a.seg_scale = reinterpret_cast<const f2 *>(seg_scale);
#ifdef LH_TIMING_EXPERIMENTS
  {
    static const int dbg = [] {
      const int v = getenv("LANCE_HIP_QM_DBG") ? atoi(getenv("LANCE_HIP_QM_DBG")) : 0;
      if (v) fprintf(stderr, "lance_hip: LANCE_HIP_QM_DBG=%d -- timing experiment, search RESULTS ARE WRONG\n", v);
      return v;
    }();
    a.dbg = dbg;
  }
#endif
  a.q = qs; a.probes = probes; a.centroids = ix->centroids; a.codebook = ix->codebook; a.codes = ix->codes; a.row_ids = ix->row_ids;
  a.d = d; a.nprobes = (int)nprobes; a.round_f16 = ix->dtype == LANCE_HIP_F16 ? 1 : 0;
  a.tbound = tbound; a.tglobal = tglobal; a.seg_cnt = seg_cnt; a.seg_pos = seg_pos; a.qovf = qovf;
  a.pool_key = pool_key; a.pool_pos = pool_pos; a.pool_cnt = pool_cnt; a.pool_cap = pool_cap; a.allow = allow;
  a.o = o;
  {
    const int dpad = (d + 3) & ~3;
    a.qm_g = std::max(1, std::min(QM_G, 32768 / (dpad * 4)));
    a.vec4 = (d % 4 == 0) && ((reinterpret_cast<uintptr_t>(qs) | reinterpret_cast<uintptr_t>(ix->centroids)) & 15) == 0;
  }
  {
    static const bool no_cut = getenv("LANCE_HIP_NO_QCUT") != nullptr;
    a.seg_sum = ctx->scratch_t<uint16_t>("q.seg_sum", (size_t)nq * nprobes * Q_CAP);
    a.ovf = ctx->scratch_t<uint32_t>("q.ovf", (size_t)nq * nprobes + 1);
    if (!a.seg_sum || !a.ovf) return LANCE_HIP_ENOMEM;
    const bool tiled = qscan_tiled_shape(m, sd);
    a.cut_shift = no_cut ? -1 : (tiled ? 7 : (m == 16 ? 3 : 2));
    a.cut_slack = tiled ? (uint32_t)(2 * m + 8) : (uint32_t)(2 * m + 4);
    if (qslack) {
      int sh = 0; uint32_t sl = 0;
      mscan_cut_params(&sh, &sl);
      a.cut_shift = no_cut ? -1 : sh; a.cut_slack = sl;
    }
  }
  static const int bs = getenv("LANCE_HIP_QMERGE_BS") ? atoi(getenv("LANCE_HIP_QMERGE_BS")) : 128;
  bool ok = true;
  if (ix->metric == LANCE_HIP_DOT) {
    if (m == 16 && sd == 4) launch_qmerge_mu<4, 1, true>(ctx, a, nq, bs);
    else if (m == 16 && sd == 8) launch_qmerge_mu<8, 1, true>(ctx, a, nq, bs);
    else if (m == 32 && sd == 4) launch_qmerge_mu<4, 2, true>(ctx, a, nq, bs);
    else ok = false;
  } else if (m == 16) {
    if (sd == 4) launch_qmerge_mu<4, 1>(ctx, a, nq, bs);
    else if (sd == 8) launch_qmerge_mu<8, 1>(ctx, a, nq, bs);
    else if (sd == 16) launch_qmerge_mu<16, 1>(ctx, a, nq, bs);
    else ok = false;
  } else if (m == 32) {
    if (sd == 4) launch_qmerge_mu<4, 2>(ctx, a, nq, bs);
    else if (sd == 8) launch_qmerge_mu<8, 2>(ctx, a, nq, bs);
    else if (sd == 16) launch_qmerge_mu<16, 2>(ctx, a, nq, bs);
    else ok = false;
  } else if (m == 48) {
    if (sd == 4) launch_qmerge_mu<4, 3>(ctx, a, nq, bs);
    else if (sd == 8) launch_qmerge_mu<8, 3>(ctx, a, nq, bs);
    else if (sd == 16) launch_qmerge_mu<16, 3>(ctx, a, nq, bs);
    else ok = false;
  } else if (m == 64) {
    if (sd == 4) launch_qmerge_mu<4, 4>(ctx, a, nq, bs);
    else if (sd == 8) launch_qmerge_mu<8, 4>(ctx, a, nq, bs);
    else if (sd == 16) launch_qmerge_mu<16, 4>(ctx, a, nq, bs);
    else ok = false;
  } else if (m == 96) {
    if (sd == 4) launch_qmerge_mu<4, 6>(ctx, a, nq, bs);
    else if (sd == 8) launch_qmerge_mu<8, 6>(ctx, a, nq, bs);
    else if (sd == 16) launch_qmerge_mu<16, 6>(ctx, a, nq, bs);
    else ok = false;
  } else ok = false;
  LH_REQUIRE(ok, "quantised scan merge: unsupported shape (m=%d, sd=%d)", m, sd);
  return LANCE_HIP_OK;
}

}
```

Before: 25.44 million queries/s.

## Count scan survivors in LDS, split tall lists in two, prefetch next chunk

The matrix-core scan now counts surviving candidates per resident pair with LDS atomics and publishes one global atomicAdd per pair at the end of each slice, instead of one global atomic per survivor. Partitions needing more than two row slices are rebalanced into exactly two halves when they fit under a tall-row cap. Each half writes one end of the per-pair segment buffer, front or back, and a new seg_back array tells the merge kernels how to index records. The scan also software-prefetches the next chunk's codes and norms and drops the per-chunk vmcnt wait. This adds flags, extra LDS and a new buffer, and the ordering and overflow accounting need careful handling.

```diff
diff --git a/lance_amd/csrc/kernels.h b/lance_amd/csrc/kernels.h
--- a/lance_amd/csrc/kernels.h
+++ b/lance_amd/csrc/kernels.h
@@ -163,14 +163,15 @@
 int qmerge_launch(lance_hip_ctx *ctx, const lance_hip_index *ix, const float *qs, uint32_t nq, const uint32_t *probes, uint32_t nprobes,
                   const uint32_t *tbound, uint32_t *tglobal, const uint32_t *seg_cnt, const uint32_t *seg_pos, const uint32_t *qovf,
                   uint32_t *pool_key, uint32_t *pool_pos, uint32_t *pool_cnt, int pool_cap, const SelectOut &o, const uint32_t *allow,
-                  const uint32_t *qslack = nullptr, const float *seg_val = nullptr, const float *seg_scale = nullptr);
+                  const uint32_t *qslack = nullptr, const float *seg_val = nullptr, const float *seg_scale = nullptr,
+                  const uint32_t *seg_back = nullptr);
 constexpr int LH_NOT_TAKEN = 1;
 bool mscan_supported(const lance_hip_index *ix, uint32_t nq, uint32_t nprobes);
 bool mscan_batch_shape(const lance_hip_index *ix, uint32_t nq, uint32_t nprobes);
 bool mscan_dot_ready(const lance_hip_index *ix, uint32_t nq, uint32_t nprobes);
 int mscan_launch(lance_hip_ctx *ctx, const lance_hip_index *ix, const float *qs, uint32_t nq, uint32_t nprobes, const uint32_t *probes,
                  const uint32_t *pair_starts, const uint32_t *pair_idx, const uint32_t *tbound, uint32_t *seg_cnt, uint32_t *seg_pos,
-                 uint32_t *qovf, const uint32_t *allow, uint32_t **qslack_out, float **seg_val_out, float **seg_scale_out);
+                 uint32_t *qovf, const uint32_t *allow, uint32_t **qslack_out, float **seg_val_out, float **seg_scale_out, uint32_t **seg_back_out);
 void mscan_cut_params(int *cut_shift, uint32_t *cut_slack);
 int mscan_prewarm(lance_hip_ctx *ctx, const lance_hip_index *ix);
 int msbound_launch(lance_hip_ctx *ctx, const lance_hip_index *ix, const float *qs, uint32_t nq, uint32_t keff, const uint32_t *pair_starts0,
diff --git a/lance_amd/csrc/search_ms.hip b/lance_amd/csrc/search_ms.hip
--- a/lance_amd/csrc/search_ms.hip
+++ b/lance_amd/csrc/search_ms.hip
@@ -203,28 +203,39 @@
   static const int v = [] { const char *e = getenv("LANCE_HIP_MS_RS2"); const int x = e ? atoi(e) : 0; return x >= 64 ? (x / 64) * 64 : ms_rows_per_slice(); }();
   return v;
 }
-struct MsSlice { uint32_t off, np, row_begin, row_count, gs, qp, pad0, pad1; };
+constexpr uint32_t MS_SLICE_BACK = 1u, MS_SLICE_SHARED = 2u;
+struct MsSlice { uint32_t off, np, row_begin, row_count, gs, qp, flags, pad1; };
 __host__ __device__ __forceinline__ uint32_t ms_nrs(uint32_t np, uint32_t rs1, uint32_t rs2) { return np <= rs1 ? (np ? 1u : 0u) : 1u + (np - rs1 + rs2 - 1u) / rs2; }
 __device__ __forceinline__ uint32_t ms_row_begin(uint32_t rs, uint32_t rs1, uint32_t rs2) { return rs ? rs1 + (rs - 1u) * rs2 : 0u; }
 __device__ __forceinline__ uint32_t ms_row_count(uint32_t rs, uint32_t np, uint32_t rs1, uint32_t rs2) {
   return rs ? min(rs2, np - ms_row_begin(rs, rs1, rs2)) : min(rs1, np);
 }
+constexpr int MS3_TALL = 8192;
+static int ms_tall_rows() {
+  static const int v = [] { const char *e = getenv("LANCE_HIP_MS_TALL"); const int x = e ? atoi(e) : MS3_TALL; return x > 0 ? (x / 64) * 64 : 0; }();
+  return v;
+}
 
 __device__ __forceinline__ uint32_t ms_work_class(uint32_t rows, uint32_t pairs, uint32_t rs_rows) {
   const uint64_t w = (uint64_t)rows * pairs;
   return 31u - (uint32_t)min<uint64_t>(31u, w * 32u / ((uint64_t)rs_rows * MS3_PB));
 }
-struct MsSplit { uint32_t npb, blk, nrs; };
-__device__ __forceinline__ MsSplit ms_split(uint32_t qp, uint32_t np, uint32_t rs_rows, uint32_t rs2_rows) {
+struct MsSplit { uint32_t npb, blk, nrs, h1, h2; };
+__device__ __forceinline__ MsSplit ms_split(uint32_t qp, uint32_t np, uint32_t rs_rows, uint32_t rs2_rows, uint32_t tall_rows) {
   MsSplit r;
   r.npb = (qp + MS3_PB - 1) / MS3_PB;
   r.blk = r.npb ? ((((qp + r.npb - 1) / r.npb) + 31u) & ~31u) : 0u;
-  r.nrs = ms_nrs(np, rs_rows, rs2_rows);
+  r.h1 = rs_rows; r.h2 = rs2_rows;
+  if (ms_nrs(np, rs_rows, rs2_rows) > 2u) {
+    const uint32_t h = (((np + 1u) >> 1) + 63u) & ~63u;
+    if (h <= tall_rows) r.h1 = r.h2 = h;
+  }
+  r.nrs = ms_nrs(np, r.h1, r.h2);
   return r;
 }
 
 __global__ __launch_bounds__(256) void ms_slice_table_kernel(const uint32_t *__restrict__ pair_starts, const uint32_t *__restrict__ part_offsets, int nlist,
-                                                             uint32_t rs_rows, uint32_t rs2_rows, uint32_t cls_rows, uint32_t *__restrict__ slice_start,
+                                                             uint32_t rs_rows, uint32_t rs2_rows, uint32_t tall_rows, uint32_t cls_rows, uint32_t *__restrict__ slice_start,
                                                              uint32_t *__restrict__ slice_ctr, uint32_t *__restrict__ cls_cursor) {
   __shared__ uint32_t wsum[4];
   __shared__ uint32_t carry_s;
@@ -238,13 +249,13 @@
     uint32_t v = 0;
     if (i < nlist) {
       const uint32_t qp = pair_starts[i + 1] - pair_starts[i], np = part_offsets[i + 1] - part_offsets[i];
-      const MsSplit sp = ms_split(qp, np, rs_rows, rs2_rows);
+      const MsSplit sp = ms_split(qp, np, rs_rows, rs2_rows, tall_rows);
       v = sp.npb * sp.nrs;
       for (uint32_t pb = 0; pb < sp.npb; pb += max(1u, sp.npb - 1u)) {
         const uint32_t pairs = min(sp.blk, qp - pb * sp.blk), npb_same = (pb + 1 == sp.npb) ? 1u : sp.npb - 1u;
-        if (sp.nrs > 0) atomicAdd(&hist[ms_work_class(ms_row_count(0u, np, rs_rows, rs2_rows), pairs, cls_rows)], npb_same);
-        if (sp.nrs > 2) atomicAdd(&hist[ms_work_class(rs2_rows, pairs, cls_rows)], npb_same * (sp.nrs - 2u));
-        if (sp.nrs > 1) atomicAdd(&hist[ms_work_class(ms_row_count(sp.nrs - 1u, np, rs_rows, rs2_rows), pairs, cls_rows)], npb_same);
+        if (sp.nrs > 0) atomicAdd(&hist[ms_work_class(ms_row_count(0u, np, sp.h1, sp.h2), pairs, cls_rows)], npb_same);
+        if (sp.nrs > 2) atomicAdd(&hist[ms_work_class(sp.h2, pairs, cls_rows)], npb_same * (sp.nrs - 2u));
+        if (sp.nrs > 1) atomicAdd(&hist[ms_work_class(ms_row_count(sp.nrs - 1u, np, sp.h1, sp.h2), pairs, cls_rows)], npb_same);
         if (sp.npb == 1) break;
       }
     }
@@ -272,20 +283,21 @@
 }
 
 __global__ __launch_bounds__(256) void ms_slice_desc_kernel(const uint32_t *__restrict__ slice_start, const uint32_t *__restrict__ pair_starts,
-                                                            const uint32_t *__restrict__ part_offsets, int nlist, uint32_t rs_rows, uint32_t rs2_rows, uint32_t cls_rows,
-                                                            MsSlice *__restrict__ slices, uint32_t *__restrict__ cls_cursor, uint32_t *__restrict__ order) {
+                                                            const uint32_t *__restrict__ part_offsets, int nlist, uint32_t rs_rows, uint32_t rs2_rows, uint32_t tall_rows,
+                                                            uint32_t cls_rows, MsSlice *__restrict__ slices, uint32_t *__restrict__ cls_cursor, uint32_t *__restrict__ order) {
   const int part = blockIdx.x * 4 + (threadIdx.x >> 6), lane = threadIdx.x & 63;
   if (part >= nlist) return;
   const uint32_t s0 = slice_start[part], s1 = slice_start[part + 1];
   if (s1 == s0) return;
   const uint32_t off = part_offsets[part], np = part_offsets[part + 1] - off;
   const uint32_t gs = pair_starts[part], qp = pair_starts[part + 1] - gs;
-  const MsSplit sp = ms_split(qp, np, rs_rows, rs2_rows);
+  const MsSplit sp = ms_split(qp, np, rs_rows, rs2_rows, tall_rows);
   for (uint32_t t = (uint32_t)lane; t < s1 - s0; t += 64u) {
     const uint32_t pb = t / sp.nrs, rs = t - pb * sp.nrs;
     MsSlice u;
-    u.off = off; u.np = np; u.row_begin = ms_row_begin(rs, rs_rows, rs2_rows); u.row_count = ms_row_count(rs, np, rs_rows, rs2_rows);
-    u.gs = gs + pb * sp.blk; u.qp = min(sp.blk, qp - pb * sp.blk); u.pad0 = u.pad1 = 0u;
+    u.off = off; u.np = np; u.row_begin = ms_row_begin(rs, sp.h1, sp.h2); u.row_count = ms_row_count(rs, np, sp.h1, sp.h2);
+    u.gs = gs + pb * sp.blk; u.qp = min(sp.blk, qp - pb * sp.blk); u.pad1 = 0u;
+    u.flags = sp.nrs > 2u ? MS_SLICE_SHARED : (rs == 1u ? MS_SLICE_BACK : 0u);
     slices[s0 + t] = u;
     order[atomicAdd(&cls_cursor[ms_work_class(u.row_count, u.qp, cls_rows)], 1u)] = s0 + t;
   }
@@ -305,6 +317,7 @@
   uint32_t nan_slot;
   int nlist, nprobes;
   uint32_t *seg_cnt, *seg_pos;
+  uint32_t *seg_back = nullptr;
   uint2 *seg_pv = nullptr;
   uint32_t *ovf;
   const uint32_t *allow;
@@ -333,60 +346,69 @@
   __shared__ __attribute__((aligned(16))) char sB[MS3_PB * RB];
   __shared__ __attribute__((aligned(16))) float sLim[MS3_PB];
   __shared__ __attribute__((aligned(16))) uint32_t sPair[MS3_PB];
-  __shared__ __attribute__((aligned(8))) uint2 sQ[16][2][MS_QH + 1];
+  __shared__ __attribute__((aligned(8))) uint2 sQ[16][MS_QH + 1];
+  __shared__ uint32_t sCnt[MS3_PB];
   __shared__ uint32_t s_slice, s_chunk;
+  static_assert(MS3_PB <= 1024, "one lane per resident pair publishes its count");
   const int lane = threadIdx.x & 63, wave = __builtin_amdgcn_readfirstlane((int)(threadIdx.x >> 6));
   const int j = lane & 31, g = lane >> 5;
   const uint32_t nslices = p.slice_start[p.nlist];
 
-  uint2 *const qw = &sQ[wave][0][0];
-  uint32_t cur = 0;
+  uint2 *const qw = &sQ[wave][0];
   uint32_t qn = 0;
-  uint32_t pd_n = 0, pd_base = 0;
-  uint32_t pd_k = 0;
   float ncn2v = 0.0f;
+  uint32_t sflags = 0;
   long long pc_t0 = 0, pc_stage = 0, pc_gather = 0, pc_tiles = 0, pc_flush = 0, pct = 0, pc_nchunk = 0;
   if constexpr (PROF) { pc_t0 = clock64(); pct = pc_t0; }
-  auto flush_end = [&]() {
-    if (pd_n) {
-      if ((uint32_t)lane < pd_n && pd_k != 0xFFFFFFFFu) {
-        const uint2 ent = qw[((uint32_t)(MS_QH + 1) - cur) + (uint32_t)lane];
-        const uint32_t pair = sPair[ent.x >> 8];
-        if (pd_k < (uint32_t)Q_CAP) {
-          p.seg_pv[(int64_t)pair * Q_CAP + pd_k] = make_uint2(pd_base + (ent.x & 255u), ent.y);
-        } else if (pd_k == (uint32_t)Q_CAP) {
-          p.ovf[1u + atomicAdd(&p.ovf[0], 1u)] = pair;
-        }
-      }
-      pd_n = 0;
-    }
+  auto flush = [&](uint32_t pos_base) {
+    const uint2 raw = qw[lane];
+    const uint32_t ln_e = raw.x & 63u, vv = (raw.x >> 6) & 15u, jbb = raw.x >> 10;
+    const float nv = __shfl(ncn2v, (int)(ln_e & 31u), 64);
+    const uint32_t eslot = jbb * 32u + 4u * (ln_e >> 5) + (vv & 3u) + 8u * (vv >> 2), pos = pos_base + (ln_e & 31u);
+    const uint32_t val = __float_as_uint(__uint_as_float(raw.y) - nv);
+    if ((uint32_t)lane < qn && !(MS_DBG(p) & 1) && row_allowed(p.allow, pos)) {
+      const uint32_t pair = sPair[eslot];
+      uint2 *seg = p.seg_pv + (int64_t)pair * Q_CAP;
+      if (sflags & MS_SLICE_SHARED) {
+        const uint32_t k = atomicAdd(&p.seg_cnt[pair], 1u);
+        if (k < (uint32_t)Q_CAP) seg[k] = make_uint2(pos, val);
+        else if (k == (uint32_t)Q_CAP) p.ovf[1u + atomicAdd(&p.ovf[0], 1u)] = pair;
+      } else {
+        const uint32_t k = atomicAdd(&sCnt[eslot], 1u);
+        if (k < (uint32_t)Q_CAP) seg[(sflags & MS_SLICE_BACK) ? (uint32_t)(Q_CAP - 1) - k : k] = make_uint2(pos, val);
+      }
+    }
+    qn = 0;
   };
-  auto flush_begin = [&](uint32_t pos_base) {
-    pd_k = 0xFFFFFFFFu;
-    {
-      const uint2 raw = qw[cur + (uint32_t)lane];
-      const uint32_t ln_e = raw.x & 63u, vv = (raw.x >> 6) & 15u, jbb = raw.x >> 10;
-      const float nv = __shfl(ncn2v, (int)(ln_e & 31u), 64);
-      const uint2 ent = make_uint2(((jbb * 32u + 4u * (ln_e >> 5) + (vv & 3u) + 8u * (vv >> 2)) << 8) | (ln_e & 31u), __float_as_uint(__uint_as_float(raw.y) - nv));
-      if ((uint32_t)lane < qn && !(MS_DBG(p) & 1)) {
-        qw[cur + (uint32_t)lane] = ent;
-        if (row_allowed(p.allow, pos_base + (ent.x & 255u))) pd_k = atomicAdd(&p.seg_cnt[sPair[ent.x >> 8]], 1u);
-      }
-    }
-    pd_n = qn; pd_base = pos_base; qn = 0;
-    cur = (uint32_t)(MS_QH + 1) - cur;
-  };
+  if (threadIdx.x < MS3_PB) sCnt[threadIdx.x] = 0u;
+  int pubQp = 0;
+  uint32_t pubflags = 0;
 
   for (;;) {
     __syncthreads();
     if (threadIdx.x == 0) { s_slice = atomicAdd(p.slice_ctr, 1u); s_chunk = 0u; }
+    uint32_t pub_c = 0, pub_pair = 0, pub_k = 0;
+    if (threadIdx.x < MS3_PB) {
+      pub_c = (int)threadIdx.x < pubQp ? sCnt[threadIdx.x] : 0u;
+      pub_pair = sPair[threadIdx.x];
+      sCnt[threadIdx.x] = 0u;
+    }
     __syncthreads();
+    if (pub_c) {
+      pub_k = atomicAdd(&p.seg_cnt[pub_pair], pub_c);
+      if (pubflags & MS_SLICE_BACK) p.seg_back[pub_pair] = pub_c;
+    }
+    auto publish_end = [&]() {
+      if (pub_c && pub_k <= (uint32_t)Q_CAP && pub_k + pub_c > (uint32_t)Q_CAP) p.ovf[1u + atomicAdd(&p.ovf[0], 1u)] = pub_pair;
+    };
     const uint32_t slice = s_slice;
-    if (slice >= nslices) break;
+    if (slice >= nslices) { publish_end(); break; }
     long long pc_slice0 = 0;
     if constexpr (PROF) pc_slice0 = clock64();
     const MsSlice U = p.slices[p.order[slice]];
     const int Qp = (int)U.qp;
+    sflags = U.flags;
+    pubQp = (U.flags & MS_SLICE_SHARED) ? 0 : Qp; pubflags = U.flags;
     const int nslots = ((Qp + 31) >> 5) << 5;
     {
       const char *src = reinterpret_cast<const char *>(p.rh + (int64_t)U.gs * D);
@@ -405,29 +427,41 @@
       }
     }
     asm volatile("s_waitcnt vmcnt(0)" ::: "memory");
+    publish_end();
     __syncthreads();
     if constexpr (PROF) { const long long t = clock64(); pc_stage += t - pct; pct = t; }
     const uint32_t nchunks = (U.row_count + 31u) >> 5;
     const int nblk = nslots >> 5;
     const int row_end = (int)(U.row_begin + U.row_count);
 
-    for (;;) {
+    auto take = [&]() -> uint32_t {
       uint32_t c = 0;
       if (lane == 0) c = atomicAdd(&s_chunk, 1u);
-      c = (uint32_t)__builtin_amdgcn_readfirstlane((int)c);
-      if (c >= nchunks) break;
+      return (uint32_t)__builtin_amdgcn_readfirstlane((int)c);
+    };
+    uint32_t cwn[M / 4];
+    float ncn2n = -INFINITY;
+    auto request = [&](uint32_t c) {
+      const int row0 = (int)(U.row_begin + c * 32u);
+      const int rowc = min(row0 + j, row_end - 1);
+      const uint4 *rc4 = reinterpret_cast<const uint4 *>(p.codes + ((int64_t)U.off + rowc) * M);
+#pragma unroll
+      for (int w = 0; w < M / 16; ++w) { const uint4 t = rc4[w]; cwn[4 * w] = t.x; cwn[4 * w + 1] = t.y; cwn[4 * w + 2] = t.z; cwn[4 * w + 3] = t.w; }
+      const float cn = p.row_cn2[(int64_t)U.off + rowc];
+      ncn2n = row0 + j < row_end ? -cn : -INFINITY;
+    };
+    uint32_t c = take();
+    if (c < nchunks) request(c);
+    while (c < nchunks) {
+      const uint32_t cnext = take();
       const int row0 = (int)(U.row_begin + c * 32u);
 
       ms_h8 rw[KS];
       {
-        const int rowc = min(row0 + j, row_end - 1);
         uint32_t cw[M / 4];
-        {
-          const uint4 *rc4 = reinterpret_cast<const uint4 *>(p.codes + ((int64_t)U.off + rowc) * M);
-#pragma unroll
-          for (int w = 0; w < M / 16; ++w) { const uint4 t = rc4[w]; cw[4 * w] = t.x; cw[4 * w + 1] = t.y; cw[4 * w + 2] = t.z; cw[4 * w + 3] = t.w; }
-        }
-        ncn2v = row0 + j < row_end ? -p.row_cn2[(int64_t)U.off + rowc] : -INFINITY;
+#pragma unroll
+        for (int w = 0; w < M / 4; ++w) cw[w] = cwn[w];
+        ncn2v = ncn2n;
         auto code = [&](int mm) -> uint32_t { return (cw[mm >> 2] >> (8 * (mm & 3))) & 255u; };
 #pragma unroll
         for (int s = 0; s < KS; ++s) {
@@ -445,8 +479,10 @@
           }
         }
       }
+      __builtin_amdgcn_sched_barrier(0);
+      request(min(cnext, nchunks - 1u));
+      __builtin_amdgcn_sched_barrier(0);
       const uint32_t pos_base = U.off + (uint32_t)row0;
-      asm volatile("s_waitcnt vmcnt(0)" ::: "memory");
 #pragma unroll
       for (int s = 0; s < KS; ++s) asm volatile("" : "+v"(rw[s]));
       asm volatile("" : "+v"(ncn2v));
@@ -476,7 +512,7 @@
         }
         if (qn > (uint32_t)(MS_QH - 32)) {
           if constexpr (PROF) { const long long t = clock64(); pc_tiles += t - pct; pct = t; }
-          flush_end(); flush_begin(pos_base);
+          flush(pos_base);
           if constexpr (PROF) { const long long t = clock64(); pc_flush += t - pct; pct = t; }
         }
         uint32_t qraw = qn;
@@ -501,7 +537,7 @@
 #else
               const uint32_t ln = (uint32_t)lane;
 #endif
-              qw[cur + idx] = make_uint2((((uint32_t)jb << 10) | (uint32_t)(v << 6)) | ln, __float_as_uint(acc[v]));
+              qw[idx] = make_uint2((((uint32_t)jb << 10) | (uint32_t)(v << 6)) | ln, __float_as_uint(acc[v]));
             }
             qraw += (uint32_t)__popcll(mk[v]);
           }
@@ -516,10 +552,10 @@
         }
       }
       if constexpr (PROF) { const long long t = clock64(); pc_tiles += t - pct; pct = t; }
-      flush_end(); flush_begin(pos_base);
+      flush(pos_base);
       if constexpr (PROF) { const long long t = clock64(); pc_flush += t - pct; pct = t; ++pc_nchunk; }
-    }
-    flush_end();
+      c = cnext;
+    }
     if constexpr (PROF) {
       __syncthreads();
       if (threadIdx.x == 0 && p.prof_slices) p.prof_slices[slice] = (unsigned long long)(clock64() - pc_slice0);
@@ -901,7 +937,7 @@
 
 int mscan_launch(lance_hip_ctx *ctx, const lance_hip_index *ix_c, const float *qs, uint32_t nq, uint32_t nprobes, const uint32_t *probes,
                  const uint32_t *pair_starts, const uint32_t *pair_idx, const uint32_t *tbound, uint32_t *seg_cnt, uint32_t *seg_pos,
-                 uint32_t *qovf, const uint32_t *allow, uint32_t **qslack_out, float **seg_val_out, float **seg_scale_out) {
+                 uint32_t *qovf, const uint32_t *allow, uint32_t **qslack_out, float **seg_val_out, float **seg_scale_out, uint32_t **seg_back_out) {
   lance_hip_index *ix = const_cast<lance_hip_index *>(ix_c);
   int sd = 0, ks = 0;
   if (!ms_shape(ix, &sd, &ks)) return LH_NOT_TAKEN;
@@ -918,13 +954,14 @@
   MsSlice *slices = reinterpret_cast<MsSlice *>(ctx->scratch("ms.slices", cap * sizeof(MsSlice)));
   uint32_t *order = ctx->scratch_t<uint32_t>("ms.order", cap);
   float *seg_val = ctx->scratch_t<float>("ms.seg_val", npairs * Q_CAP * 2);
+  uint32_t *seg_back = ctx->scratch_t<uint32_t>("ms.seg_back", npairs);
   uint32_t *ovf = ctx->scratch_t<uint32_t>("q.ovf", npairs + 1);
-  if (!rh || !prm || !prm2 || !qslack || !slice_start || !slices || !order || !seg_val || !ovf) return LANCE_HIP_ENOMEM;
+  if (!rh || !prm || !prm2 || !qslack || !slice_start || !slices || !order || !seg_val || !seg_back || !ovf) return LANCE_HIP_ENOMEM;
   uint32_t *slice_ctr = slice_start + nlist + 1, *cls_cursor = slice_ctr + 1;
   const uint32_t nan_slot = (uint32_t)npairs + 1u;
   {
     ScopedTimer t(ctx, "q_residual");
-    LH_CHECK_HIP(lh::memset_multi(ctx->stream, {{seg_cnt, 0, npairs * 4}, {qovf, 0, (size_t)nq * 4}, {qslack, 0, (size_t)nq * 4}, {ovf, 0, 4}}));
+    LH_CHECK_HIP(lh::memset_multi(ctx->stream, {{seg_cnt, 0, npairs * 4}, {seg_back, 0, npairs * 4}, {qovf, 0, (size_t)nq * 4}, {qslack, 0, (size_t)nq * 4}, {ovf, 0, 4}}));
     MsPrepArgs pa;
     pa.q = qs; pa.centroids = ix->centroids; pa.pair_idx = pair_idx; pa.pair_starts = pair_starts; pa.probes = probes; pa.tbound = tbound;
     pa.d = d; pa.nprobes = (int)nprobes; pa.nlist = nlist; pa.round_f16 = ix->dtype == LANCE_HIP_F16 ? 1 : 0;
@@ -932,13 +969,13 @@
     pa.nan_slot = nan_slot; pa.prm2 = prm2;
     pa.dot = ix->metric == LANCE_HIP_DOT ? 1 : 0; pa.cmax = ix->ms->cmax; pa.cmax_full = ix->ms->cmax_full; pa.cmaxp = ix->ms->cmaxp; pa.mu = ix->cb_mean; pa.m = (int)ix->m;
     hipLaunchKernelGGL(ms_prep_kernel, dim3((unsigned)cdiv(npairs, 4 * MS_PPW)), dim3(256), 0, ctx->stream, pa);
-    const uint32_t rs_rows = (uint32_t)ms_rows_per_slice(), rs2_rows = (uint32_t)ms_rows_per_slice2();
+    const uint32_t rs_rows = (uint32_t)ms_rows_per_slice(), rs2_rows = (uint32_t)ms_rows_per_slice2(), tall_rows = (uint32_t)ms_tall_rows();
     static const bool no_order = getenv("LANCE_HIP_MS_NOORDER") != nullptr;
     const uint32_t cls_rows = no_order ? 0x40000000u : rs_rows;
-    hipLaunchKernelGGL(ms_slice_table_kernel, dim3(1), dim3(256), 0, ctx->stream, pair_starts, ix->part_offsets, nlist, rs_rows, rs2_rows, cls_rows, slice_start,
-                       slice_ctr, cls_cursor);
+    hipLaunchKernelGGL(ms_slice_table_kernel, dim3(1), dim3(256), 0, ctx->stream, pair_starts, ix->part_offsets, nlist, rs_rows, rs2_rows, tall_rows, cls_rows,
+                       slice_start, slice_ctr, cls_cursor);
     hipLaunchKernelGGL(ms_slice_desc_kernel, dim3((unsigned)cdiv((uint64_t)nlist, 4)), dim3(256), 0, ctx->stream, slice_start, pair_starts, ix->part_offsets,
-                       nlist, rs_rows, rs2_rows, cls_rows, slices, cls_cursor, order);
+                       nlist, rs_rows, rs2_rows, tall_rows, cls_rows, slices, cls_cursor, order);
   }
   ScopedTimer t(ctx, "ivfpq_scan_c1");
   ScopedTimer tm(ctx, "ivfpq_mscan");
@@ -946,7 +983,7 @@
   a.order = order; a.slices = slices; a.slice_start = slice_start; a.slice_ctr = slice_ctr; a.codes = ix->codes;
   a.cbh = reinterpret_cast<const _Float16 *>(ix->ms->cbh); a.row_cn2 = ix->ms->row_cn2; a.rh = rh; a.prm = prm; a.prm2 = prm2;
   a.nan_slot = nan_slot; a.nlist = nlist; a.nprobes = (int)nprobes;
-  a.seg_cnt = seg_cnt; a.seg_pos = seg_pos; a.seg_pv = reinterpret_cast<uint2 *>(seg_val); a.ovf = ovf; a.allow = allow;
+  a.seg_cnt = seg_cnt; a.seg_pos = seg_pos; a.seg_back = seg_back; a.seg_pv = reinterpret_cast<uint2 *>(seg_val); a.ovf = ovf; a.allow = allow;
 #ifdef LH_TIMING_EXPERIMENTS
   static const int dbg = [] {
     const int v = getenv("LANCE_HIP_MS_DBG") ? atoi(getenv("LANCE_HIP_MS_DBG")) : 0;
@@ -1001,7 +1038,7 @@
   else if (sd == 4 && ks == 4) hipLaunchKernelGGL((ivfpq_mscan_kernel<4, 4>), dim3(grid), dim3(1024), 0, ctx->stream, a);
   else { set_error("matrix-core scan: unsupported shape (d=%d, sd=%d)", d, sd); return LANCE_HIP_EINVAL; }
   LH_CHECK_HIP(hipGetLastError());
-  *qslack_out = qslack; *seg_val_out = seg_val; *seg_scale_out = reinterpret_cast<float *>(prm2);
+  *qslack_out = qslack; *seg_val_out = seg_val; *seg_scale_out = reinterpret_cast<float *>(prm2); *seg_back_out = seg_back;
   return LANCE_HIP_OK;
 }
 
diff --git a/lance_amd/csrc/search_pm.hip b/lance_amd/csrc/search_pm.hip
--- a/lance_amd/csrc/search_pm.hip
+++ b/lance_amd/csrc/search_pm.hip
@@ -614,13 +614,14 @@
   }
   uint32_t *qslack = nullptr;
   float *seg_val = nullptr, *seg_scale = nullptr;
+  uint32_t *seg_back = nullptr;
   int ms_rc = LH_NOT_TAKEN;
   if (mscan_supported(ix, nq, nprobes))
-    ms_rc = mscan_launch(ctx, ix, qs, nq, nprobes, probes, pair_starts, pair_idx, tbound, seg_cnt, seg_pos, qovf, allow, &qslack, &seg_val, &seg_scale);
+    ms_rc = mscan_launch(ctx, ix, qs, nq, nprobes, probes, pair_starts, pair_idx, tbound, seg_cnt, seg_pos, qovf, allow, &qslack, &seg_val, &seg_scale, &seg_back);
   if (ms_rc < 0) return ms_rc;
   if (ms_rc == LH_NOT_TAKEN && dot) return LH_NOT_TAKEN;
   if (ms_rc == LH_NOT_TAKEN) {
-    qslack = nullptr; seg_val = nullptr; seg_scale = nullptr;
+    qslack = nullptr; seg_val = nullptr; seg_scale = nullptr; seg_back = nullptr;
     LH_TRY(qscan_launch(ctx, ix, qs, nq, nprobes, pair_idx, item_start4, desc4, max_items4, tbound, seg_cnt, seg_pos, qovf, allow, probes));
   }
   static const bool q_stats = getenv("LANCE_HIP_Q_STATS") != nullptr;
@@ -653,7 +654,7 @@
     o.out_ids = ids; o.out_dists = dists; o.cand_rid = cand_rid; o.cand_cnt = cand_cnt; o.flags = flags;
     o.part_offsets = ix->part_offsets; o.nlist = nlist;
     ScopedTimer t(ctx, "ivfpq_merge");
-    LH_TRY(qmerge_launch(ctx, ix, qs, nq, probes, nprobes, tbound, tglobal, seg_cnt, seg_pos, qovf, pool_key, pool_pos, pool_cnt, pool_cap, o, allow, qslack, seg_val, seg_scale));
+    LH_TRY(qmerge_launch(ctx, ix, qs, nq, probes, nprobes, tbound, tglobal, seg_cnt, seg_pos, qovf, pool_key, pool_pos, pool_cnt, pool_cap, o, allow, qslack, seg_val, seg_scale, seg_back));
   }
   LH_CHECK_HIP(hipGetLastError());
   return LANCE_HIP_OK;
diff --git a/lance_amd/csrc/search_q.hip b/lance_amd/csrc/search_q.hip
--- a/lance_amd/csrc/search_q.hip
+++ b/lance_amd/csrc/search_q.hip
@@ -343,6 +343,7 @@
   const float *seg_val;
   const uint2 *seg_pv;
   const f2 *seg_scale;
+  const uint32_t *seg_back;
 #ifdef LH_TIMING_EXPERIMENTS
   int dbg;
 #define QM_DBG_RETURN(a, n) do { if ((a).dbg == (n)) return; } while (0)
@@ -359,6 +360,8 @@
   const uint32_t *allow;
   SelectOut o;
 };
+
+__device__ __forceinline__ int seg_record(int t, int front) { return t < front ? t : Q_CAP - 1 - (t - front); }
 
 template <int SD, int MU, int BS, bool DOT = false>
 __global__ __launch_bounds__(BS) void ivfpq_qrescan_kernel(QmergeArgs a) {
@@ -479,7 +482,7 @@
   uint64_t *rid = reinterpret_cast<uint64_t *>(smem);
   uint32_t *skey = reinterpret_cast<uint32_t *>(rid + SCAN_LCAP);
   uint32_t *spos = skey + SCAN_LCAP;
-  __shared__ uint32_t s_cnt[QM_G + 1], s_pre[QM_G + 1];
+  __shared__ uint32_t s_cnt[QM_G + 1], s_pre[QM_G + 1], s_front[QM_G];
   __shared__ f2 s_yz[QM_G];
   __shared__ int s_amb;
   constexpr int QM_LC = 512;
@@ -523,7 +526,9 @@
       __syncthreads();
       if ((int)threadIdx.x < ng) {
         const uint32_t c = a.seg_cnt[(int64_t)q * a.nprobes + g0 + threadIdx.x];
+        const uint32_t bk = a.seg_back ? a.seg_back[(int64_t)q * a.nprobes + g0 + threadIdx.x] : 0u;
         s_cnt[threadIdx.x] = c > (uint32_t)Q_CAP ? 0u : c;
+        s_front[threadIdx.x] = c > (uint32_t)Q_CAP ? 0u : c - bk;
         if (a.seg_val) s_yz[threadIdx.x] = a.seg_scale[(int64_t)q * a.nprobes + g0 + threadIdx.x];
       }
       __syncthreads();
@@ -541,7 +546,7 @@
           const int pi = (int)s_pre[i];
           if (t >= pi) { rr = i; st = pi; }
         }
-        const int64_t e = ((int64_t)q * a.nprobes + g0 + rr) * Q_CAP + (t - st);
+        const int64_t e = ((int64_t)q * a.nprobes + g0 + rr) * Q_CAP + seg_record(t - st, (int)s_front[rr]);
         const uint32_t sv = a.seg_val ? (uint32_t)__builtin_amdgcn_fmed3f(rintf(__builtin_fmaf(__uint_as_float(a.seg_pv[e].y), s_yz[rr].x, s_yz[rr].y)), 0.0f, 65535.0f)
                                       : (uint32_t)a.seg_sum[e];
         atomicAdd(&s_hist[min(511u, sv >> a.cut_shift)], 1u);
@@ -581,7 +586,9 @@
       __syncthreads();
       if ((int)threadIdx.x < ng) {
         const uint32_t c = a.seg_cnt[(int64_t)q * a.nprobes + g0 + threadIdx.x];
+        const uint32_t bk = a.seg_back ? a.seg_back[(int64_t)q * a.nprobes + g0 + threadIdx.x] : 0u;
         s_cnt[threadIdx.x] = c > (uint32_t)Q_CAP ? 0u : c;
+        s_front[threadIdx.x] = c > (uint32_t)Q_CAP ? 0u : c - bk;
         if (a.seg_val) s_yz[threadIdx.x] = a.seg_scale[(int64_t)q * a.nprobes + g0 + threadIdx.x];
       }
       if constexpr (DOT) {
@@ -631,7 +638,7 @@
             const int pi = (int)s_pre[i];
             if (t >= pi) { rr = i; st = pi; }
           }
-          const int64_t e = ((int64_t)q * a.nprobes + g0 + rr) * Q_CAP + (t - st);
+          const int64_t e = ((int64_t)q * a.nprobes + g0 + rr) * Q_CAP + seg_record(t - st, (int)s_front[rr]);
           uint2 pv = make_uint2(0u, 0u);
           if (a.seg_val) pv = a.seg_pv[e];
           const uint32_t sv = a.seg_val ? (uint32_t)__builtin_amdgcn_fmed3f(rintf(__builtin_fmaf(__uint_as_float(pv.y), s_yz[rr].x, s_yz[rr].y)), 0.0f, 65535.0f)
@@ -728,7 +735,7 @@
   uint32_t *spos = skey + SCAN_LCAP;
   constexpr int QM_LC = 512;
   constexpr int SPL = QM_LC / BS;
-  __shared__ uint32_t s_cnt[QM_G], s_part[QM_G];
+  __shared__ uint32_t s_cnt[QM_G], s_part[QM_G], s_front[QM_G];
   __shared__ f2 s_yz[QM_G];
   __shared__ int s_amb;
   __shared__ uint32_t s_hist[512], l_pos[QM_LC], s_cut, l_cnt;
@@ -738,10 +745,11 @@
   const int np = a.nprobes;
   const uint32_t qflags = o.flags[q];
   const uint32_t tb = a.tbound[q];
-  uint32_t c_l = 0, part_l = 0;
+  uint32_t c_l = 0, part_l = 0, bk_l = 0;
   f2 yz_l = {0.0f, 0.0f};
   if ((int)threadIdx.x < np) {
     c_l = a.seg_cnt[(int64_t)q * np + threadIdx.x];
+    if (a.seg_back) bk_l = a.seg_back[(int64_t)q * np + threadIdx.x];
     part_l = a.probes[(int64_t)q * np + threadIdx.x];
     if (a.seg_val) yz_l = a.seg_scale[(int64_t)q * np + threadIdx.x];
   }
@@ -754,6 +762,7 @@
   for (int i = threadIdx.x; i < 512; i += BS) s_hist[i] = 0u;
   if ((int)threadIdx.x < QM_G) {
     s_cnt[threadIdx.x] = ((int)threadIdx.x < np && c_l <= (uint32_t)Q_CAP) ? c_l : 0u;
+    s_front[threadIdx.x] = ((int)threadIdx.x < np && c_l <= (uint32_t)Q_CAP) ? c_l - bk_l : 0u;
     s_part[threadIdx.x] = part_l;
     s_yz[threadIdx.x] = yz_l;
   }
@@ -798,7 +807,7 @@
             if (t >= run) { rr = i; st = run; }
             run += (int)s_cnt[i];
           }
-          const int64_t e = ((int64_t)q * np + rr) * Q_CAP + (t - st);
+          const int64_t e = ((int64_t)q * np + rr) * Q_CAP + seg_record(t - st, (int)s_front[rr]);
           sv_rr[j] = (uint32_t)rr;
           if (a.seg_val) { const uint2 pv = a.seg_pv[e]; sv_pos[j] = pv.x; sv_sum[j] = pv.y; }
           else { sv_pos[j] = a.seg_pos[e]; sv_sum[j] = (uint32_t)a.seg_sum[e]; }
@@ -1202,9 +1211,10 @@
 int qmerge_launch(lance_hip_ctx *ctx, const lance_hip_index *ix, const float *qs, uint32_t nq, const uint32_t *probes, uint32_t nprobes,
                   const uint32_t *tbound, uint32_t *tglobal, const uint32_t *seg_cnt, const uint32_t *seg_pos, const uint32_t *qovf,
                   uint32_t *pool_key, uint32_t *pool_pos, uint32_t *pool_cnt, int pool_cap, const SelectOut &o, const uint32_t *allow,
-                  const uint32_t *qslack, const float *seg_val, const float *seg_scale) {
+                  const uint32_t *qslack, const float *seg_val, const float *seg_scale, const uint32_t *seg_back) {
   const int d = (int)ix->d, m = (int)ix->m, sd = d / m;
   QmergeArgs a;
+  a.seg_back = seg_back;
   a.qslack = qslack; a.seg_val = seg_val; a.seg_pv = reinterpret_cast<const uint2 *>(seg_val); a.seg_scale = reinterpret_cast<const f2 *>(seg_scale);
 #ifdef LH_TIMING_EXPERIMENTS
   {
```

New measurement: 25.40 million queries/s. No clear change (-0.2%).
